# uc-vision/smart-tree

Measured on AMD Instinct MI355X. Metric: points/sec end-to-end (voxelize->sparse-UNet->skeleton), 1M-pt tree, higher is better.
Workload: dtype f32

## Files before the change

### include/smarttree_hip.h

```cpp
#ifndef SMARTTREE_HIP_H
#define SMARTTREE_HIP_H

#include <stdint.h>

#ifdef __cplusplus
extern "C" {
#endif

int st_version(void);
#define ST_SKELETON_STATS_ENTRIES 16
#define ST_SKELETON_TUNING_ENTRIES 24
int st_abi_entries(int what);
const char* st_last_error(void);
int64_t st_query_workspace(int op, int64_t a, int64_t b, int64_t c);

int64_t st_scan_workspace_bytes(int64_t n);
int st_scan_u32(const uint32_t* in, uint32_t* out, int64_t n, uint32_t* total, void* ws, int64_t ws_bytes, void* stream);
int64_t st_sort_workspace_bytes(int64_t n);
int st_sort_pairs_u32(uint32_t* keys, uint32_t* vals, int64_t n, int key_bits, void* ws, int64_t ws_bytes, void* stream);

int64_t st_voxelize_workspace_bytes(int64_t n_points, int max_blocks, int64_t max_voxels);
int st_voxelize_blocks(const float* xyz, const float* rgb, int64_t n, double voxel_size, double block_size,
                       double buffer_size, int min_points, int max_blocks, int64_t max_voxels, float* feats,
                       int32_t* coords, uint8_t* mask, int64_t* point_index, float* block_centres,
                       int64_t* n_voxels_host, int64_t* n_blocks_host, void* ws, int64_t ws_bytes, void* stream);

int64_t st_hash_capacity(int64_t n);
int st_build_coord_hash(const int32_t* coords, int64_t n, unsigned long long* keys, unsigned* vals, int64_t cap, void* stream);
int st_build_subm_rulebook(const int32_t* coords, int64_t n, const unsigned long long* keys, const unsigned* vals,
                           int64_t cap, int32_t* nbr , void* stream);
int64_t st_spatial_order_workspace_bytes(int64_t n);
int st_spatial_order(const int32_t* coords, int64_t n, int32_t* order , void* ws, int64_t ws_bytes, void* stream);
int st_move_rows(const void* src, int row_words, const int32_t* order, int64_t n, void* dst, int scatter, void* stream);
int64_t st_strided_workspace_bytes(int64_t n_fine);
int st_build_strided_outputs(const int32_t* coords, int64_t n, int64_t max_out, int32_t* out_coords,
                             unsigned long long* ckeys, unsigned* cvals, int64_t ccap, int64_t* n_out_host,
                             int32_t* extent_host , void* ws, int64_t ws_bytes, void* stream);
int st_build_strided_rulebook(const int32_t* coords, int64_t n, const unsigned long long* fkeys, const unsigned* fvals,
                              int64_t fcap, const int32_t* out_coords, int64_t n_out, const unsigned long long* ckeys,
                              const unsigned* cvals, int64_t ccap, const int32_t* extent_host,
                              int32_t* nbr_down , int32_t* nbr_up ,
                              int32_t* up_order ,
                              void* stream);

int st_sparse_conv_fwd(const float* x0, int c0, const float* x1, int cin, const int32_t* nbr, int K, int64_t n_out,
                       const float* w, int cout, const float* scale, const float* shift, const float* residual,
                       int relu, float* y, const int32_t* row_order ,
                       void* stream, int64_t nbr_stride );
int st_sparse_conv_mfma_fwd(const float* x0, int c0, const float* x1, int cin, const int32_t* nbr, int K, int64_t n_out,
                            const float* wp, int cout, const float* scale, const float* shift, const float* residual,
                            int relu, float* y, const int32_t* row_order ,
                            void* stream, int64_t nbr_stride ,
                            int variant );
int st_sparse_conv_b3_fwd(const float* x0, int c0, const float* x1, int cin, const int32_t* nbr, int K, int64_t n_out, const void* wq,
                          int cout, const float* scale, const float* shift, const float* residual, int relu, float* y,
                          const int32_t* row_order, void* stream, int64_t nbr_stride, int variant);
int st_sparse_conv_f16_fwd(const void* x0, int c0, const void* x1, int cin, const int32_t* nbr, int K, int64_t n_out,
                           const void* w, int cout, const float* scale, const float* shift, const void* residual, int relu,
                           void* y, int in_half, int out_half, const int32_t* row_order, void* stream, int64_t nbr_stride );

int64_t st_brick_pyramid_workspace_bytes(int64_t n0, int n_blocks, int coord_bound, int depth, const int64_t* caps);
int st_brick_pyramid(const int32_t* coords0 , int64_t n0, int n_blocks ,
                     int coord_bound , int depth, const int32_t* blk_seg ,
                     int nseg, const int64_t* caps ,
                     int32_t* order0 , int32_t* const* coords_out ,
                     int32_t* const* subm , int32_t* const* down ,
                     int32_t* const* up , int32_t* const* up_order ,
                     int64_t* counts_host , void* ws, int64_t ws_bytes, void* stream);
int st_head_param_floats(void);
int st_pointwise_mlp_heads(const float* x, int64_t n, const float* params, float* radius, float* direction,
                           float* class_l, float* medial_vector , int64_t* class_idx , void* stream);

int st_centre_cloud(const float* xyz, int64_t n, float* out, void* ws, int64_t ws_bytes, void* stream);
int st_medial_points(const float* xyz, const float* mv, int64_t n, float* medial, float* radius, void* stream);
int64_t st_knn_workspace_bytes(int64_t n_dst);
int st_knn_radius(const float* src, int64_t n1, const float* dst, int64_t n2, int K, float r, const float* bound,
                  int bound_mode, float cell_hint, int64_t* idx, float* dist, void* ws, int64_t ws_bytes, void* stream);
int64_t st_make_edges_workspace_bytes(int64_t n);
int st_make_edges(const int64_t* idx, const float* dist, int64_t n, int K, int64_t* edges, float* w,
                  int64_t* n_edges_host, void* ws, int64_t ws_bytes, void* stream);
int64_t st_connected_components_workspace_bytes(int64_t n);
int st_connected_components(const int64_t* edges, int64_t E, int64_t n, int32_t* labels, void* ws, int64_t ws_bytes, void* stream);
int64_t st_component_layout_workspace_bytes(int64_t n);
int st_component_layout(const int32_t* labels, int64_t n, int min_vertices, int32_t* comp_size, int32_t* comp_off,
                        int32_t* vert_order, int32_t* new_id, int64_t* n_comp_host, int64_t* n_kept_host, void* ws,
                        int64_t ws_bytes, void* stream);
int64_t st_component_csr_workspace_bytes(int64_t m);
int st_component_csr(const int64_t* edges, const float* w, int64_t E, const int32_t* new_id, int64_t m, uint32_t* row_off,
                     uint32_t* col, float* wgt, void* ws, int64_t ws_bytes, void* stream);
int64_t st_skeleton_workspace_bytes(int64_t m, int64_t n_comp);
int st_skeleton_components(int n_comp, const int32_t* comp_off, const int32_t* comp_size_host, int64_t m, const float* pts,
                           const float* rad, const float* ysurf, const uint32_t* row_off, const uint32_t* col,
                           const float* wgt, float grid_cell, int stages, int block_threads, float* dist, int32_t* pred,
                           int32_t* root_local, float* tree_dist, int32_t* branch_parent, int32_t* branch_off,
                           int32_t* branch_len, int32_t* n_branches, int32_t* path_verts, int32_t* branch_of,
                           int64_t* stats_host, void* ws, int64_t ws_bytes, void* stream);
#define ST_SKELETON_STAGE_ARGS                                                                                          \
    int n_comp, const int32_t *comp_off, const int32_t *comp_size_host, int64_t m, const float *pts, const float *rad, \
        const float *ysurf, const uint32_t *row_off, const uint32_t *col, const float *wgt, float grid_cell,           \
        int block_threads, float *dist, int32_t *pred, int32_t *root_local, float *tree_dist, int32_t *branch_parent,  \
        int32_t *branch_off, int32_t *branch_len, int32_t *n_branches, int32_t *path_verts, int32_t *branch_of,        \
        int64_t *stats_host, void *ws, int64_t ws_bytes, void *stream
int st_sssp(ST_SKELETON_STAGE_ARGS);
int st_tree_distance(ST_SKELETON_STAGE_ARGS);
int st_sample_tree(ST_SKELETON_STAGE_ARGS);
int64_t st_assemble_workspace_bytes(int64_t cap_b);
int st_assemble_branches(int n_comp, const int32_t* comp_off, const int32_t* n_branches, const int32_t* branch_parent,
                         const int32_t* branch_off, const int32_t* branch_len, const int32_t* path_verts,
                         const int32_t* vert_order, const float* medial, const float* radius, int32_t* tree_off,
                         int32_t* parent, int32_t* start, int32_t* length, float* xyz, float* rad, int64_t cap_b,
                         int64_t cap_p, int64_t* counts_host, void* ws, int64_t ws_bytes, void* stream);
int st_post_process(int n_trees, const int32_t* tree_off, const int32_t* parent, const int32_t* start, const int32_t* len,
                    float* xyz, const float* rad_in, float* rad_out, uint8_t* keep, uint8_t* repaired, uint8_t* smoothed,
                    int32_t* depth_scratch, int do_prune, float min_radius, float min_length, int do_repair, int do_smooth, int kernel_size,
                    void* stream);

int st_points_to_nearest_tube(const float* pts, int64_t n, const float* a, const float* b, const float* r1, const float* r2,
                              int64_t m, float* vec, int64_t* idx, float* rad, void* stream);

int st_centre_cloud_seg(const float* xyz, int64_t n, const int32_t* seg_off, int nseg, float* out, void* ws,
                        int64_t ws_bytes , void* stream);
int64_t st_voxelize_workspace_bytes_seg(int64_t n_points, int max_blocks, int64_t max_voxels, int nseg);
int st_voxelize_blocks_seg(const float* xyz, const float* rgb, int64_t n, const int32_t* seg_off, int nseg,
                           double voxel_size, double block_size, double buffer_size, int min_points, int max_blocks,
                           int64_t max_voxels, float* feats, int32_t* coords, uint8_t* mask, int64_t* point_index,
                           float* block_centres, int32_t* blk_seg ,
                           int32_t* seg_vox_off , int32_t* seg_blk_off , int64_t* n_voxels_host,
                           int64_t* n_blocks_host, void* ws, int64_t ws_bytes, void* stream);
int st_build_strided_outputs_seg(const int32_t* coords, int64_t n, int64_t max_out, int32_t* out_coords,
                                 unsigned long long* ckeys, unsigned* cvals, int64_t ccap, int64_t* n_out_host,
                                 int32_t* extent_host, const int32_t* blk_seg, int nseg, int32_t* ext_dev ,
                                 void* ws, int64_t ws_bytes, void* stream);
int st_build_strided_rulebook_seg(const int32_t* coords, int64_t n, const unsigned long long* fkeys, const unsigned* fvals,
                                  int64_t fcap, const int32_t* out_coords, int64_t n_out, const unsigned long long* ckeys,
                                  const unsigned* cvals, int64_t ccap, const int32_t* extent_host, int32_t* nbr_down,
                                  int32_t* nbr_up, int32_t* up_order, const int32_t* blk_seg, const int32_t* ext_dev,
                                  void* stream);
int64_t st_voxelize_cloud_workspace_bytes(int64_t n_points, int64_t max_voxels, int nseg);
int st_voxelize_cloud_seg(const float* xyz, const float* rgb, int64_t n, const int32_t* seg_off, int nseg, double voxel_size,
                          int64_t max_voxels, float* feats, int32_t* coords, uint8_t* mask, int64_t* point_index,
                          int32_t* seg_vox_off, int64_t* n_voxels_host, void* ws, int64_t ws_bytes, void* stream);
int64_t st_knn_workspace_bytes_seg(int64_t n_dst, int nseg);
int st_knn_radius_seg(const float* src, int64_t n1, const float* dst, int64_t n2, int K, float r, const float* bound,
                      int bound_mode, float cell_hint, int64_t* idx, float* dist, const int32_t* src_seg_off,
                      const int32_t* dst_seg_off, int nseg, void* ws, int64_t ws_bytes, void* stream, float cell_mean_mult);
int st_radius_count_seg(const float* src, int64_t n1, const float* dst, int64_t n2, int K, float r, const float* bound,
                        int bound_mode, float cell_hint, uint8_t* mask, const int32_t* src_seg_off,
                        const int32_t* dst_seg_off, int nseg, void* ws, int64_t ws_bytes, void* stream, float cell_mean_mult,
                        const uint8_t* valid );
int64_t st_component_csr_knn_workspace_bytes(int64_t m, int64_t n, int K);
int st_connected_components_knn(const int64_t* idx, int64_t n, int K, const int32_t* first_of , int32_t* labels, void* ws, int64_t ws_bytes, void* stream);
int st_component_csr_knn(const int64_t* idx, const float* dist, int64_t n, int K, const int32_t* first_of,
                         const int32_t* new_id, int64_t m, uint32_t* row_off, uint32_t* col, float* wgt, void* ws,
                         int64_t ws_bytes, void* stream);
int st_make_edges_seg(const int64_t* idx, const float* dist, int64_t n, int K, int64_t* edges, float* w,
                      int64_t* n_edges_host, const int32_t* seg_off, int nseg, void* ws, int64_t ws_bytes, void* stream);
int st_component_layout_seg(const int32_t* labels, int64_t n, int min_vertices, const int32_t* seg_off, int nseg,
                            int32_t* comp_size, int32_t* comp_off, int32_t* vert_order, int32_t* new_id,
                            int32_t* comp_seg , int32_t* comp_seg_off , int32_t* vert_seg_off ,
                            int64_t* n_comp_host, int64_t* n_kept_host, void* ws, int64_t ws_bytes, void* stream,
                            int64_t* max_comp_host );
int64_t st_skeleton_workspace_bytes_seg(int64_t m, int64_t n_comp, int nseg);
int st_skeleton_components_seg(int n_comp, const int32_t* comp_off, const int32_t* comp_seg, const int32_t* vert_seg_off,
                               int nseg, int64_t m, const float* pts, const float* rad, const float* ysurf,
                               const uint32_t* row_off, const uint32_t* col, const float* wgt, float grid_cell, int stages,
                               int block_threads, float* dist, int32_t* pred, int32_t* root_local, float* tree_dist,
                               int32_t* branch_parent, int32_t* branch_off, int32_t* branch_len, int32_t* n_branches,
                               int32_t* path_verts, int32_t* branch_of, int64_t* stats_host, void* ws, int64_t ws_bytes,
                               void* stream, const int64_t* tuning );
int st_post_process_seg(int n_trees, const int32_t* tree_off, const int32_t* parent, const int32_t* start, const int32_t* len,
                        float* xyz, const float* rad_in, float* rad_out, uint8_t* keep, uint8_t* repaired, uint8_t* smoothed,
                        int32_t* depth_scratch, int do_prune, float min_radius, float min_length, int do_repair,
                        int do_smooth, int kernel_size, const int32_t* first_tree ,
                        int n_first, void* stream);

int64_t st_loss_workspace_bytes(void);
int st_loss_forward(const float* radius, const float* direction, const float* class_l, int n_classes, const float* targets,
                    int target_cols, const uint8_t* mask, int64_t n, int vector_class, int target_radius_log,
                    double* out_host, void* ws, int64_t ws_bytes, void* stream);

int st_loss_backward(const float* radius, const float* direction, const float* class_l, int n_classes, const float* targets,
                     int target_cols, const uint8_t* mask, int64_t n, int vector_class, int target_radius_log,
                     double n_vector_rows, double n_class_rows, const float* upstream, float* d_radius, float* d_direction,
                     float* d_class_l, void* stream);

int64_t st_sparse_conv_wgrad_workspace_bytes(int K, int cin, int cout, int64_t n_out);
int st_sparse_conv_wgrad(const float* x0, int c0, const float* x1, int cin, const int32_t* nbr, int K, int64_t n_out,
                         int64_t nbr_stride, const float* dy, int cout, float* dw, void* ws, int64_t ws_bytes, void* stream);

int st_sparse_conv_h_fwd(const void* x0, int c0, const void* x1, int cin, const int32_t* nbr, int K, int64_t n_out,
                         int64_t nbr_stride, const void* w, int cout, void* y, void* stream);
int64_t st_sparse_conv_wgrad_h_workspace_bytes(int K, int cin, int cout, int64_t n_out);
int st_sparse_conv_wgrad_h(const void* x0, int c0, const void* x1, int cin, const int32_t* nbr, int K, int64_t n_out,
                           int64_t nbr_stride, const void* dy, int cout, float* dw, void* ws, int64_t ws_bytes, void* stream);
int st_move_rows_h(const void* src, int row_elems, const int32_t* order, int64_t n, void* dst, int scatter, void* stream);

int64_t st_bn_workspace_bytes(int64_t n, int C);
int st_bn_stats(const void* x, int half, int64_t n, int C, double* out, void* ws, int64_t ws_bytes, void* stream);
int st_bn_apply(const void* x, int half, int64_t n, int C, const float* mean, const float* invstd, const float* gamma,
                const float* beta, void* y, void* stream);
int st_bn_backward_stats(const void* x, const void* dy, int half, int64_t n, int C, const float* mean, const float* invstd,
                         double* out, void* ws, int64_t ws_bytes, void* stream);
int st_bn_backward_apply(const void* x, const void* dy, int half, int64_t n, int C, const float* mean, const float* invstd,
                         const float* gamma, const double* sums, const double* count, void* dx, void* stream);

#ifdef __cplusplus
}
#endif
#endif
```

### smart_tree_amd/_lib.py

```python
from __future__ import annotations

import ctypes
from ctypes import c_double, c_float, c_int, c_int64, c_void_p
from pathlib import Path

import torch

_PKG = Path(__file__).resolve().parent
LIB_PATH = _PKG / "libsmarttree_hip.so"

_LIB = None
_ALLOW_HOST_POINTERS = False

P = c_void_p
I64 = c_int64

SIGNATURES = {
    "st_version": (c_int, []),
    "st_abi_entries": (c_int, [c_int]),
    "st_last_error": (ctypes.c_char_p, []),
    "st_scan_workspace_bytes": (I64, [I64]),
    "st_scan_u32": (c_int, [P, P, I64, P, P, I64, P]),
    "st_sort_workspace_bytes": (I64, [I64]),
    "st_sort_pairs_u32": (c_int, [P, P, I64, c_int, P, I64, P]),
    "st_voxelize_workspace_bytes": (I64, [I64, c_int, I64]),
    "st_voxelize_blocks": (c_int, [P, P, I64, c_double, c_double, c_double, c_int, c_int, I64, P, P, P, P, P,
                                   ctypes.POINTER(I64), ctypes.POINTER(I64), P, I64, P]),
    "st_hash_capacity": (I64, [I64]),
    "st_build_coord_hash": (c_int, [P, I64, P, P, I64, P]),
    "st_build_subm_rulebook": (c_int, [P, I64, P, P, I64, P, P]),
    "st_strided_workspace_bytes": (I64, [I64]),
    "st_spatial_order_workspace_bytes": (I64, [I64]),
    "st_spatial_order": (c_int, [P, I64, P, P, I64, P]),
    "st_move_rows": (c_int, [P, c_int, P, I64, P, c_int, P]),
    "st_build_strided_outputs": (c_int, [P, I64, I64, P, P, P, I64, ctypes.POINTER(I64), ctypes.POINTER(ctypes.c_int32),
                                         P, I64, P]),
    "st_build_strided_rulebook": (c_int, [P, I64, P, P, I64, P, I64, P, P, I64, ctypes.POINTER(ctypes.c_int32), P, P, P, P]),
    "st_sparse_conv_fwd": (c_int, [P, c_int, P, c_int, P, c_int, I64, P, c_int, P, P, P, c_int, P, P, P, I64]),
    "st_sparse_conv_mfma_fwd": (c_int, [P, c_int, P, c_int, P, c_int, I64, P, c_int, P, P, P, c_int, P, P, P, I64, c_int]),
    "st_sparse_conv_b3_fwd": (c_int, [P, c_int, P, c_int, P, c_int, I64, P, c_int, P, P, P, c_int, P, P, P, I64, c_int]),
    "st_sparse_conv_f16_fwd": (c_int, [P, c_int, P, c_int, P, c_int, I64, P, c_int, P, P, P, c_int, P, c_int, c_int, P, P, I64]),
    "st_brick_pyramid_workspace_bytes": (I64, [I64, c_int, c_int, c_int, ctypes.POINTER(I64)]),
    "st_brick_pyramid": (c_int, [P, I64, c_int, c_int, c_int, P, c_int, ctypes.POINTER(I64), P, ctypes.POINTER(P), ctypes.POINTER(P),
                                 ctypes.POINTER(P), ctypes.POINTER(P), ctypes.POINTER(P), ctypes.POINTER(I64), P, I64, P]),
    "st_head_param_floats": (c_int, []),
    "st_pointwise_mlp_heads": (c_int, [P, I64, P, P, P, P, P, P, P]),
    "st_knn_workspace_bytes": (I64, [I64]),
    "st_knn_radius": (c_int, [P, I64, P, I64, c_int, c_float, P, c_int, c_float, P, P, P, I64, P]),
    "st_medial_points": (c_int, [P, P, I64, P, P, P]),
    "st_centre_cloud": (c_int, [P, I64, P, P, I64, P]),
    "st_make_edges_workspace_bytes": (I64, [I64]),
    "st_make_edges": (c_int, [P, P, I64, c_int, P, P, ctypes.POINTER(I64), P, I64, P]),
    "st_connected_components_workspace_bytes": (c_int64, [c_int64]),
    "st_connected_components": (c_int, [P, I64, I64, P, P, I64, P]),
    "st_component_layout_workspace_bytes": (I64, [I64]),
    "st_component_layout": (c_int, [P, I64, c_int, P, P, P, P, ctypes.POINTER(I64), ctypes.POINTER(I64), P, I64, P]),
    "st_component_csr_workspace_bytes": (I64, [I64]),
    "st_component_csr": (c_int, [P, P, I64, P, I64, P, P, P, P, I64, P]),
    "st_assemble_workspace_bytes": (c_int64, [c_int64]),
    "st_assemble_branches": (c_int, [c_int, P, P, P, P, P, P, P, P, P, P, P, P, P, P, P, c_int64, c_int64, P, P, c_int64, P]),
    "st_points_to_nearest_tube": (c_int, [P, c_int64, P, P, P, P, c_int64, P, P, P, P]),
    "st_post_process": (c_int, [c_int, P, P, P, P, P, P, P, P, P, P, P, c_int, c_float, c_float, c_int, c_int, c_int, P]),
    "st_skeleton_workspace_bytes": (I64, [I64, I64]),
    "st_centre_cloud_seg": (c_int, [P, I64, P, c_int, P, P, I64, P]),
    "st_voxelize_workspace_bytes_seg": (I64, [I64, c_int, I64, c_int]),
    "st_voxelize_blocks_seg": (c_int, [P, P, I64, P, c_int, c_double, c_double, c_double, c_int, c_int, I64, P, P, P, P, P, P, P, P,
                                       ctypes.POINTER(I64), ctypes.POINTER(I64), P, I64, P]),
    "st_voxelize_cloud_workspace_bytes": (I64, [I64, I64, c_int]),
    "st_voxelize_cloud_seg": (c_int, [P, P, I64, P, c_int, c_double, I64, P, P, P, P, P, ctypes.POINTER(I64), P, I64, P]),
    "st_loss_workspace_bytes": (I64, []),
    "st_loss_forward": (c_int, [P, P, P, c_int, P, c_int, P, I64, c_int, c_int, ctypes.POINTER(ctypes.c_double), P, I64, P]),
    "st_build_strided_outputs_seg": (c_int, [P, I64, I64, P, P, P, I64, ctypes.POINTER(I64), ctypes.POINTER(ctypes.c_int32),
                                             P, c_int, P, P, I64, P]),
    "st_build_strided_rulebook_seg": (c_int, [P, I64, P, P, I64, P, I64, P, P, I64, ctypes.POINTER(ctypes.c_int32), P, P, P, P, P, P]),
    "st_knn_workspace_bytes_seg": (I64, [I64, c_int]),
    "st_knn_radius_seg": (c_int, [P, I64, P, I64, c_int, c_float, P, c_int, c_float, P, P, P, P, c_int, P, I64, P, c_float]),
    "st_radius_count_seg": (c_int, [P, I64, P, I64, c_int, c_float, P, c_int, c_float, P, P, P, c_int, P, I64, P, c_float, P]),
    "st_connected_components_knn": (c_int, [P, I64, c_int, P, P, P, I64, P]),
    "st_component_csr_knn": (c_int, [P, P, I64, c_int, P, P, I64, P, P, P, P, I64, P]),
    "st_component_csr_knn_workspace_bytes": (I64, [I64, I64, c_int]),
    "st_make_edges_seg": (c_int, [P, P, I64, c_int, P, P, ctypes.POINTER(I64), P, c_int, P, I64, P]),
    "st_component_layout_seg": (c_int, [P, I64, c_int, P, c_int, P, P, P, P, P, P, P, ctypes.POINTER(I64), ctypes.POINTER(I64), P, I64, P,
                                        ctypes.POINTER(I64)]),
    "st_skeleton_workspace_bytes_seg": (I64, [I64, I64, c_int]),
    "st_skeleton_components_seg": (c_int, [c_int, P, P, P, c_int, I64, P, P, P, P, P, P, c_float, c_int, c_int, P, P, P, P, P, P, P, P,
                                           P, P, ctypes.POINTER(I64), P, I64, P, ctypes.POINTER(I64)]),
    "st_post_process_seg": (c_int, [c_int, P, P, P, P, P, P, P, P, P, P, P, c_int, c_float, c_float, c_int, c_int, c_int, P, c_int, P]),
    "st_loss_backward": (c_int, [P, P, P, c_int, P, c_int, P, I64, c_int, c_int, c_double, c_double, P, P, P, P, P]),
    "st_sparse_conv_wgrad_workspace_bytes": (I64, [c_int, c_int, c_int, I64]),
    "st_sparse_conv_wgrad": (c_int, [P, c_int, P, c_int, P, c_int, I64, I64, P, c_int, P, P, I64, P]),
    "st_sparse_conv_h_fwd": (c_int, [P, c_int, P, c_int, P, c_int, I64, I64, P, c_int, P, P]),
    "st_sparse_conv_wgrad_h_workspace_bytes": (I64, [c_int, c_int, c_int, I64]),
    "st_sparse_conv_wgrad_h": (c_int, [P, c_int, P, c_int, P, c_int, I64, I64, P, c_int, P, P, I64, P]),
    "st_move_rows_h": (c_int, [P, c_int, P, I64, P, c_int, P]),
    "st_bn_workspace_bytes": (I64, [I64, c_int]),
    "st_bn_stats": (c_int, [P, c_int, I64, c_int, P, P, I64, P]),
    "st_bn_apply": (c_int, [P, c_int, I64, c_int, P, P, P, P, P, P]),
    "st_bn_backward_stats": (c_int, [P, P, c_int, I64, c_int, P, P, P, P, I64, P]),
    "st_bn_backward_apply": (c_int, [P, P, c_int, I64, c_int, P, P, P, P, P, P, P]),
    "st_skeleton_components": (c_int, [c_int, P, P, I64, P, P, P, P, P, P, c_float, c_int, c_int, P, P, P, P, P, P, P, P,
                                       P, P, ctypes.POINTER(I64), P, I64, P]),
}


ENQUEUE_ONLY = frozenset({
    "st_version", "st_abi_entries", "st_last_error", "st_scan_workspace_bytes", "st_sort_workspace_bytes", "st_voxelize_workspace_bytes",
    "st_hash_capacity", "st_strided_workspace_bytes", "st_head_param_floats", "st_knn_workspace_bytes",
    "st_make_edges_workspace_bytes", "st_connected_components_workspace_bytes", "st_component_layout_workspace_bytes",
    "st_component_csr_workspace_bytes", "st_assemble_workspace_bytes", "st_skeleton_workspace_bytes",
    "st_build_coord_hash", "st_build_subm_rulebook", "st_build_strided_rulebook", "st_sparse_conv_fwd",
    "st_sparse_conv_mfma_fwd", "st_sparse_conv_b3_fwd", "st_sparse_conv_f16_fwd", "st_pointwise_mlp_heads", "st_medial_points", "st_centre_cloud",
    "st_connected_components", "st_component_csr", "st_post_process", "st_knn_radius", "st_brick_pyramid_workspace_bytes",
    "st_centre_cloud_seg", "st_voxelize_workspace_bytes_seg", "st_build_strided_rulebook_seg", "st_knn_workspace_bytes_seg",
    "st_knn_radius_seg", "st_skeleton_workspace_bytes_seg", "st_post_process_seg", "st_radius_count_seg",
    "st_voxelize_cloud_workspace_bytes", "st_loss_workspace_bytes", "st_spatial_order_workspace_bytes", "st_spatial_order", "st_connected_components_knn", "st_component_csr_knn", "st_component_csr_knn_workspace_bytes", "st_move_rows",
    "st_loss_backward", "st_sparse_conv_wgrad_workspace_bytes", "st_sparse_conv_wgrad",
    "st_sparse_conv_h_fwd", "st_sparse_conv_wgrad_h_workspace_bytes", "st_sparse_conv_wgrad_h", "st_move_rows_h",
    "st_bn_workspace_bytes", "st_bn_stats", "st_bn_apply", "st_bn_backward_stats", "st_bn_backward_apply",
})


NOWAIT_VARIANTS = ("st_make_edges", "st_assemble_branches", "st_make_edges_seg")


class _Bound:

    def __init__(self, cdll):
        self._cdll = cdll

    def __getattr__(self, name):
        return getattr(self._cdll, name)


def declare(cdll, pydll=None):
    out = _Bound(cdll) if pydll is not None else cdll
    for name, (res, args) in SIGNATURES.items():
        for handle in ((cdll, pydll) if pydll is not None else (cdll,)):
            fn = getattr(handle, name)
            fn.restype = res
            fn.argtypes = args
        if pydll is not None:
            setattr(out, name, getattr(pydll if name in ENQUEUE_ONLY else cdll, name))
    for name in NOWAIT_VARIANTS:
        setattr(out, name + "_nowait", getattr(pydll if pydll is not None else cdll, name))
    return out


def lib():
    global _LIB
    if _LIB is None:
        if not LIB_PATH.exists():
            raise RuntimeError(
                f"{LIB_PATH} is missing: the HIP extension has not been built. "
                "Run `python -c 'import __graft_entry__ as g; g.build()'` (needs hipcc). "
                "smart_tree_amd has no CPU fallback.")
        import os
        if os.environ.get("ST_CDLL_ONLY") == "1":
            _LIB = declare(ctypes.CDLL(str(LIB_PATH)))
        else:
            _LIB = declare(ctypes.CDLL(str(LIB_PATH)), ctypes.PyDLL(str(LIB_PATH)))
    return _LIB


class StError(RuntimeError):
    pass


def check(rc: int) -> None:
    if rc != 0:
        raise StError(f"smarttree_hip error {rc}: {lib().st_last_error().decode()}")


def ptr(t):
    if t is None:
        return None
    if not t.is_cuda and not _ALLOW_HOST_POINTERS:
        raise StError("smart_tree_amd kernels need tensors on the GPU (got a CPU tensor); there is no CPU fallback")
    if not t.is_contiguous():
        raise StError("smart_tree_amd kernels need contiguous tensors")
    return t.data_ptr()


_HAS_GPU = None
_RAW_STREAM = getattr(torch._C, "_cuda_getCurrentRawStream", None)


def stream(device=None):
    global _HAS_GPU
    if _HAS_GPU is None:
        _HAS_GPU = torch.cuda.is_available()
    if _HAS_GPU and not _ALLOW_HOST_POINTERS:
        if _RAW_STREAM is not None:
            idx = device.index if isinstance(device, torch.device) and device.index is not None else torch.cuda.current_device()
            return _RAW_STREAM(idx)
        return torch.cuda.current_stream(device).cuda_stream
    return None


def workspace(nbytes: int, device) -> torch.Tensor:
    ws = torch.empty(max(int(nbytes), 256), dtype=torch.uint8, device=device)
    if _ALLOW_HOST_POINTERS:
        ws.fill_(0xCD)
    return ws
```

### smart_tree_amd/csrc/graph.hip

```cpp
#include "st_common.h"
#include "st_grid.h"

#define GR_BLOCK 256
static inline unsigned gr_grid(int64_t n) {
    int64_t g = st_div_up(n > 0 ? n : 1, GR_BLOCK);
    return (unsigned)(g < 8192 ? g : 8192);
}
#define GR_LOOP(i, n) for (int64_t i = (int64_t)blockIdx.x * blockDim.x + threadIdx.x; i < (n); i += (int64_t)gridDim.x * blockDim.x)

__global__ void __launch_bounds__(GR_BLOCK) k_medial(const float* xyz, const float* mv, int64_t n, float* medial, float* radius) {
    GR_LOOP(i, n) {
        const float x = mv[3 * i], y = mv[3 * i + 1], z = mv[3 * i + 2];
        medial[3 * i] = xyz[3 * i] + x;
        medial[3 * i + 1] = xyz[3 * i + 1] + y;
        medial[3 * i + 2] = xyz[3 * i + 2] + z;
        float s = x * x;
        float t = y * y;
        s = s + t;
        t = z * z;
        s = s + t;
        radius[i] = sqrtf(s);
    }
}

extern "C" int st_medial_points(const float* xyz, const float* mv, int64_t n, float* medial, float* radius, void* stream_) {
    if (n <= 0) return ST_OK;
    hipLaunchKernelGGL(k_medial, dim3(gr_grid(n)), dim3(GR_BLOCK), 0, (hipStream_t)stream_, xyz, mv, n, medial, radius);
    ST_CHECK_LAUNCH();
    return ST_OK;
}

struct GrRange {
    int64_t i0, i1;
    int64_t a0, a1;
    int64_t nq;
};
__device__ __forceinline__ GrRange gr_range(const void* p0, const void* p1, int64_t n, const int* seg_off, int seg) {
    GrRange r;
    r.i0 = seg_off ? seg_off[seg] : 0;
    r.i1 = seg_off ? seg_off[seg + 1] : n;
    const bool vec = ((((uintptr_t)p0) | ((uintptr_t)p1)) & 15) == 0;
    r.a0 = vec ? st_min((r.i0 + 3) & ~(int64_t)3, r.i1) : r.i1;
    r.a1 = r.a0 + ((r.i1 - r.a0) & ~(int64_t)3);
    r.nq = (r.a1 - r.a0) / 4 * 3;
    return r;
}
__device__ __forceinline__ int64_t gr_edge_point(const GrRange& r, int64_t j) { return j < r.a0 - r.i0 ? r.i0 + j : r.a1 + (j - (r.a0 - r.i0)); }

__global__ void __launch_bounds__(GR_BLOCK) k_bbox(const float* xyz, int64_t n, unsigned* box, const int* seg_off) {
    __shared__ unsigned lo[3], hi[3];
    if (threadIdx.x < 3) { lo[threadIdx.x] = 0xffffffffu; hi[threadIdx.x] = 0u; }
    __syncthreads();
    const int seg = blockIdx.y;
    const GrRange r = gr_range(xyz, nullptr, n, seg_off, seg);
    unsigned lx = 0xffffffffu, ly = 0xffffffffu, lz = 0xffffffffu, hx = 0u, hy = 0u, hz = 0u;
    const float4* v = reinterpret_cast<const float4*>(xyz + 3 * r.a0);
    for (int64_t q = (int64_t)blockIdx.x * blockDim.x + threadIdx.x; q < r.nq; q += (int64_t)gridDim.x * blockDim.x) {
        const float4 f = v[q];
        const int ax = (int)(q % 3);
        const unsigned o0 = st_f2ord(f.x), o1 = st_f2ord(f.y), o2 = st_f2ord(f.z), o3 = st_f2ord(f.w);
        const unsigned a = st_min(o0, o3), b = st_max(o0, o3);
        lx = st_min(lx, ax == 0 ? a : (ax == 1 ? o2 : o1)); hx = st_max(hx, ax == 0 ? b : (ax == 1 ? o2 : o1));
        ly = st_min(ly, ax == 0 ? o1 : (ax == 1 ? a : o2)); hy = st_max(hy, ax == 0 ? o1 : (ax == 1 ? b : o2));
        lz = st_min(lz, ax == 0 ? o2 : (ax == 1 ? o1 : a)); hz = st_max(hz, ax == 0 ? o2 : (ax == 1 ? o1 : b));
    }
    const int64_t ne = (r.a0 - r.i0) + (r.i1 - r.a1);
    for (int64_t j = (int64_t)blockIdx.x * blockDim.x + threadIdx.x; j < ne; j += (int64_t)gridDim.x * blockDim.x) {
        const int64_t i = gr_edge_point(r, j);
        const unsigned ox = st_f2ord(xyz[3 * i]), oy = st_f2ord(xyz[3 * i + 1]), oz = st_f2ord(xyz[3 * i + 2]);
        lx = st_min(lx, ox); hx = st_max(hx, ox); ly = st_min(ly, oy); hy = st_max(hy, oy); lz = st_min(lz, oz); hz = st_max(hz, oz);
    }
    for (int d = 32; d > 0; d >>= 1) {
        lx = st_min(lx, (unsigned)__shfl_xor((int)lx, d)); ly = st_min(ly, (unsigned)__shfl_xor((int)ly, d)); lz = st_min(lz, (unsigned)__shfl_xor((int)lz, d));
        hx = st_max(hx, (unsigned)__shfl_xor((int)hx, d)); hy = st_max(hy, (unsigned)__shfl_xor((int)hy, d)); hz = st_max(hz, (unsigned)__shfl_xor((int)hz, d));
    }
    if ((threadIdx.x & 63) == 0) {
        atomicMin(&lo[0], lx); atomicMin(&lo[1], ly); atomicMin(&lo[2], lz);
        atomicMax(&hi[0], hx); atomicMax(&hi[1], hy); atomicMax(&hi[2], hz);
    }
    __syncthreads();
    if (threadIdx.x < 3 && r.i1 > r.i0) { atomicMin(&box[6 * seg + threadIdx.x], lo[threadIdx.x]); atomicMax(&box[6 * seg + 3 + threadIdx.x], hi[threadIdx.x]); }
}
__global__ void __launch_bounds__(GR_BLOCK) k_centre(const float* xyz, int64_t n, const unsigned* box, float* out, const int* seg_off) {
    const int seg = blockIdx.y;
    const GrRange r = gr_range(xyz, out, n, seg_off, seg);
    float shift[3];
    for (int a = 0; a < 3; a++) {
        const float mn = st_ord2f(box[6 * seg + a]), mx = st_ord2f(box[6 * seg + 3 + a]);
        const float half = (mx - mn) / 2.0f;
        const float centre = mn + half;
        shift[a] = -centre + (a == 1 ? half : 0.0f);
    }
    const float4* v = reinterpret_cast<const float4*>(xyz + 3 * r.a0);
    float4* o = reinterpret_cast<float4*>(out + 3 * r.a0);
    for (int64_t q = (int64_t)blockIdx.x * blockDim.x + threadIdx.x; q < r.nq; q += (int64_t)gridDim.x * blockDim.x) {
        float4 f = v[q];
        const int ax = (int)(q % 3);
        const float s0 = ax == 0 ? shift[0] : (ax == 1 ? shift[1] : shift[2]);
        const float s1 = ax == 0 ? shift[1] : (ax == 1 ? shift[2] : shift[0]);
        const float s2 = ax == 0 ? shift[2] : (ax == 1 ? shift[0] : shift[1]);
        f.x = f.x + s0; f.y = f.y + s1; f.z = f.z + s2; f.w = f.w + s0;
        o[q] = f;
    }
    const int64_t ne = (r.a0 - r.i0) + (r.i1 - r.a1);
    for (int64_t j = (int64_t)blockIdx.x * blockDim.x + threadIdx.x; j < ne; j += (int64_t)gridDim.x * blockDim.x) {
        const int64_t i = gr_edge_point(r, j);
        for (int a = 0; a < 3; a++) out[3 * i + a] = xyz[3 * i + a] + shift[a];
    }
}

__global__ void k_box_init(unsigned* box, int nseg) {
    for (int i = threadIdx.x; i < 6 * nseg; i += blockDim.x) box[i] = i % 6 < 3 ? 0xffffffffu : 0u;
}

extern "C" int st_centre_cloud_seg(const float* xyz, int64_t n, const int32_t* seg_off, int nseg, float* out, void* ws,
                                   int64_t ws_bytes, void* stream_) {
    hipStream_t stream = (hipStream_t)stream_;
    if (n <= 0) return ST_OK;
    ST_REQUIRE(nseg >= 1 && nseg <= ST_MAX_SEG && (nseg == 1 || seg_off), "centre_cloud: 1 <= clouds per batch <= %d", ST_MAX_SEG);
    if (nseg == 1) seg_off = nullptr;
    StArena a(ws, ws_bytes);
    unsigned* box = a.take<unsigned>(6 * (int64_t)nseg);
    if (!box) { st_set_error("centre_cloud: workspace too small"); return ST_ERR_WORKSPACE; }
    hipLaunchKernelGGL(k_box_init, dim3(1), dim3(64), 0, stream, box, nseg);
    const int64_t per = st_div_up(st_div_up(3 * n, 4), nseg);
    const unsigned gx = (unsigned)st_min64(st_div_up(per > 0 ? per : 1, GR_BLOCK), 2048 / (nseg < 8 ? nseg : 8) + 1);
    hipLaunchKernelGGL(k_bbox, dim3(gx, (unsigned)nseg), dim3(GR_BLOCK), 0, stream, xyz, n, box, seg_off);
    hipLaunchKernelGGL(k_centre, dim3((unsigned)st_min64(st_div_up(per > 0 ? per : 1, GR_BLOCK), 8192), (unsigned)nseg), dim3(GR_BLOCK), 0, stream,
                       xyz, n, (const unsigned*)box, out, seg_off);
    ST_CHECK_LAUNCH();
    return ST_OK;
}
extern "C" int st_centre_cloud(const float* xyz, int64_t n, float* out, void* ws, int64_t ws_bytes, void* stream_) {
    return st_centre_cloud_seg(xyz, n, nullptr, 1, out, ws, ws_bytes, stream_);
}

__global__ void __launch_bounds__(GR_BLOCK) k_edge_count(const int64_t* idx, int64_t n, int K, uint32_t* cnt, const int* seg_off,
                                                         int nseg) {
    GR_LOOP(i, n) {
        const int64_t first = seg_off ? seg_off[st_seg_find(seg_off, nseg, i)] : 0;
        uint32_t c = 0;
        for (int k = 0; k < K; k++) c += idx[i * K + k] > first;
        cnt[i] = c;
    }
}
__global__ void __launch_bounds__(GR_BLOCK) k_edge_emit(const int64_t* idx, const float* dist, int64_t n, int K,
                                                        const uint32_t* off, int64_t* edges, float* w, const int* seg_off,
                                                        int nseg) {
    GR_LOOP(i, n) {
        const int64_t first = seg_off ? seg_off[st_seg_find(seg_off, nseg, i)] : 0;
        uint32_t o = off[i];
        for (int k = 0; k < K; k++) {
            int64_t j = idx[i * K + k];
            if (j > first) { edges[2 * (int64_t)o] = i; edges[2 * (int64_t)o + 1] = j; w[o] = dist[i * K + k]; o++; }
        }
    }
}

extern "C" int64_t st_make_edges_workspace_bytes(int64_t n) {
    StArena a(nullptr, 0);
    a.take<uint32_t>(n + 1);
    a.take<char>(st_scan_ws_bytes(n));
    return a.used;
}

__global__ void __launch_bounds__(GR_BLOCK) k_edge_pad(int64_t* edges, float* w, const uint32_t* total, int64_t cap) {
    for (int64_t e = (int64_t)*total + (int64_t)blockIdx.x * blockDim.x + threadIdx.x; e < cap; e += (int64_t)gridDim.x * blockDim.x) {
        edges[2 * e] = 0;
        edges[2 * e + 1] = 0;
        w[e] = 0.0f;
    }
}

extern "C" int st_make_edges_seg(const int64_t* idx, const float* dist, int64_t n, int K, int64_t* edges, float* w,
                                 int64_t* n_edges_host, const int32_t* seg_off, int nseg, void* ws, int64_t ws_bytes,
                                 void* stream_) {
    hipStream_t stream = (hipStream_t)stream_;
    if (n_edges_host) *n_edges_host = 0;
    if (n <= 0) return ST_OK;
    ST_REQUIRE(nseg >= 1 && nseg <= ST_MAX_SEG && (nseg == 1 || seg_off), "make_edges: 1 <= clouds per batch <= %d", ST_MAX_SEG);
    if (nseg == 1) seg_off = nullptr;
    StArena a(ws, ws_bytes);
    uint32_t* cnt = a.take<uint32_t>(n + 1);
    int64_t sb = st_scan_ws_bytes(n);
    char* sw = a.take<char>(sb);
    if (!cnt || !sw) { st_set_error("make_edges: workspace too small"); return ST_ERR_WORKSPACE; }
    hipLaunchKernelGGL(k_edge_count, dim3(gr_grid(n)), dim3(GR_BLOCK), 0, stream, idx, n, K, cnt, seg_off, nseg);
    ST_TRY(st_exclusive_scan_u32(cnt, cnt, n, cnt + n, sw, sb, stream));
    hipLaunchKernelGGL(k_edge_emit, dim3(gr_grid(n)), dim3(GR_BLOCK), 0, stream, idx, dist, n, K, (const uint32_t*)cnt, edges, w,
                       seg_off, nseg);
    if (!n_edges_host) {
        hipLaunchKernelGGL(k_edge_pad, dim3(64), dim3(GR_BLOCK), 0, stream, edges, w, (const uint32_t*)(cnt + n), n * (int64_t)K);
        ST_CHECK_LAUNCH();
        return ST_OK;
    }
    uint32_t total = 0;
    (void)hipMemcpyAsync(&total, cnt + n, sizeof(uint32_t), hipMemcpyDeviceToHost, stream);
    st_stream_wait(stream);
    ST_CHECK_LAUNCH();
    *n_edges_host = total;
    return ST_OK;
}

extern "C" int st_make_edges(const int64_t* idx, const float* dist, int64_t n, int K, int64_t* edges, float* w,
                             int64_t* n_edges_host, void* ws, int64_t ws_bytes, void* stream_) {
    return st_make_edges_seg(idx, dist, n, K, edges, w, n_edges_host, nullptr, 1, ws, ws_bytes, stream_);
}

struct GrEdges {
    const int64_t* edges;
    const float* w;
    const int64_t* idx;
    const float* dist;
    int K, k_shift;
    const int* first_of;
};
static inline int gr_shift_of(int K) { int sh = 0; while ((1 << sh) < K) sh++; return (1 << sh) == K ? sh : -1; }
__device__ __forceinline__ void gr_edge(const GrEdges& G, int64_t e, int64_t* u, int64_t* v) {
    if (G.idx == nullptr) { *u = G.edges[2 * e]; *v = G.edges[2 * e + 1]; return; }
    const int64_t i = G.k_shift >= 0 ? (e >> G.k_shift) : e / G.K, j = G.idx[e];
    const int64_t first = G.first_of ? G.first_of[i] : 0;
    *u = i;
    *v = j > first ? j : i;
}
__device__ __forceinline__ float gr_edge_weight(const GrEdges& G, int64_t e) { return G.idx ? G.dist[e] : G.w[e]; }

#define CC_MUL 0x9E3779B1u
#define CC_INV 0x0E8B2F51u
__device__ __forceinline__ unsigned cc_key(unsigned x) { return x * CC_MUL; }
__device__ __forceinline__ unsigned cc_idx(unsigned k) { return k * CC_INV; }

__device__ __forceinline__ unsigned cc_find(unsigned* label, unsigned k) {
    unsigned p = __atomic_load_n(&label[cc_idx(k)], __ATOMIC_RELAXED);
    while (p != k) {
        const unsigned gp = __atomic_load_n(&label[cc_idx(p)], __ATOMIC_RELAXED);
        if (gp != p) atomicMin(&label[cc_idx(k)], gp);
        k = p;
        p = gp;
    }
    return k;
}
__global__ void __launch_bounds__(GR_BLOCK) k_cc_init(unsigned* label, int64_t n) { GR_LOOP(i, n) label[i] = cc_key((unsigned)i); }
__global__ void __launch_bounds__(GR_BLOCK) k_cc_hook(GrEdges G, int64_t E, unsigned* label, int sample) {
    GR_LOOP(e, E) {
        if (sample && (((uint32_t)e * 2654435761u) >> 29) != 0u) continue;
        int64_t u64, v64;
        gr_edge(G, e, &u64, &v64);
        const unsigned u = (unsigned)u64, v = (unsigned)v64;
        if (u == v) continue;
        if (!sample) {
            if (label[u] == label[v]) continue;
        }
        unsigned a = cc_find(label, cc_key(u)), b = cc_find(label, cc_key(v));
        while (a != b) {
            if (a < b) { const unsigned t = a; a = b; b = t; }
            const unsigned seen = atomicCAS(&label[cc_idx(a)], a, b);
            if (seen == a) break;
            a = seen;
        }
    }
}
__global__ void __launch_bounds__(GR_BLOCK) k_cc_compress(unsigned* label, int64_t n) {
    GR_LOOP(i, n) { const unsigned r = cc_find(label, cc_key((unsigned)i)); label[i] = r; }
}
__global__ void __launch_bounds__(GR_BLOCK) k_cc_minid_init(unsigned* minid, int64_t n) { GR_LOOP(i, n) minid[i] = 0xffffffffu; }
__global__ void __launch_bounds__(GR_BLOCK) k_cc_minid(const unsigned* label, int64_t n, unsigned* minid) {
    const int lane = threadIdx.x & 63;
    for (int64_t base = (int64_t)blockIdx.x * blockDim.x; base < n; base += (int64_t)gridDim.x * blockDim.x) {
        const int64_t i = base + threadIdx.x;
        const bool valid = i < n;
        const unsigned r = valid ? cc_idx(label[i]) : 0xffffffffu;
        unsigned long long todo = __ballot(valid);
        while (todo) {
            const int leader = __ffsll(todo) - 1;
            const unsigned lr = __shfl(r, leader);
            const unsigned long long same = __ballot(valid && r == lr);
            if (lane == leader) atomicMin(&minid[lr], (unsigned)i);
            todo &= ~same;
        }
    }
}
__global__ void __launch_bounds__(GR_BLOCK) k_cc_relabel(unsigned* label, int64_t n, const unsigned* minid) {
    GR_LOOP(i, n) label[i] = minid[cc_idx(label[i])];
}

extern "C" int64_t st_connected_components_workspace_bytes(int64_t n) { return (n > 0 ? n : 1) * (int64_t)sizeof(unsigned) + 256; }

static int cc_run(GrEdges G, int64_t E, int64_t n, int32_t* labels, void* ws, int64_t ws_bytes, void* stream_);

extern "C" int st_connected_components(const int64_t* edges, int64_t E, int64_t n, int32_t* labels, void* ws,
                                       int64_t ws_bytes, void* stream_) {
    GrEdges G = {edges, nullptr, nullptr, nullptr, 0, -1, nullptr};
    return cc_run(G, E, n, labels, ws, ws_bytes, stream_);
}

extern "C" int st_connected_components_knn(const int64_t* idx, int64_t n, int K, const int32_t* first_of,
                                           int32_t* labels, void* ws, int64_t ws_bytes, void* stream_) {
    ST_REQUIRE(K >= 1, "cc(knn): K must be positive");
    GrEdges G = {nullptr, nullptr, idx, nullptr, K, gr_shift_of(K), first_of};
    return cc_run(G, n * (int64_t)K, n, labels, ws, ws_bytes, stream_);
}

static int cc_run(GrEdges G, int64_t E, int64_t n, int32_t* labels, void* ws, int64_t ws_bytes, void* stream_) {
    hipStream_t stream = (hipStream_t)stream_;
    ST_REQUIRE(n < (1ll << 31), "cc: too many vertices");
    if (n <= 0) return ST_OK;
    StArena ar(ws, ws_bytes);
    unsigned* minid = ar.take<unsigned>(n);
    if (!ar.ok() || !minid) {
        st_set_error("cc: workspace too small (%lld < %lld)", (long long)ws_bytes, (long long)ar.used);
        return ST_ERR_WORKSPACE;
    }
    unsigned* label = (unsigned*)labels;
    hipLaunchKernelGGL(k_cc_init, dim3(gr_grid(n)), dim3(GR_BLOCK), 0, stream, label, n);
    if (E > 0) {
        hipLaunchKernelGGL(k_cc_hook, dim3(gr_grid(E)), dim3(GR_BLOCK), 0, stream, G, E, label, 1);
        hipLaunchKernelGGL(k_cc_compress, dim3(gr_grid(n)), dim3(GR_BLOCK), 0, stream, label, n);
        hipLaunchKernelGGL(k_cc_hook, dim3(gr_grid(E)), dim3(GR_BLOCK), 0, stream, G, E, label, 0);
    }
    hipLaunchKernelGGL(k_cc_compress, dim3(gr_grid(n)), dim3(GR_BLOCK), 0, stream, label, n);
    hipLaunchKernelGGL(k_cc_minid_init, dim3(gr_grid(n)), dim3(GR_BLOCK), 0, stream, minid, n);
    hipLaunchKernelGGL(k_cc_minid, dim3(gr_grid(n)), dim3(GR_BLOCK), 0, stream, (const unsigned*)label, n, minid);
    hipLaunchKernelGGL(k_cc_relabel, dim3(gr_grid(n)), dim3(GR_BLOCK), 0, stream, label, n, (const unsigned*)minid);
    ST_CHECK_LAUNCH();
    return ST_OK;
}

__global__ void __launch_bounds__(GR_BLOCK) k_cl_sizes(const int* label, int64_t n, uint32_t* size) {
    const int lane = threadIdx.x & 63;
    for (int64_t base = (int64_t)blockIdx.x * blockDim.x; base < n; base += (int64_t)gridDim.x * blockDim.x) {
        const int64_t i = base + threadIdx.x;
        const bool valid = i < n;
        const int lab = valid ? label[i] : -1;
        unsigned long long todo = __ballot(valid);
        while (todo) {
            const int leader = __ffsll(todo) - 1;
            const int l = __shfl(lab, leader);
            const unsigned long long same = __ballot(valid && lab == l);
            if (lane == leader) atomicAdd(&size[l], (uint32_t)__popcll(same));
            todo &= ~same;
        }
    }
}
__global__ void __launch_bounds__(GR_BLOCK) k_cl_rootflag(const int* label, const uint32_t* size, int64_t n, uint32_t minv,
                                                          uint32_t* flag, uint32_t* kept) {
    GR_LOOP(i, n) {
        const bool root = label[i] == (int)i && size[i] >= minv;
        flag[i] = root ? 1u : 0u;
        if (root) { atomicAdd(kept, size[i]); atomicMax(kept + 1, size[i]); }
    }
}
__global__ void __launch_bounds__(GR_BLOCK) k_cl_rootlist(const uint32_t* flag_off, const int* label, const uint32_t* size,
                                                          int64_t n, uint32_t minv, uint32_t* key, uint32_t* root) {
    GR_LOOP(i, n) if (label[i] == (int)i && size[i] >= minv) { key[flag_off[i]] = 0xffffffffu - size[i]; root[flag_off[i]] = (uint32_t)i; }
}
__global__ void __launch_bounds__(GR_BLOCK) k_cl_rank(const uint32_t* root_sorted, const uint32_t* size, int64_t C,
                                                      int* rank_of_root, uint32_t* comp_size) {
    GR_LOOP(c, C) { rank_of_root[root_sorted[c]] = (int)c; comp_size[c] = size[root_sorted[c]]; }
}
__global__ void __launch_bounds__(GR_BLOCK) k_cl_segkey(const uint32_t* root_sorted, int64_t C, const int* seg_off, int nseg,
                                                        uint32_t* key) {
    GR_LOOP(c, C) key[c] = (uint32_t)st_seg_find(seg_off, nseg, root_sorted[c]);
}
__global__ void __launch_bounds__(GR_BLOCK) k_cl_segments(const uint32_t* root_sorted, int C, const int* seg_off, int nseg,
                                                          const int32_t* comp_off, int32_t* comp_seg, int32_t* comp_seg_off,
                                                          int32_t* vert_seg_off) {
    for (int b = threadIdx.x; b <= nseg; b += blockDim.x) comp_seg_off[b] = C;
    __syncthreads();
    for (int c = threadIdx.x; c < C; c += blockDim.x) {
        const int s = st_seg_find(seg_off, nseg, root_sorted[c]);
        comp_seg[c] = s;
        const int prev = c > 0 ? st_seg_find(seg_off, nseg, root_sorted[c - 1]) : -1;
        for (int b = prev + 1; b <= s; b++) comp_seg_off[b] = c;
    }
    __syncthreads();
    for (int b = threadIdx.x; b <= nseg; b += blockDim.x) vert_seg_off[b] = comp_off[comp_seg_off[b]];
}
__global__ void __launch_bounds__(GR_BLOCK) k_cl_vflag(const int* label, const int* rank_of_root, int64_t n, uint32_t* flag) {
    GR_LOOP(i, n) flag[i] = rank_of_root[label[i]] >= 0 ? 1u : 0u;
}
__global__ void __launch_bounds__(GR_BLOCK) k_cl_vlist(const uint32_t* flag_off, const int* label, const int* rank_of_root,
                                                       int64_t n, uint32_t* vkey, uint32_t* vid) {
    GR_LOOP(i, n) {
        int r = rank_of_root[label[i]];
        if (r >= 0) { vkey[flag_off[i]] = (uint32_t)r; vid[flag_off[i]] = (uint32_t)i; }
    }
}
__global__ void __launch_bounds__(GR_BLOCK) k_cl_newid(const uint32_t* vid_sorted, int64_t m, int* new_id, int32_t* vert_order) {
    GR_LOOP(p, m) { new_id[vid_sorted[p]] = (int)p; vert_order[p] = (int32_t)vid_sorted[p]; }
}
__global__ void __launch_bounds__(GR_BLOCK) k_fill_i32(int* p, int64_t n, int v) { GR_LOOP(i, n) p[i] = v; }

extern "C" int64_t st_component_layout_workspace_bytes(int64_t n) {
    StArena a(nullptr, 0);
    a.take<uint32_t>(n + 2);
    a.take<uint32_t>(n + 1);
    a.take<uint32_t>(n);
    a.take<uint32_t>(n);
    a.take<int>(n);
    a.take<char>(st_sort_ws_bytes(n) > st_scan_ws_bytes(n + 1) ? st_sort_ws_bytes(n) : st_scan_ws_bytes(n + 1));
    return a.used;
}

extern "C" int st_component_layout_seg(const int32_t* labels, int64_t n, int min_vertices, const int32_t* seg_off, int nseg,
                                       int32_t* comp_size, int32_t* comp_off, int32_t* vert_order, int32_t* new_id,
                                       int32_t* comp_seg, int32_t* comp_seg_off, int32_t* vert_seg_off,
                                       int64_t* n_comp_host, int64_t* n_kept_host, void* ws, int64_t ws_bytes, void* stream_,
                                       int64_t* max_comp_host ) {
    hipStream_t stream = (hipStream_t)stream_;
    *n_comp_host = 0;
    *n_kept_host = 0;
    if (max_comp_host) *max_comp_host = 0;
    ST_REQUIRE(nseg >= 1 && nseg <= ST_MAX_SEG, "component_layout: 1 <= clouds per batch <= %d", ST_MAX_SEG);
    ST_REQUIRE(nseg == 1 || (seg_off && comp_seg && comp_seg_off && vert_seg_off), "component_layout: a batch needs seg_off and the per-cloud outputs");
    if (n <= 0) {
        if (nseg > 1) { (void)hipMemsetAsync(comp_seg_off, 0, (nseg + 1) * sizeof(int32_t), stream); (void)hipMemsetAsync(vert_seg_off, 0, (nseg + 1) * sizeof(int32_t), stream); }
        return ST_OK;
    }
    StArena a(ws, ws_bytes);
    uint32_t* size = a.take<uint32_t>(n + 2);
    uint32_t* flag = a.take<uint32_t>(n + 1);
    uint32_t* key = a.take<uint32_t>(n);
    uint32_t* val = a.take<uint32_t>(n);
    int* rank_of_root = a.take<int>(n);
    int64_t sb = st_sort_ws_bytes(n) > st_scan_ws_bytes(n + 1) ? st_sort_ws_bytes(n) : st_scan_ws_bytes(n + 1);
    char* sw = a.take<char>(sb);
    if (!a.ok() || !sw) { st_set_error("component_layout: workspace too small"); return ST_ERR_WORKSPACE; }
    const unsigned g = gr_grid(n);
    uint32_t minv = min_vertices > 0 ? (uint32_t)min_vertices : 0u;
    (void)hipMemsetAsync(size, 0, (n + 2) * sizeof(uint32_t), stream);
    hipLaunchKernelGGL(k_cl_sizes, dim3(g), dim3(GR_BLOCK), 0, stream, labels, n, size);
    hipLaunchKernelGGL(k_cl_rootflag, dim3(g), dim3(GR_BLOCK), 0, stream, labels, (const uint32_t*)size, n, minv, flag, size + n);
    ST_TRY(st_exclusive_scan_u32(flag, flag, n, flag + n, sw, sb, stream));
    uint32_t C = 0, mk[2] = {0, 0};
    (void)hipMemcpyAsync(&C, flag + n, sizeof(uint32_t), hipMemcpyDeviceToHost, stream);
    (void)hipMemcpyAsync(mk, size + n, 2 * sizeof(uint32_t), hipMemcpyDeviceToHost, stream);
    st_stream_wait(stream);
    const uint32_t m = mk[0];
    if (max_comp_host) *max_comp_host = mk[1];
    ST_CHECK_LAUNCH();
    hipLaunchKernelGGL(k_fill_i32, dim3(g), dim3(GR_BLOCK), 0, stream, new_id, n, -1);
    if (C == 0) {
        if (nseg > 1) { (void)hipMemsetAsync(comp_seg_off, 0, (nseg + 1) * sizeof(int32_t), stream); (void)hipMemsetAsync(vert_seg_off, 0, (nseg + 1) * sizeof(int32_t), stream); }
        ST_CHECK_LAUNCH();
        return ST_OK;
    }
    hipLaunchKernelGGL(k_cl_rootlist, dim3(g), dim3(GR_BLOCK), 0, stream, (const uint32_t*)flag, labels, (const uint32_t*)size, n,
                       minv, key, val);
    ST_TRY(st_radix_sort_pairs_u32(key, val, C, 32, sw, sb, stream));
    if (nseg > 1) {
        int sbits = 1;
        while ((1 << sbits) < nseg) sbits++;
        hipLaunchKernelGGL(k_cl_segkey, dim3(gr_grid(C)), dim3(GR_BLOCK), 0, stream, (const uint32_t*)val, (int64_t)C, seg_off, nseg, key);
        ST_TRY(st_radix_sort_pairs_u32(key, val, C, sbits, sw, sb, stream));
    }
    hipLaunchKernelGGL(k_fill_i32, dim3(g), dim3(GR_BLOCK), 0, stream, rank_of_root, n, -1);
    hipLaunchKernelGGL(k_cl_rank, dim3(gr_grid(C)), dim3(GR_BLOCK), 0, stream, (const uint32_t*)val, (const uint32_t*)size,
                       (int64_t)C, rank_of_root, (uint32_t*)comp_size);
    ST_TRY(st_exclusive_scan_u32((const uint32_t*)comp_size, (uint32_t*)comp_off, C, (uint32_t*)comp_off + C, sw, sb, stream));
    if (nseg > 1)
        hipLaunchKernelGGL(k_cl_segments, dim3(1), dim3(GR_BLOCK), 0, stream, (const uint32_t*)val, (int)C, seg_off, nseg,
                           (const int32_t*)comp_off, comp_seg, comp_seg_off, vert_seg_off);
    hipLaunchKernelGGL(k_cl_vflag, dim3(g), dim3(GR_BLOCK), 0, stream, labels, (const int*)rank_of_root, n, flag);
    ST_TRY(st_exclusive_scan_u32(flag, flag, n, flag + n, sw, sb, stream));
    hipLaunchKernelGGL(k_cl_vlist, dim3(g), dim3(GR_BLOCK), 0, stream, (const uint32_t*)flag, labels, (const int*)rank_of_root, n,
                       key, val);
    int bits = 1;
    while ((1u << bits) < C && bits < 32) bits++;
    ST_TRY(st_radix_sort_pairs_u32(key, val, m, bits, sw, sb, stream));
    hipLaunchKernelGGL(k_cl_newid, dim3(gr_grid(m)), dim3(GR_BLOCK), 0, stream, (const uint32_t*)val, (int64_t)m, new_id,
                       vert_order);
    ST_CHECK_LAUNCH();
    *n_comp_host = C;
    *n_kept_host = m;
    return ST_OK;
}

extern "C" int st_component_layout(const int32_t* labels, int64_t n, int min_vertices, int32_t* comp_size, int32_t* comp_off,
                                   int32_t* vert_order, int32_t* new_id, int64_t* n_comp_host, int64_t* n_kept_host,
                                   void* ws, int64_t ws_bytes, void* stream_) {
    return st_component_layout_seg(labels, n, min_vertices, nullptr, 1, comp_size, comp_off, vert_order, new_id, nullptr, nullptr,
                                   nullptr, n_comp_host, n_kept_host, ws, ws_bytes, stream_, nullptr);
}

__device__ __forceinline__ uint32_t gr_run_add(uint32_t* ctr, int key) {
    const int lane = threadIdx.x & 63;
    const int prev = __shfl_up(key, 1);
    const bool head = key >= 0 && (lane == 0 || prev != key);
    const unsigned long long heads = __ballot(head), active = __ballot(key >= 0);
    const unsigned long long upto = heads & (~0ull >> (63 - lane));
    const int h = 63 - __clzll((long long)(upto | 1ull));
    const unsigned long long stop = (heads | ~active) & ~(~0ull >> (63 - h));
    const int end = stop ? __ffsll((long long)stop) - 1 : 64;
    uint32_t base = 0;
    if (head) base = atomicAdd(&ctr[key], (uint32_t)(end - lane));
    base = __shfl(base, h);
    return base + (uint32_t)(lane - h);
}

__device__ __forceinline__ void csr_edge_ends(const GrEdges& G, int64_t E, const int* new_id, int64_t e, int* a, int* b) {
    *a = -1; *b = -1;
    if (e >= E) return;
    int64_t u, v;
    gr_edge(G, e, &u, &v);
    if (u == v) return;
    const int x = new_id[u], y = new_id[v];
    if (x < 0 || y < 0) return;
    *a = x; *b = y;
}

__global__ void __launch_bounds__(GR_BLOCK) k_csr_count(GrEdges G, int64_t E, const int* new_id, uint32_t* deg) {
    const int lane = threadIdx.x & 63;
    for (int64_t base = (int64_t)blockIdx.x * blockDim.x + (threadIdx.x - lane); base < E; base += (int64_t)gridDim.x * blockDim.x) {
        int a, b;
        csr_edge_ends(G, E, new_id, base + lane, &a, &b);
        gr_run_add(deg, a);
        if (b >= 0) atomicAdd(&deg[b], 1u);
    }
}
__global__ void __launch_bounds__(GR_BLOCK) k_csr_fill(GrEdges G, int64_t E, const int* new_id,
                                                       uint32_t* cursor, uint32_t* col, float* wgt) {
    const int lane = threadIdx.x & 63;
    for (int64_t base = (int64_t)blockIdx.x * blockDim.x + (threadIdx.x - lane); base < E; base += (int64_t)gridDim.x * blockDim.x) {
        int a, b;
        csr_edge_ends(G, E, new_id, base + lane, &a, &b);
        const uint32_t pa = gr_run_add(cursor, a);
        if (a < 0) continue;
        const float we = gr_edge_weight(G, base + lane);
        col[pa] = (uint32_t)b; wgt[pa] = we;
        const uint32_t pb = atomicAdd(&cursor[b], 1u);
        col[pb] = (uint32_t)a; wgt[pb] = we;
    }
}

#define CSRK_MUTUAL 0x40000000
struct __attribute__((aligned(16))) GrI64x2 { int64_t x, y; };
template <int K>
__global__ void __launch_bounds__(GR_BLOCK) k_csrk_count(const int64_t* __restrict__ idx, int64_t n, const int* __restrict__ first_of,
                                                         const int* __restrict__ new_id, uint32_t* deg, uint32_t* fwdc,
                                                         int32_t* __restrict__ tgt) {
    const int64_t E = n * K;
    const int lane = threadIdx.x & 63;
    for (int64_t base = (int64_t)blockIdx.x * blockDim.x + (threadIdx.x - lane); base < E; base += (int64_t)gridDim.x * blockDim.x) {
        const int64_t e = base + lane;
        const int64_t i = e / K;
        int x = -1, y = -1;
        bool mutual = false;
        if (e < E) {
            x = new_id[i];
            const int64_t j = idx[e], first = first_of ? first_of[i] : 0;
            if (x >= 0 && j > first && j != i) {
                y = new_id[j];
                if (y >= 0 && i > first) {
                    const int64_t* row = idx + j * K;
                    if (K % 2 == 0) {
#pragma unroll
                        for (int k = 0; k < K; k += 2) {
                            const GrI64x2 r = *reinterpret_cast<const GrI64x2*>(row + k);
                            mutual = mutual || r.x == i || r.y == i;
                        }
                    } else {
                        for (int k = 0; k < K; k++) mutual = mutual || row[k] == i;
                    }
                }
            }
        }
        const bool fwd = y >= 0;
        const unsigned long long fb = __ballot(fwd);
        if (e < E) tgt[e] = fwd ? (y | (mutual ? CSRK_MUTUAL : 0)) : -1;
        if (fwd && !mutual) atomicAdd(&deg[y], 1u);
        if ((lane % K) == 0 && x >= 0) {
            const unsigned cnt = (unsigned)__popcll(K == 64 ? fb : (fb >> lane) & ((1ull << (K & 63)) - 1ull));
            fwdc[x] = cnt;
            if (cnt) atomicAdd(&deg[x], cnt);
        }
    }
}
template <int K>
__global__ void __launch_bounds__(GR_BLOCK) k_csrk_fill(const int64_t n, const float* __restrict__ dist, const int* __restrict__ new_id,
                                                        const int32_t* __restrict__ tgt, const uint32_t* __restrict__ row_off,
                                                        uint32_t* cursor, uint32_t* __restrict__ col, float* __restrict__ wgt) {
    const int64_t E = n * K;
    const int lane = threadIdx.x & 63;
    for (int64_t base = (int64_t)blockIdx.x * blockDim.x + (threadIdx.x - lane); base < E; base += (int64_t)gridDim.x * blockDim.x) {
        const int64_t e = base + lane;
        const int32_t t = e < E ? tgt[e] : -1;
        const bool fwd = t >= 0;
        const unsigned long long fb = __ballot(fwd);
        if (!fwd) continue;
        const int x = new_id[e / K], y = t & ~CSRK_MUTUAL;
        const float we = dist[e];
        const int k = lane % K;
        const unsigned long long mine = K == 64 ? fb : (fb >> (lane - k)) & ((1ull << (K & 63)) - 1ull);
        const uint32_t pa = row_off[x] + (uint32_t)__popcll(mine & ((1ull << k) - 1ull));
        col[pa] = (uint32_t)y; wgt[pa] = we;
        if (!(t & CSRK_MUTUAL)) {
            const uint32_t pb = atomicAdd(&cursor[y], 1u);
            col[pb] = (uint32_t)x; wgt[pb] = we;
        }
    }
}
__global__ void __launch_bounds__(GR_BLOCK) k_csrk_cursor(const uint32_t* __restrict__ row_off, const uint32_t* __restrict__ fwdc, int64_t m,
                                                          uint32_t* __restrict__ cursor) {
    GR_LOOP(v, m) cursor[v] = row_off[v] + fwdc[v];
}

extern "C" int64_t st_component_csr_workspace_bytes(int64_t m) {
    StArena a(nullptr, 0);
    a.take<uint32_t>(m + 1);
    a.take<char>(st_scan_ws_bytes(m + 1));
    return a.used;
}
extern "C" int64_t st_component_csr_knn_workspace_bytes(int64_t m, int64_t n, int K) {
    StArena a(nullptr, 0);
    a.take<uint32_t>(m + 1);
    a.take<char>(st_scan_ws_bytes(m + 1));
    a.take<uint32_t>(m + 1);
    a.take<int32_t>(n * (int64_t)(K > 0 ? K : 1));
    return a.used;
}

static int csr_run(GrEdges G, int64_t E, const int32_t* new_id, int64_t m, uint32_t* row_off, uint32_t* col, float* wgt, void* ws,
                   int64_t ws_bytes, void* stream_);

extern "C" int st_component_csr(const int64_t* edges, const float* w, int64_t E, const int32_t* new_id, int64_t m,
                                uint32_t* row_off, uint32_t* col, float* wgt, void* ws, int64_t ws_bytes, void* stream_) {
    GrEdges G = {edges, w, nullptr, nullptr, 0, -1, nullptr};
    return csr_run(G, E, new_id, m, row_off, col, wgt, ws, ws_bytes, stream_);
}

template <int K>
static void csrk_launch(const int64_t* idx, const float* dist, int64_t n, const int32_t* first_of, const int32_t* new_id, int64_t m,
                        uint32_t* row_off, uint32_t* col, float* wgt, uint32_t* cursor, uint32_t* fwdc, int32_t* tgt, char* sw, int64_t sb,
                        hipStream_t stream, int* rc) {
    const int64_t E = n * K;
    (void)hipMemsetAsync(row_off, 0, (m + 1) * sizeof(uint32_t), stream);
    hipLaunchKernelGGL((k_csrk_count<K>), dim3(gr_grid(E)), dim3(GR_BLOCK), 0, stream, idx, n, first_of, new_id, row_off, fwdc, tgt);
    *rc = st_exclusive_scan_u32(row_off, row_off, m + 1, nullptr, sw, sb, stream);
    if (*rc != ST_OK) return;
    hipLaunchKernelGGL(k_csrk_cursor, dim3(gr_grid(m)), dim3(GR_BLOCK), 0, stream, (const uint32_t*)row_off, (const uint32_t*)fwdc, m, cursor);
    hipLaunchKernelGGL((k_csrk_fill<K>), dim3(gr_grid(E)), dim3(GR_BLOCK), 0, stream, n, dist, new_id, (const int32_t*)tgt,
                       (const uint32_t*)row_off, cursor, col, wgt);
}
extern "C" int st_component_csr_knn(const int64_t* idx, const float* dist, int64_t n, int K, const int32_t* first_of,
                                    const int32_t* new_id, int64_t m, uint32_t* row_off, uint32_t* col, float* wgt, void* ws,
                                    int64_t ws_bytes, void* stream_) {
    ST_REQUIRE(K >= 1, "csr(knn): K must be positive");
    hipStream_t stream = (hipStream_t)stream_;
    if (m > 0 && n > 0 && gr_shift_of(K) >= 0 && K <= 64 && ws_bytes >= st_component_csr_knn_workspace_bytes(m, n, K)) {
        ST_REQUIRE(m < CSRK_MUTUAL, "csr(knn): too many vertices");
        StArena a(ws, ws_bytes);
        uint32_t* cursor = a.take<uint32_t>(m + 1);
        const int64_t sb = st_scan_ws_bytes(m + 1);
        char* sw = a.take<char>(sb);
        uint32_t* fwdc = a.take<uint32_t>(m + 1);
        int32_t* tgt = a.take<int32_t>(n * (int64_t)K);
        if (!cursor || !sw || !fwdc || !tgt) { st_set_error("component_csr(knn): workspace too small"); return ST_ERR_WORKSPACE; }
        int rc = ST_OK;
#define CSRK_CASE(K_) case K_: csrk_launch<K_>(idx, dist, n, first_of, new_id, m, row_off, col, wgt, cursor, fwdc, tgt, sw, sb, stream, &rc); break;
        switch (K) { CSRK_CASE(1) CSRK_CASE(2) CSRK_CASE(4) CSRK_CASE(8) CSRK_CASE(16) CSRK_CASE(32) CSRK_CASE(64) }
#undef CSRK_CASE
        if (rc != ST_OK) return rc;
        ST_CHECK_LAUNCH();
        return ST_OK;
    }
    GrEdges G = {nullptr, nullptr, idx, dist, K, gr_shift_of(K), first_of};
    return csr_run(G, n * (int64_t)K, new_id, m, row_off, col, wgt, ws, ws_bytes, stream_);
}

static int csr_run(GrEdges G, int64_t E, const int32_t* new_id, int64_t m, uint32_t* row_off, uint32_t* col, float* wgt, void* ws,
                   int64_t ws_bytes, void* stream_) {
    hipStream_t stream = (hipStream_t)stream_;
    if (m <= 0) return ST_OK;
    StArena a(ws, ws_bytes);
    uint32_t* cursor = a.take<uint32_t>(m + 1);
    int64_t sb = st_scan_ws_bytes(m + 1);
    char* sw = a.take<char>(sb);
    if (!cursor || !sw) { st_set_error("component_csr: workspace too small"); return ST_ERR_WORKSPACE; }
    (void)hipMemsetAsync(row_off, 0, (m + 1) * sizeof(uint32_t), stream);
    if (E > 0) hipLaunchKernelGGL(k_csr_count, dim3(gr_grid(E)), dim3(GR_BLOCK), 0, stream, G, E, new_id, row_off);
    ST_TRY(st_exclusive_scan_u32(row_off, row_off, m + 1, nullptr, sw, sb, stream));
    (void)hipMemcpyAsync(cursor, row_off, (m + 1) * sizeof(uint32_t), hipMemcpyDeviceToDevice, stream);
    if (E > 0) hipLaunchKernelGGL(k_csr_fill, dim3(gr_grid(E)), dim3(GR_BLOCK), 0, stream, G, E, new_id, cursor, col, wgt);
    ST_CHECK_LAUNCH();
    return ST_OK;
}
```

### smart_tree_amd/csrc/prims.hip

```cpp
#include <cstdarg>

#include "st_common.h"

static thread_local char g_err[512] = "";

void st_set_error(const char* fmt, ...) {
    va_list ap;
    va_start(ap, fmt);
    vsnprintf(g_err, sizeof(g_err), fmt, ap);
    va_end(ap);
}

extern "C" const char* st_last_error(void) { return g_err; }
void st_stream_wait(hipStream_t stream) { (void)hipStreamSynchronize(stream); }

extern "C" int st_version(void) { return 104; }

#define SCAN_BLOCK 256
#define SCAN_ITEMS 16
#define SCAN_TILE (SCAN_BLOCK * SCAN_ITEMS)
#define SCAN_DIRECT_BLOCKS 1024

__device__ __forceinline__ void scan_load(const uint32_t* in, int64_t base, int64_t n, uint32_t (&v)[SCAN_ITEMS]) {
    if (base + SCAN_ITEMS <= n && ((((uintptr_t)in) & 15) == 0)) {
        const uint4* p = reinterpret_cast<const uint4*>(in + base);
#pragma unroll
        for (int q = 0; q < SCAN_ITEMS / 4; q++) {
            const uint4 t = p[q];
            v[4 * q] = t.x; v[4 * q + 1] = t.y; v[4 * q + 2] = t.z; v[4 * q + 3] = t.w;
        }
    } else {
#pragma unroll
        for (int i = 0; i < SCAN_ITEMS; i++) v[i] = base + i < n ? in[base + i] : 0u;
    }
}

__global__ void __launch_bounds__(SCAN_BLOCK) k_scan_reduce(const uint32_t* in, uint32_t* block_sums, int64_t n, const int64_t* n_dev) {
    __shared__ uint32_t lds[SCAN_BLOCK / 64 + 1];
    if (n_dev) {
        const int64_t m = *n_dev;
        n = m < n ? m : n;
        if ((int64_t)blockIdx.x * SCAN_TILE >= n) { if (threadIdx.x == 0) block_sums[blockIdx.x] = 0u; return; }
    }
    int64_t base = (int64_t)blockIdx.x * SCAN_TILE + (int64_t)threadIdx.x * SCAN_ITEMS;
    uint32_t v[SCAN_ITEMS];
    scan_load(in, base, n, v);
    uint32_t s = 0;
#pragma unroll
    for (int i = 0; i < SCAN_ITEMS; i++) s += v[i];
    uint32_t total;
    block_exclusive_scan(s, lds, &total);
    if (threadIdx.x == 0) block_sums[blockIdx.x] = total;
}

__global__ void __launch_bounds__(SCAN_BLOCK) k_scan_apply(const uint32_t* in, uint32_t* out, const uint32_t* block_sums,
                                                           int64_t n, uint32_t* total_out, int sums_scanned, const int64_t* n_dev) {
    __shared__ uint32_t lds[SCAN_BLOCK / 64 + 1];
    if (n_dev) {
        const int64_t m = *n_dev;
        n = m < n ? m : n;
        const bool last_live = (int64_t)blockIdx.x * SCAN_TILE < n && ((int64_t)blockIdx.x + 1) * SCAN_TILE >= n;
        if ((int64_t)blockIdx.x * SCAN_TILE >= n && !(n == 0 && blockIdx.x == 0)) return;
        if (total_out && !last_live && !(n == 0)) total_out = nullptr;
    } else if (blockIdx.x != gridDim.x - 1) {
        total_out = nullptr;
    }
    uint32_t carry;
    if (sums_scanned) {
        carry = block_sums[blockIdx.x];
    } else {
        uint32_t pre = 0;
        for (int64_t j = threadIdx.x; j < (int64_t)blockIdx.x; j += SCAN_BLOCK) pre += block_sums[j];
        block_exclusive_scan(pre, lds, &carry);
    }
    int64_t base = (int64_t)blockIdx.x * SCAN_TILE + (int64_t)threadIdx.x * SCAN_ITEMS;
    uint32_t v[SCAN_ITEMS];
    scan_load(in, base, n, v);
    uint32_t s = 0;
#pragma unroll
    for (int i = 0; i < SCAN_ITEMS; i++) s += v[i];
    uint32_t total;
    uint32_t ex = block_exclusive_scan(s, lds, &total) + carry;
    if (base + SCAN_ITEMS <= n && ((((uintptr_t)out) & 15) == 0)) {
        uint4* p = reinterpret_cast<uint4*>(out + base);
#pragma unroll
        for (int q = 0; q < SCAN_ITEMS / 4; q++) {
            uint4 t;
            t.x = ex; ex += v[4 * q];
            t.y = ex; ex += v[4 * q + 1];
            t.z = ex; ex += v[4 * q + 2];
            t.w = ex; ex += v[4 * q + 3];
            p[q] = t;
        }
    } else {
#pragma unroll
        for (int i = 0; i < SCAN_ITEMS; i++) {
            if (base + i < n) out[base + i] = ex;
            ex += v[i];
        }
    }
    if (total_out && threadIdx.x == 0) *total_out = carry + total;
}

int64_t st_scan_ws_bytes(int64_t n) {
    StArena a(nullptr, 0);
    for (int64_t nb = st_div_up(n > 0 ? n : 1, SCAN_TILE);; nb = st_div_up(nb, SCAN_TILE)) {
        a.take<uint32_t>(nb + 1);
        if (nb <= SCAN_DIRECT_BLOCKS) break;
    }
    return a.used;
}

static int scan_level(const uint32_t* in, uint32_t* out, int64_t n, uint32_t* total, StArena& a, hipStream_t stream,
                      const int64_t* n_dev = nullptr) {
    const int64_t nb = st_div_up(n, SCAN_TILE);
    uint32_t* sums = a.take<uint32_t>(nb + 1);
    if (!sums) {
        st_set_error("scan: workspace too small (%lld < %lld)", (long long)a.size, (long long)a.used);
        return ST_ERR_WORKSPACE;
    }
    hipLaunchKernelGGL(k_scan_reduce, dim3((unsigned)nb), dim3(SCAN_BLOCK), 0, stream, in, sums, n, n_dev);
    const bool deep = nb > SCAN_DIRECT_BLOCKS;
    if (deep) ST_TRY(scan_level(sums, sums, nb, sums + nb, a, stream));
    hipLaunchKernelGGL(k_scan_apply, dim3((unsigned)nb), dim3(SCAN_BLOCK), 0, stream, in, out, (const uint32_t*)sums, n, total,
                       deep ? 1 : 0, n_dev);
    return ST_OK;
}

int st_exclusive_scan_u32(const uint32_t* in, uint32_t* out, int64_t n, uint32_t* total, void* ws, int64_t ws_bytes,
                          hipStream_t stream, const int64_t* n_dev) {
    if (n <= 0) {
        if (total) (void)hipMemsetAsync(total, 0, sizeof(uint32_t), stream);
        return ST_OK;
    }
    StArena a(ws, ws_bytes);
    ST_TRY(scan_level(in, out, n, total, a, stream, n_dev));
    ST_CHECK_LAUNCH();
    return ST_OK;
}

__global__ void __launch_bounds__(SCAN_BLOCK) k_fill_u32_dev(uint32_t* p, int64_t n, const int64_t* n_dev, uint32_t value) {
    const int64_t m = *n_dev < n ? *n_dev : n;
    for (int64_t i = ((int64_t)blockIdx.x * blockDim.x + threadIdx.x) * 4; i < m; i += (int64_t)gridDim.x * blockDim.x * 4) {
        if (i + 4 <= m && ((((uintptr_t)p) & 15) == 0)) *reinterpret_cast<uint4*>(p + i) = make_uint4(value, value, value, value);
        else for (int64_t j = i; j < m && j < i + 4; j++) p[j] = value;
    }
}
void st_fill_u32_dev(uint32_t* p, int64_t n, const int64_t* n_dev, uint32_t value, hipStream_t stream) {
    if (n <= 0) return;
    const int64_t g = st_div_up(st_div_up(n, 4), SCAN_BLOCK);
    hipLaunchKernelGGL(k_fill_u32_dev, dim3((unsigned)(g < 16384 ? g : 16384)), dim3(SCAN_BLOCK), 0, stream, p, n, n_dev, value);
}

#define SORT_BLOCK 256
#define SORT_ITEMS 4
#define SORT_TILE (SORT_BLOCK * SORT_ITEMS)
#define SORT_WAVES (SORT_BLOCK / 64)

__global__ void __launch_bounds__(SORT_BLOCK) k_sort_hist(const uint32_t* keys, int64_t n, int shift, uint32_t* hist,
                                                          int64_t nb) {
    __shared__ uint32_t h[256];
    h[threadIdx.x] = 0;
    __syncthreads();
    int64_t base = (int64_t)blockIdx.x * SORT_TILE;
    for (int r = 0; r < SORT_ITEMS; r++) {
        int64_t e = base + (int64_t)r * SORT_BLOCK + threadIdx.x;
        if (e < n) atomicAdd(&h[(keys[e] >> shift) & 255u], 1u);
    }
    __syncthreads();
    hist[(int64_t)threadIdx.x * nb + blockIdx.x] = h[threadIdx.x];
}

__global__ void __launch_bounds__(SORT_BLOCK) k_sort_scatter(const uint32_t* keys, const uint32_t* vals, uint32_t* okeys,
                                                             uint32_t* ovals, int64_t n, int shift, const uint32_t* hist,
                                                             int64_t nb) {
    __shared__ uint32_t running[256];
    __shared__ uint32_t wd[SORT_WAVES][256];
    const int tid = threadIdx.x, lane = tid & 63, wave = tid >> 6;
    running[tid] = hist[(int64_t)tid * nb + blockIdx.x];
    for (int w = 0; w < SORT_WAVES; w++) wd[w][tid] = 0;
    __syncthreads();
    int64_t base = (int64_t)blockIdx.x * SORT_TILE;
    for (int r = 0; r < SORT_ITEMS; r++) {
        int64_t e = base + (int64_t)r * SORT_BLOCK + tid;
        bool valid = e < n;
        uint32_t key = valid ? keys[e] : 0u;
        uint32_t val = valid ? vals[e] : 0u;
        uint32_t digit = (key >> shift) & 255u;
        unsigned long long peers = __ballot(valid);
        for (int b = 0; b < 8; b++) {
            bool bit = (digit >> b) & 1u;
            unsigned long long bal = __ballot(valid && bit);
            peers &= bit ? bal : ~bal;
        }
        unsigned long long below = peers & ((1ull << lane) - 1ull);
        uint32_t rank = (uint32_t)__popcll(below);
        if (valid && rank == 0) wd[wave][digit] = (uint32_t)__popcll(peers);
        __syncthreads();
        if (valid) {
            uint32_t off = running[digit] + rank;
            for (int w = 0; w < wave; w++) off += wd[w][digit];
            okeys[off] = key;
            ovals[off] = val;
        }
        __syncthreads();
        uint32_t add = 0;
        for (int w = 0; w < SORT_WAVES; w++) {
            add += wd[w][tid];
            wd[w][tid] = 0;
        }
        running[tid] += add;
        __syncthreads();
    }
}

int64_t st_sort_ws_bytes(int64_t n) {
    if (n <= 0) n = 1;
    StArena a(nullptr, 0);
    int64_t nb = st_div_up(n, SORT_TILE);
    a.take<uint32_t>(n);
    a.take<uint32_t>(n);
    a.take<uint32_t>(256 * nb);
    a.take<char>(st_scan_ws_bytes(256 * nb));
    return a.used;
}

int st_radix_sort_pairs_u32(uint32_t* keys, uint32_t* vals, int64_t n, int key_bits, void* ws, int64_t ws_bytes,
                            hipStream_t stream) {
    if (n <= 1 || key_bits <= 0) return ST_OK;
    StArena a(ws, ws_bytes);
    int64_t nb = st_div_up(n, SORT_TILE);
    uint32_t* tk = a.take<uint32_t>(n);
    uint32_t* tv = a.take<uint32_t>(n);
    uint32_t* hist = a.take<uint32_t>(256 * nb);
    int64_t scan_bytes = st_scan_ws_bytes(256 * nb);
    char* scan_ws = a.take<char>(scan_bytes);
    if (!tk || !tv || !hist || !scan_ws) {
        st_set_error("sort: workspace too small (%lld < %lld)", (long long)ws_bytes, (long long)a.used);
        return ST_ERR_WORKSPACE;
    }
    uint32_t *ik = keys, *iv = vals, *ok = tk, *ov = tv;
    for (int shift = 0; shift < key_bits; shift += 8) {
        hipLaunchKernelGGL(k_sort_hist, dim3((unsigned)nb), dim3(SORT_BLOCK), 0, stream, (const uint32_t*)ik, n, shift,
                           hist, nb);
        ST_TRY(st_exclusive_scan_u32(hist, hist, 256 * nb, nullptr, scan_ws, scan_bytes, stream));
        hipLaunchKernelGGL(k_sort_scatter, dim3((unsigned)nb), dim3(SORT_BLOCK), 0, stream, (const uint32_t*)ik,
                           (const uint32_t*)iv, ok, ov, n, shift, (const uint32_t*)hist, nb);
        uint32_t* t;
        t = ik; ik = ok; ok = t;
        t = iv; iv = ov; ov = t;
    }
    if (ik != keys) {
        (void)hipMemcpyAsync(keys, ik, n * sizeof(uint32_t), hipMemcpyDeviceToDevice, stream);
        (void)hipMemcpyAsync(vals, iv, n * sizeof(uint32_t), hipMemcpyDeviceToDevice, stream);
    }
    ST_CHECK_LAUNCH();
    return ST_OK;
}

extern "C" int64_t st_scan_workspace_bytes(int64_t n) { return st_scan_ws_bytes(n); }
extern "C" int st_scan_u32(const uint32_t* in, uint32_t* out, int64_t n, uint32_t* total, void* ws, int64_t ws_bytes,
                           void* stream) {
    return st_exclusive_scan_u32(in, out, n, total, ws, ws_bytes, (hipStream_t)stream);
}
extern "C" int64_t st_sort_workspace_bytes(int64_t n) { return st_sort_ws_bytes(n); }
extern "C" int st_sort_pairs_u32(uint32_t* keys, uint32_t* vals, int64_t n, int key_bits, void* ws, int64_t ws_bytes,
                                 void* stream) {
    return st_radix_sort_pairs_u32(keys, vals, n, key_bits, ws, ws_bytes, (hipStream_t)stream);
}

extern "C" int64_t st_voxelize_workspace_bytes(int64_t, int, int64_t);
extern "C" int64_t st_strided_workspace_bytes(int64_t);
extern "C" int64_t st_knn_workspace_bytes(int64_t);
extern "C" int64_t st_make_edges_workspace_bytes(int64_t);
extern "C" int64_t st_component_layout_workspace_bytes(int64_t);
extern "C" int64_t st_component_csr_workspace_bytes(int64_t);
extern "C" int64_t st_skeleton_workspace_bytes(int64_t, int64_t);
extern "C" int64_t st_query_workspace(int op, int64_t a, int64_t b, int64_t c) {
    switch (op) {
        case 0: return st_scan_ws_bytes(a);
        case 1: return st_sort_ws_bytes(a);
        case 2: return st_voxelize_workspace_bytes(a, (int)b, c);
        case 3: return st_strided_workspace_bytes(a);
        case 4: return st_knn_workspace_bytes(a);
        case 5: return st_make_edges_workspace_bytes(a);
        case 6: return st_component_layout_workspace_bytes(a);
        case 7: return st_component_csr_workspace_bytes(a);
        case 8: return st_skeleton_workspace_bytes(a, b);
        default: st_set_error("st_query_workspace: unknown op %d", op); return -1;
    }
}
```

### smart_tree_amd/csrc/voxelize.hip

```cpp
#include "st_common.h"
#include "st_grid.h"

#define VX_BLOCK 256
#define VX_TABLE_CAP 32768
static inline int64_t vx_table_cells(int max_blocks, int nseg) {
    const int64_t want = 8ll * ((max_blocks + nseg - 1) / (nseg > 0 ? nseg : 1));
    return want > VX_TABLE_CAP ? want : VX_TABLE_CAP;
}
#define VX_LDS_BLOCKS 128

struct VxState {
    int lo[3], hi[3];
    uint32_t n_blocks;
    uint32_t n_vox;
    uint32_t overflow;
    int table_cells;
    uint32_t seg_blk_off[ST_MAX_SEG + 1];
    uint32_t seg_vox_off[ST_MAX_SEG + 1];
};

struct VxParams {
    float bs;
    float bs_inv;
    float half_outer;
    float half_inner;
    float bs_half;
    float vs;
    float vs_inv;
    int min_points;
    int max_blocks;
    int nseg;
    int whole;
};

__device__ __forceinline__ int vx_block_id(float v, const VxParams& p) {
    if (p.whole) return 0;
    return (int)floorf(p.bs_inv != 0.0f ? v * p.bs_inv : v / p.bs);
}

template <class F>
__device__ __forceinline__ void vx_stream_points(const float* __restrict__ xyz, int64_t n_total, int64_t i0, int64_t i1, F fn) {
    const bool vec = (((uintptr_t)xyz) & 15) == 0;
    const int64_t step = (int64_t)gridDim.x * blockDim.x * 4;
    for (int64_t base = (i0 & ~(int64_t)3) + ((int64_t)blockIdx.x * blockDim.x + threadIdx.x) * 4; base < i1; base += step) {
        float c[12];
        if (vec && base + 4 <= n_total) {
            const float4* v = reinterpret_cast<const float4*>(xyz + 3 * base);
            const float4 f0 = v[0], f1 = v[1], f2 = v[2];
            c[0] = f0.x; c[1] = f0.y; c[2] = f0.z; c[3] = f0.w; c[4] = f1.x; c[5] = f1.y; c[6] = f1.z; c[7] = f1.w;
            c[8] = f2.x; c[9] = f2.y; c[10] = f2.z; c[11] = f2.w;
        } else {
#pragma unroll
            for (int j = 0; j < 12; j++) c[j] = base + j / 3 < n_total ? xyz[3 * base + j] : 0.0f;
        }
#pragma unroll
        for (int j = 0; j < 4; j++) {
            const int64_t i = base + j;
            if (i >= i0 && i < i1) fn(i, c[3 * j], c[3 * j + 1], c[3 * j + 2]);
        }
    }
}

__global__ void k_vx_init(VxState* st, int table_cells) {
    if (threadIdx.x == 0 && blockIdx.x == 0) {
        st->table_cells = table_cells;
        for (int a = 0; a < 3; a++) { st->lo[a] = 0x7fffffff; st->hi[a] = (int)0x80000000; }
        st->n_blocks = 0; st->n_vox = 0; st->overflow = 0;
    }
}

__device__ __forceinline__ int vx_wave_min(int v) { for (int d = 32; d > 0; d >>= 1) { const int o = __shfl_xor(v, d); v = o < v ? o : v; } return v; }
__device__ __forceinline__ int vx_wave_max(int v) { for (int d = 32; d > 0; d >>= 1) { const int o = __shfl_xor(v, d); v = o > v ? o : v; } return v; }

__global__ void __launch_bounds__(VX_BLOCK) k_vx_bbox(const float* xyz, int64_t n, const int* seg_off, VxParams p, VxState* st) {
    __shared__ int lo[3], hi[3];
    if (threadIdx.x < 3) { lo[threadIdx.x] = 0x7fffffff; hi[threadIdx.x] = (int)0x80000000; }
    __syncthreads();
    const int seg = blockIdx.y;
    const int64_t i0 = seg_off ? seg_off[seg] : 0, i1 = seg_off ? seg_off[seg + 1] : n;
    int l[3] = {0x7fffffff, 0x7fffffff, 0x7fffffff}, h[3] = {(int)0x80000000, (int)0x80000000, (int)0x80000000};
    bool finite = true;
    vx_stream_points(xyz, n, i0, i1, [&](int64_t, float x, float y, float z) {
        if (!(fabsf(x) <= 3.0e38f && fabsf(y) <= 3.0e38f && fabsf(z) <= 3.0e38f)) { finite = false; return; }
        const int q[3] = {vx_block_id(x, p), vx_block_id(y, p), vx_block_id(z, p)};
#pragma unroll
        for (int a = 0; a < 3; a++) { l[a] = q[a] < l[a] ? q[a] : l[a]; h[a] = q[a] > h[a] ? q[a] : h[a]; }
    });
    if (!finite) atomicOr(&st->overflow, 16u);
#pragma unroll
    for (int a = 0; a < 3; a++) { l[a] = vx_wave_min(l[a]); h[a] = vx_wave_max(h[a]); }
    if ((threadIdx.x & 63) == 0)
        for (int a = 0; a < 3; a++) { atomicMin(&lo[a], l[a]); atomicMax(&hi[a], h[a]); }
    __syncthreads();
    if (threadIdx.x < 3 && lo[threadIdx.x] <= hi[threadIdx.x]) { atomicMin(&st->lo[threadIdx.x], lo[threadIdx.x]); atomicMax(&st->hi[threadIdx.x], hi[threadIdx.x]); }
}

__device__ __forceinline__ bool vx_dims(const VxState* st, int* d) {
    int64_t total = 1;
    for (int a = 0; a < 3; a++) { d[a] = st->hi[a] - st->lo[a] + 1; if (d[a] < 1) return false; total *= d[a]; }
    return total <= st->table_cells;
}

#define VX_LDS_CELLS 2048
__global__ void __launch_bounds__(VX_BLOCK) k_vx_hist(const float* xyz, int64_t n, const int* seg_off, VxParams p, VxState* st,
                                                      int* table) {
    __shared__ int h[VX_LDS_CELLS];
    int d[3];
    if (st->overflow & 16u) return;
    if (!vx_dims(st, d)) { if (threadIdx.x == 0 && blockIdx.x == 0 && blockIdx.y == 0) atomicOr(&st->overflow, 1u); return; }
    const int ncell = d[0] * d[1] * d[2];
    const int seg = blockIdx.y;
    int* tab = table + (int64_t)seg * ncell;
    const int64_t i0 = seg_off ? seg_off[seg] : 0, i1 = seg_off ? seg_off[seg + 1] : n;
    const bool use_lds = ncell <= VX_LDS_CELLS;
    if (use_lds) for (int c = threadIdx.x; c < ncell; c += blockDim.x) h[c] = 0;
    __syncthreads();
    const int l0 = st->lo[0], l1 = st->lo[1], l2 = st->lo[2];
    vx_stream_points(xyz, n, i0, i1, [&](int64_t, float x, float y, float z) {
        const int c = ((vx_block_id(x, p) - l0) * d[1] + (vx_block_id(y, p) - l1)) * d[2] + (vx_block_id(z, p) - l2);
        if (use_lds) atomicAdd(&h[c], 1); else atomicAdd(&tab[c], 1);
    });
    __syncthreads();
    if (use_lds) for (int c = threadIdx.x; c < ncell; c += blockDim.x) if (h[c]) atomicAdd(&tab[c], h[c]);
}

__global__ void __launch_bounds__(VX_BLOCK) k_vx_blocks(VxState* st, int* table, VxParams p, float* centres, unsigned* blk_lo,
                                                        unsigned* blk_hi, int32_t* blk_seg) {
    __shared__ uint32_t lds[VX_BLOCK / 64 + 1];
    int d[3];
    if (!vx_dims(st, d)) return;
    const int ncell = d[0] * d[1] * d[2];
    const int64_t total_cells = (int64_t)ncell * p.nseg;
    uint32_t carry = 0;
    for (int64_t base = 0; base < total_cells; base += VX_BLOCK) {
        const int64_t g = base + threadIdx.x;
        const int seg = (int)(g / ncell), c = (int)(g % ncell);
        uint32_t keep = (g < total_cells && table[g] > p.min_points) ? 1u : 0u;
        uint32_t total;
        uint32_t rank = block_exclusive_scan(keep, lds, &total) + carry;
        if (g < total_cells) {
            if (c == 0) st->seg_blk_off[seg] = rank < (uint32_t)p.max_blocks ? rank : (uint32_t)p.max_blocks;
            if (keep && (int)rank < p.max_blocks) {
                table[g] = (int)rank;
                int cz = c % d[2], cy = (c / d[2]) % d[1], cx = c / (d[2] * d[1]);
                float id[3] = {(float)(cx + st->lo[0]), (float)(cy + st->lo[1]), (float)(cz + st->lo[2])};
                for (int a = 0; a < 3; a++) {
                    centres[3 * rank + a] = id[a] * p.bs + p.bs_half;
                    blk_lo[3 * rank + a] = 0xffffffffu;
                    blk_hi[3 * rank + a] = 0u;
                }
                if (blk_seg) blk_seg[rank] = seg;
            } else {
                table[g] = -1;
            }
        }
        carry += total;
    }
    if (threadIdx.x == 0) {
        st->n_blocks = carry;
        st->seg_blk_off[p.nseg] = carry < (uint32_t)p.max_blocks ? carry : (uint32_t)p.max_blocks;
        if ((int)carry > p.max_blocks) atomicOr(&st->overflow, 2u);
    }
}

template <class F>
__device__ __forceinline__ void vx_for_each_block(const float* pt, const VxState* st, const int* d, const int* table,
                                                  const VxParams& p, F fn) {
    if (p.whole) {
        if (table[0] >= 0) fn(table[0]);
        return;
    }
    int q[3];
    unsigned ok[3];
    for (int a = 0; a < 3; a++) {
        q[a] = vx_block_id(pt[a], p) - st->lo[a];
        ok[a] = 0;
        for (int o = -1; o <= 1; o++) {
            const int c = q[a] + o;
            if (c < 0 || c >= d[a]) continue;
            const float ctr = (float)(c + st->lo[a]) * p.bs + p.bs_half;
            if (pt[a] >= ctr - p.half_outer && pt[a] < ctr + p.half_outer) ok[a] |= 1u << (o + 1);
        }
    }
    if (!(ok[0] && ok[1] && ok[2])) return;
    if (__popc(ok[0]) <= 2 && __popc(ok[1]) <= 2 && __popc(ok[2]) <= 2) {
        int lo_opt[3], hi_opt[3];
        for (int a = 0; a < 3; a++) {
            lo_opt[a] = __ffs(ok[a]) - 2;
            const unsigned rest = ok[a] & (ok[a] - 1u);
            hi_opt[a] = rest ? __ffs(rest) - 2 : 2;
        }
        int blk[8];
#pragma unroll
        for (int j = 0; j < 8; j++) {
            const int ox = (j & 4) ? hi_opt[0] : lo_opt[0], oy = (j & 2) ? hi_opt[1] : lo_opt[1], oz = (j & 1) ? hi_opt[2] : lo_opt[2];
            blk[j] = (ox == 2 || oy == 2 || oz == 2) ? -1 : table[((q[0] + ox) * d[1] + (q[1] + oy)) * d[2] + (q[2] + oz)];
        }
#pragma unroll
        for (int j = 0; j < 8; j++)
            if (blk[j] >= 0) fn(blk[j]);
        return;
    }
    for (int dx = -1; dx <= 1; dx++) {
        if (!((ok[0] >> (dx + 1)) & 1u)) continue;
        for (int dy = -1; dy <= 1; dy++) {
            if (!((ok[1] >> (dy + 1)) & 1u)) continue;
            for (int dz = -1; dz <= 1; dz++) {
                if (!((ok[2] >> (dz + 1)) & 1u)) continue;
                const int b = table[((q[0] + dx) * d[1] + (q[1] + dy)) * d[2] + (q[2] + dz)];
                if (b >= 0) fn(b);
            }
        }
    }
}

__global__ void __launch_bounds__(VX_BLOCK) k_vx_minmax(const float* xyz, int64_t n, const int* seg_off, const VxState* st,
                                                        const int* table, VxParams p, unsigned* blk_lo, unsigned* blk_hi) {
    __shared__ unsigned slo[VX_LDS_BLOCKS * 3], shi[VX_LDS_BLOCKS * 3];
    int d[3];
    if ((st->overflow & 16u) || !vx_dims(st, d)) return;
    const int seg = blockIdx.y;
    const int* tab = table + (int64_t)seg * (d[0] * d[1] * d[2]);
    const int64_t i0 = seg_off ? seg_off[seg] : 0, i1 = seg_off ? seg_off[seg + 1] : n;
    const int b0 = (int)st->seg_blk_off[seg], nb = (int)st->seg_blk_off[seg + 1] - b0;
    const bool use_lds = nb <= VX_LDS_BLOCKS;
    if (use_lds)
        for (int i = threadIdx.x; i < nb * 3; i += blockDim.x) { slo[i] = 0xffffffffu; shi[i] = 0u; }
    __syncthreads();
    vx_stream_points(xyz, n, i0, i1, [&](int64_t, float x, float y, float z) {
        const float pt[3] = {x, y, z};
        vx_for_each_block(pt, st, d, tab, p, [&](int b) {
            for (int a = 0; a < 3; a++) {
                unsigned o = st_f2ord(pt[a]);
                if (use_lds) {
                    if (o < slo[3 * (b - b0) + a]) atomicMin(&slo[3 * (b - b0) + a], o);
                    if (o > shi[3 * (b - b0) + a]) atomicMax(&shi[3 * (b - b0) + a], o);
                } else {
                    atomicMin(&blk_lo[3 * b + a], o);
                    atomicMax(&blk_hi[3 * b + a], o);
                }
            }
        });
    });
    __syncthreads();
    if (use_lds)
        for (int i = threadIdx.x; i < nb * 3; i += blockDim.x) {
            if (slo[i] != 0xffffffffu) atomicMin(&blk_lo[3 * b0 + i], slo[i]);
            if (shi[i] != 0u) atomicMax(&blk_hi[3 * b0 + i], shi[i]);
        }
}

__global__ void __launch_bounds__(VX_BLOCK) k_vx_block_grid(VxState* st, int max_blocks, const unsigned* blk_lo,
                                                            const unsigned* blk_hi, float vs, float* blk_lof, int* blk_grid) {
    const int nb = (int)st_min<uint32_t>(st->n_blocks, (uint32_t)max_blocks);
    for (int i = blockIdx.x * blockDim.x + threadIdx.x; i < 3 * nb; i += gridDim.x * blockDim.x) {
        const float lo = st_ord2f(blk_lo[i]), hi = st_ord2f(blk_hi[i]);
        blk_lof[i] = lo;
        const float cells = roundf((hi - lo) / vs);
        if (!(cells <= 65535.0f)) atomicOr(&st->overflow, 8u);
        blk_grid[i] = cells <= 65535.0f ? (int)cells : 65535;
    }
}

__device__ __forceinline__ int vx_floor_div(float q, float v, float inv_v) {
    const float t = q * inv_v;
    const float f = floorf(t);
    const float frac = t - f, tol = fabsf(t) * 1e-6f + 1e-30f;
    if (frac < tol || 1.0f - frac < tol) return (int)floorf(q / v);
    return (int)f;
}

__device__ __forceinline__ bool vx_coord(const float* pt, int b, const float* blk_lof, const int* blk_grid, float vs, float inv_vs,
                                         int* c) {
    bool ok = true;
    for (int a = 0; a < 3; a++) {
        c[a] = vx_floor_div(pt[a] - blk_lof[3 * b + a], vs, inv_vs);
        ok = ok && c[a] >= 0 && c[a] < blk_grid[3 * b + a];
    }
    return ok;
}

struct __attribute__((aligned(16))) VxSlot {
    unsigned long long key;
    unsigned val;
    unsigned pad;
};
struct __attribute__((aligned(16))) VxRaw { unsigned long long x, y; };
__device__ __forceinline__ int vx_insert_min(VxSlot* slots, unsigned long long cap, unsigned long long key, unsigned val,
                                             const unsigned* give_up) {
    unsigned long long slot = st_hash_slot(key, cap);
    for (unsigned long long probe = 0; probe < cap && probe < ST_HASH_MAX_PROBE; probe++) {
        if ((probe & 63ull) == 63ull && (__hip_atomic_load(give_up, __ATOMIC_RELAXED, __HIP_MEMORY_SCOPE_AGENT) & 4u)) return 0;
        const VxRaw seen = *reinterpret_cast<const VxRaw*>(&slots[slot]);
        unsigned long long prev = seen.x;
        if (prev == ST_EMPTY_KEY) prev = atomicCAS(&slots[slot].key, (unsigned long long)ST_EMPTY_KEY, key);
        if (prev == ST_EMPTY_KEY || prev == key) {
            if (seen.x != key || (unsigned)(seen.y & 0xffffffffull) > val) { atomicMin(&slots[slot].val, val); return 2; }
            return 1;
        }
        slot = st_hash_next(slot, key, cap);
    }
    return 0;
}
__device__ __forceinline__ int vx_find(const VxSlot* slots, unsigned long long cap, unsigned long long key) {
    unsigned long long slot = st_hash_slot(key, cap);
    for (unsigned long long probe = 0; probe < cap && probe < ST_HASH_MAX_PROBE; probe++) {
        const VxRaw seen = *reinterpret_cast<const VxRaw*>(&slots[slot]);
        if (seen.x == key) return (int)(unsigned)(seen.y & 0xffffffffull);
        if (seen.x == ST_EMPTY_KEY) return -1;
        slot = st_hash_next(slot, key, cap);
    }
    return -1;
}

__global__ void __launch_bounds__(VX_BLOCK) k_vx_insert(const float* xyz, int64_t n, const int* seg_off, VxState* st,
                                                        const int* table, VxParams p, const float* blk_lof,
                                                        const int* blk_grid, VxSlot* slots, unsigned long long cap) {
    int d[3];
    if ((st->overflow & 16u) || !vx_dims(st, d)) return;
    const int seg = blockIdx.y;
    const int* tab = table + (int64_t)seg * (d[0] * d[1] * d[2]);
    const int64_t i0 = seg_off ? seg_off[seg] : 0, i1 = seg_off ? seg_off[seg + 1] : n;
    for (int64_t i = i0 + (int64_t)blockIdx.x * blockDim.x + threadIdx.x; i < i1; i += (int64_t)gridDim.x * blockDim.x) {
        const float pt[3] = {xyz[3 * i], xyz[3 * i + 1], xyz[3 * i + 2]};
        vx_for_each_block(pt, st, d, tab, p, [&](int b) {
            int c[3];
            if (!vx_coord(pt, b, blk_lof, blk_grid, p.vs, p.vs_inv, c)) return;
            if (vx_insert_min(slots, cap, st_pack_key(b, c[2], c[1], c[0]), (unsigned)i, &st->overflow) == 0) atomicOr(&st->overflow, 4u);
        });
    }
}

#define VX_EMIT_TILE 4096
__global__ void __launch_bounds__(VX_BLOCK) k_vx_emit(const VxSlot* __restrict__ slots, unsigned long long cap, VxState* st,
                                                      uint32_t* __restrict__ rec_b, uint32_t* __restrict__ rec_pt, int64_t max_voxels) {
    __shared__ uint32_t l_pt[VX_EMIT_TILE], l_b[VX_EMIT_TILE];
    __shared__ unsigned l_n, l_base;
    const int lane = threadIdx.x & 63;
    const unsigned long long ntile = (cap + VX_EMIT_TILE - 1) / VX_EMIT_TILE;
    for (unsigned long long tile = blockIdx.x; tile < ntile; tile += gridDim.x) {
        if (threadIdx.x == 0) l_n = 0u;
        __syncthreads();
#pragma unroll 4
        for (int k = 0; k < VX_EMIT_TILE / VX_BLOCK; k++) {
            const unsigned long long s = tile * VX_EMIT_TILE + (unsigned long long)k * VX_BLOCK + threadIdx.x;
            VxRaw seen = {ST_EMPTY_KEY, 0ull};
            if (s < cap) seen = *reinterpret_cast<const VxRaw*>(&slots[s]);
            const bool occ = seen.x != ST_EMPTY_KEY;
            const unsigned long long ob = __ballot(occ);
            if (ob == 0ull) continue;
            unsigned at = 0;
            if (lane == 0) at = atomicAdd(&l_n, (unsigned)__popcll(ob));
            at = __shfl(at, 0) + (unsigned)__popcll(ob & ((1ull << lane) - 1ull));
            if (occ) { l_pt[at] = (uint32_t)(seen.y & 0xffffffffull); l_b[at] = (uint32_t)(seen.x >> 48); }
        }
        __syncthreads();
        const unsigned cnt = l_n;
        if (threadIdx.x == 0 && cnt) l_base = atomicAdd(&st->n_vox, cnt);
        __syncthreads();
        for (unsigned i = threadIdx.x; i < cnt; i += VX_BLOCK)
            if ((int64_t)l_base + i < max_voxels) { rec_pt[l_base + i] = l_pt[i]; rec_b[l_base + i] = l_b[i]; }
        __syncthreads();
    }
}

__global__ void __launch_bounds__(VX_BLOCK) k_vx_iota(uint32_t* v, int64_t n) {
    for (int64_t i = (int64_t)blockIdx.x * blockDim.x + threadIdx.x; i < n; i += (int64_t)gridDim.x * blockDim.x)
        v[i] = (uint32_t)i;
}

__global__ void __launch_bounds__(VX_BLOCK) k_vx_gather(const float* xyz, const float* rgb, int64_t m, const uint32_t* sorted_b,
                                                        const uint32_t* order, const uint32_t* rec_pt, const float* centres,
                                                        VxParams p, const float* blk_lof, const int* blk_grid,
                                                        float* feats, int32_t* coords, uint8_t* mask, int64_t* point_index,
                                                        const int32_t* blk_seg, VxState* st) {
    for (int64_t j = (int64_t)blockIdx.x * blockDim.x + threadIdx.x; j < m; j += (int64_t)gridDim.x * blockDim.x) {
        int b = (int)sorted_b[j];
        int64_t i = order ? rec_pt[order[j]] : rec_pt[j];
        float pt[3] = {xyz[3 * i], xyz[3 * i + 1], xyz[3 * i + 2]};
        int c[3];
        vx_coord(pt, b, blk_lof, blk_grid, p.vs, p.vs_inv, c);
        bool inner = true;
        for (int a = 0; a < 3; a++) {
            float ctr = centres[3 * b + a];
            feats[6 * j + a] = pt[a];
            feats[6 * j + 3 + a] = rgb ? rgb[3 * i + a] : 0.0f;
            inner = inner && pt[a] >= ctr - p.half_inner && pt[a] < ctr + p.half_inner;
        }
        if (p.whole) inner = true;
        coords[4 * j] = b;
        coords[4 * j + 1] = c[2];
        coords[4 * j + 2] = c[1];
        coords[4 * j + 3] = c[0];
        mask[j] = inner ? 1 : 0;
        point_index[j] = i;
        if (blk_seg) {
            const int s = blk_seg[b], prev = j > 0 ? blk_seg[sorted_b[j - 1]] : -1;
            for (int t = prev + 1; t <= s; t++) st->seg_vox_off[t] = (uint32_t)j;
        }
    }
}
__global__ void k_vx_seg_vox_init(VxState* st, int nseg, const uint32_t* n_vox) {
    for (int t = threadIdx.x; t <= nseg; t += blockDim.x) st->seg_vox_off[t] = *n_vox;
}
__global__ void k_vx_seg_out(const VxState* st, int nseg, int32_t* seg_vox_off, int32_t* seg_blk_off) {
    for (int t = threadIdx.x; t <= nseg; t += blockDim.x) { seg_vox_off[t] = (int32_t)st->seg_vox_off[t]; seg_blk_off[t] = (int32_t)st->seg_blk_off[t]; }
}

static inline unsigned vx_grid(int64_t n) {
    int64_t g = st_div_up(n > 0 ? n : 1, VX_BLOCK);
    return (unsigned)(g < 4096 ? g : 4096);
}

static inline dim3 vx_grid_seg(int64_t n, int nseg, int64_t cap) {
    int64_t per = st_div_up(n > 0 ? n : 1, nseg);
    int64_t g = st_div_up(st_div_up(per, 4), VX_BLOCK) + 1;
    if (g > cap) g = cap;
    return dim3((unsigned)g, (unsigned)nseg);
}

static int64_t vx_layout(StArena& a, int64_t n, int max_blocks, int64_t max_voxels, int nseg, VxState** st, int** table,
                         unsigned** blk_lo, unsigned** blk_hi, float** blk_lof, int** blk_grid, VxSlot** slots, uint32_t** cnt, uint32_t** win,
                         uint32_t** rec_b, uint32_t** rec_pt, uint32_t** order, char** sub, int64_t* sub_bytes,
                         int64_t* cap, float** spare_centres = nullptr, int32_t** spare_i32 = nullptr) {
    *cap = st_next_pow2((max_voxels > 8 ? max_voxels : 8) + (max_voxels > 8 ? max_voxels : 8) / 2);
    *st = a.take<VxState>(1);
    *table = a.take<int>(vx_table_cells(max_blocks, nseg) * nseg);
    *blk_lo = a.take<unsigned>(3 * (int64_t)max_blocks);
    *blk_hi = a.take<unsigned>(3 * (int64_t)max_blocks);
    *blk_lof = a.take<float>(3 * (int64_t)max_blocks);
    *blk_grid = a.take<int>(3 * (int64_t)max_blocks);
    *slots = a.take<VxSlot>(*cap);
    *cnt = a.take<uint32_t>(n);
    *win = a.take<uint32_t>(n);
    *rec_b = a.take<uint32_t>(max_voxels);
    *rec_pt = a.take<uint32_t>(max_voxels);
    *order = a.take<uint32_t>(max_voxels);
    int64_t s1 = st_scan_ws_bytes(n), s2 = st_sort_ws_bytes(max_voxels);
    *sub_bytes = s1 > s2 ? s1 : s2;
    *sub = a.take<char>(*sub_bytes);
    float* sc = a.take<float>(3 * (int64_t)max_blocks);
    int32_t* si = a.take<int32_t>(max_blocks + 2 * ((int64_t)nseg + 1));
    if (spare_centres) *spare_centres = sc;
    if (spare_i32) *spare_i32 = si;
    return a.used;
}

extern "C" int64_t st_voxelize_workspace_bytes_seg(int64_t n_points, int max_blocks, int64_t max_voxels, int nseg) {
    StArena a(nullptr, 0);
    VxState* st; int* table; unsigned *lo, *hi; float* lof; int* grd; VxSlot* slots;
    uint32_t *cnt, *win, *rb, *rp, *ord; char* sub; int64_t sb, cap;
    return vx_layout(a, n_points, max_blocks, max_voxels, nseg < 1 ? 1 : nseg, &st, &table, &lo, &hi, &lof, &grd, &slots, &cnt,
                     &win, &rb, &rp, &ord, &sub, &sb, &cap);
}
extern "C" int64_t st_voxelize_workspace_bytes(int64_t n_points, int max_blocks, int64_t max_voxels) {
    return st_voxelize_workspace_bytes_seg(n_points, max_blocks, max_voxels, 1);
}

static int vx_voxelize(const float* xyz, const float* rgb, int64_t n, const int32_t* seg_off, int nseg, double voxel_size,
                       double block_size, double buffer_size, int min_points, int max_blocks, int64_t max_voxels, float* feats,
                       int32_t* coords, uint8_t* mask, int64_t* point_index, float* block_centres, int32_t* blk_seg,
                       int32_t* seg_vox_off, int32_t* seg_blk_off, int64_t* n_voxels_out, int64_t* n_blocks_out, void* ws,
                       int64_t ws_bytes, void* stream_, int whole) {
    hipStream_t stream = (hipStream_t)stream_;
    ST_REQUIRE(n >= 0 && n < (1ll << 31), "voxelize: n_points out of range");
    ST_REQUIRE(voxel_size > 0 && block_size > 0 && buffer_size >= 0 && buffer_size < block_size,
               "voxelize: need voxel_size > 0, 0 <= buffer_size < block_size");
    ST_REQUIRE(max_blocks > 0 && max_blocks < 65536 && max_voxels > 0, "voxelize: bad capacities");
    ST_REQUIRE(nseg >= 1 && nseg <= ST_MAX_SEG, "voxelize: 1 <= clouds per batch <= %d", ST_MAX_SEG);
    ST_REQUIRE(nseg == 1 || (seg_off && seg_vox_off && (whole || (blk_seg && seg_blk_off))), "voxelize: a batch needs seg_off and the per-cloud outputs");
    if (nseg == 1) seg_off = nullptr;
    *n_voxels_out = 0;
    *n_blocks_out = 0;
    if (n == 0) {
        if (seg_vox_off) (void)hipMemsetAsync(seg_vox_off, 0, (nseg + 1) * sizeof(int32_t), stream);
        if (seg_blk_off) (void)hipMemsetAsync(seg_blk_off, 0, (nseg + 1) * sizeof(int32_t), stream);
        return ST_OK;
    }

    StArena a(ws, ws_bytes);
    VxState* st; int* table; unsigned *blk_lo, *blk_hi; float* blk_lof; int* blk_grid; VxSlot* slots;
    uint32_t *cnt, *win, *rec_b, *rec_pt, *order; char* sub; int64_t sub_bytes, cap;
    float* spare_centres = nullptr; int32_t* spare_i32 = nullptr;
    vx_layout(a, n, max_blocks, max_voxels, nseg, &st, &table, &blk_lo, &blk_hi, &blk_lof, &blk_grid, &slots, &cnt, &win, &rec_b,
              &rec_pt, &order, &sub, &sub_bytes, &cap, &spare_centres, &spare_i32);
    if (!a.ok() || !sub || !spare_centres || !spare_i32) {
        st_set_error("voxelize: workspace too small (%lld < %lld)", (long long)ws_bytes, (long long)a.used);
        return ST_ERR_WORKSPACE;
    }
    if (!block_centres) block_centres = spare_centres;
    if (nseg > 1 && !blk_seg) blk_seg = spare_i32;
    if (nseg > 1 && !seg_blk_off) seg_blk_off = spare_i32 + max_blocks;
    VxParams p;
    p.whole = whole;
    p.bs = (float)block_size;
    {
        int e = 0;
        const float mant = frexpf(p.bs, &e);
        p.bs_inv = mant == 0.5f ? 1.0f / p.bs : 0.0f;
    }
    p.half_outer = (float)((block_size + buffer_size * 2) / 2);
    p.half_inner = (float)(block_size / 2);
    p.bs_half = (float)(block_size / 2);
    p.vs = (float)voxel_size;
    p.vs_inv = 1.0f / p.vs;
    p.min_points = min_points;
    p.max_blocks = max_blocks;
    p.nseg = nseg;

    const dim3 gr = vx_grid_seg(n, nseg, 512 / (nseg < 8 ? nseg : 8) + 8);
    hipLaunchKernelGGL(k_vx_init, dim3(1), dim3(64), 0, stream, st, (int)vx_table_cells(max_blocks, nseg));
    (void)hipMemsetAsync(table, 0, vx_table_cells(max_blocks, nseg) * nseg * sizeof(int), stream);
    (void)hipMemsetAsync(slots, 0xff, cap * sizeof(VxSlot), stream);
    hipLaunchKernelGGL(k_vx_bbox, gr, dim3(VX_BLOCK), 0, stream, xyz, n, seg_off, p, st);
    hipLaunchKernelGGL(k_vx_hist, gr, dim3(VX_BLOCK), 0, stream, xyz, n, seg_off, p, st, table);
    hipLaunchKernelGGL(k_vx_blocks, dim3(1), dim3(VX_BLOCK), 0, stream, st, table, p, block_centres, blk_lo, blk_hi, blk_seg);
    hipLaunchKernelGGL(k_vx_minmax, gr, dim3(VX_BLOCK), 0, stream, xyz, n, seg_off, (const VxState*)st, (const int*)table, p, blk_lo,
                       blk_hi);
    hipLaunchKernelGGL(k_vx_block_grid, dim3((unsigned)st_min64(st_div_up(3 * (int64_t)max_blocks, VX_BLOCK), 64)), dim3(VX_BLOCK), 0, stream,
                       st, max_blocks, (const unsigned*)blk_lo, (const unsigned*)blk_hi, p.vs, blk_lof, blk_grid);
    {
        const int64_t per = st_div_up(n > 0 ? n : 1, nseg);
        const dim3 gi((unsigned)st_min64(st_div_up(per, VX_BLOCK) + 1, 8192), (unsigned)nseg);
        hipLaunchKernelGGL(k_vx_insert, gi, dim3(VX_BLOCK), 0, stream, xyz, n, seg_off, st, (const int*)table, p, (const float*)blk_lof,
                           (const int*)blk_grid, slots, (unsigned long long)cap);
    }
    hipLaunchKernelGGL(k_vx_emit, dim3((unsigned)st_min64(st_div_up(cap, VX_EMIT_TILE), 4096)), dim3(VX_BLOCK), 0, stream,
                       (const VxSlot*)slots, (unsigned long long)cap, st, rec_b, rec_pt, max_voxels);
    if (nseg > 1) hipLaunchKernelGGL(k_vx_seg_vox_init, dim3(1), dim3(128), 0, stream, st, nseg, (const uint32_t*)&st->n_vox);
    ST_CHECK_LAUNCH();

    VxState h;
    (void)hipMemcpyAsync(&h, st, sizeof(VxState), hipMemcpyDeviceToHost, stream);
    st_stream_wait(stream);
    ST_CHECK_LAUNCH();
    ST_REQUIRE(!(h.overflow & 16u), "voxelize: the cloud holds non-finite coordinates (NaN or infinity)");
    ST_REQUIRE(!(h.overflow & 1u), "voxelize: the block-id bounding box of a cloud has more than %lld cells (raise max_blocks)",
               (long long)vx_table_cells(max_blocks, nseg));
    ST_REQUIRE(!(h.overflow & 2u), "voxelize: %u blocks exceed max_blocks=%d", h.n_blocks, max_blocks);
    ST_REQUIRE(!(h.overflow & 8u), "voxelize: a voxel grid spans more than 65535 cells along an axis (voxel size %g): use blocks, or a larger voxel", voxel_size);
    ST_REQUIRE(!(h.overflow & 4u) && (int64_t)h.n_vox <= max_voxels, "voxelize: %u voxels exceed max_voxels=%lld",
               h.n_vox, (long long)max_voxels);
    const int64_t m = h.n_vox;
    *n_voxels_out = m;
    *n_blocks_out = h.n_blocks;
    if (m > 0) {
        int bits = 1, pbits = 1;
        while ((1u << bits) < h.n_blocks) bits++;
        while ((1ll << pbits) < n) pbits++;
        ST_TRY(st_radix_sort_pairs_u32(rec_pt, rec_b, m, pbits, sub, sub_bytes, stream));
        ST_TRY(st_radix_sort_pairs_u32(rec_b, rec_pt, m, bits, sub, sub_bytes, stream));
        hipLaunchKernelGGL(k_vx_gather, dim3(vx_grid(m)), dim3(VX_BLOCK), 0, stream, xyz, rgb, m, (const uint32_t*)rec_b,
                           (const uint32_t*)nullptr, (const uint32_t*)rec_pt, (const float*)block_centres, p,
                           (const float*)blk_lof, (const int*)blk_grid, feats, coords, mask, point_index,
                           (const int32_t*)(nseg > 1 ? blk_seg : nullptr), st);
    }
    if (nseg > 1) hipLaunchKernelGGL(k_vx_seg_out, dim3(1), dim3(128), 0, stream, (const VxState*)st, nseg, seg_vox_off, seg_blk_off);
    ST_CHECK_LAUNCH();
    return ST_OK;
}

extern "C" int st_voxelize_blocks_seg(const float* xyz, const float* rgb, int64_t n, const int32_t* seg_off, int nseg,
                                      double voxel_size, double block_size, double buffer_size, int min_points, int max_blocks,
                                      int64_t max_voxels, float* feats, int32_t* coords, uint8_t* mask, int64_t* point_index,
                                      float* block_centres, int32_t* blk_seg, int32_t* seg_vox_off, int32_t* seg_blk_off,
                                      int64_t* n_voxels_out, int64_t* n_blocks_out, void* ws, int64_t ws_bytes, void* stream_) {
    ST_REQUIRE(block_centres != nullptr, "voxelize: block_centres is an output of the blocked call");
    ST_REQUIRE(nseg == 1 || (blk_seg && seg_blk_off), "voxelize: a batch needs the per-cloud block outputs");
    return vx_voxelize(xyz, rgb, n, seg_off, nseg, voxel_size, block_size, buffer_size, min_points, max_blocks, max_voxels, feats,
                       coords, mask, point_index, block_centres, blk_seg, seg_vox_off, seg_blk_off, n_voxels_out, n_blocks_out, ws,
                       ws_bytes, stream_, 0);
}

extern "C" int64_t st_voxelize_cloud_workspace_bytes(int64_t n_points, int64_t max_voxels, int nseg) {
    return st_voxelize_workspace_bytes_seg(n_points, nseg < 1 ? 1 : nseg, max_voxels, nseg);
}
extern "C" int st_voxelize_cloud_seg(const float* xyz, const float* rgb, int64_t n, const int32_t* seg_off, int nseg,
                                     double voxel_size, int64_t max_voxels, float* feats, int32_t* coords, uint8_t* mask,
                                     int64_t* point_index, int32_t* seg_vox_off, int64_t* n_voxels_out, void* ws, int64_t ws_bytes,
                                     void* stream_) {
    int64_t n_blocks = 0;
    return vx_voxelize(xyz, rgb, n, seg_off, nseg, voxel_size, 1.0, 0.0, -1, nseg < 1 ? 1 : nseg, max_voxels, feats, coords, mask,
                       point_index, nullptr, nullptr, seg_vox_off, nullptr, n_voxels_out, &n_blocks, ws, ws_bytes, stream_, 1);
}

extern "C" int st_voxelize_blocks(const float* xyz, const float* rgb, int64_t n, double voxel_size, double block_size,
                                  double buffer_size, int min_points, int max_blocks, int64_t max_voxels, float* feats,
                                  int32_t* coords, uint8_t* mask, int64_t* point_index, float* block_centres,
                                  int64_t* n_voxels_out, int64_t* n_blocks_out, void* ws, int64_t ws_bytes,
                                  void* stream_) {
    return st_voxelize_blocks_seg(xyz, rgb, n, nullptr, 1, voxel_size, block_size, buffer_size, min_points, max_blocks, max_voxels,
                                  feats, coords, mask, point_index, block_centres, nullptr, nullptr, nullptr, n_voxels_out,
                                  n_blocks_out, ws, ws_bytes, stream_);
}
```

### smart_tree_amd/data_types/cloud.py

```python
from __future__ import annotations

from dataclasses import dataclass, fields, replace
from pathlib import Path
from typing import Optional

import numpy as np
import torch
import torch.nn.functional as F

_PER_POINT = ("xyz", "rgb", "medial_vector", "branch_direction", "branch_ids", "class_l")

_CLASS_LISTS: dict = {}


def _class_tensor(classes, device) -> torch.Tensor:
    if torch.is_tensor(classes):
        return classes.to(device)
    key = (tuple(int(c) for c in classes), str(device))
    t = _CLASS_LISTS.get(key)
    if t is None:
        t = _CLASS_LISTS[key] = torch.as_tensor(list(key[0]), device=device)
    return t


@dataclass
class Cloud:
    xyz: torch.Tensor
    rgb: Optional[torch.Tensor] = None
    medial_vector: Optional[torch.Tensor] = None
    branch_direction: Optional[torch.Tensor] = None
    branch_ids: Optional[torch.Tensor] = None
    class_l: Optional[torch.Tensor] = None
    filename: Optional[Path] = None
    seg_off: Optional[torch.Tensor] = None

    def __post_init__(self):
        n = self.xyz.shape[0]
        if self.xyz.ndim != 2 or self.xyz.shape[1] != 3:
            raise TypeError(f"xyz must be [N,3], got {tuple(self.xyz.shape)}")
        for name, width in (("rgb", 3), ("medial_vector", 3), ("branch_direction", 3), ("branch_ids", 1), ("class_l", 1)):
            t = getattr(self, name)
            if t is not None and tuple(t.shape) != (n, width):
                raise TypeError(f"{name} must be [{n},{width}], got {tuple(t.shape)}")

    def __len__(self) -> int:
        return self.xyz.shape[0]

    def __str__(self) -> str:
        return (f"Cloud with {len(self)} points, min {self.min_xyz.tolist()}, "
                f"max {self.max_xyz.tolist()}, device {self.xyz.device}")

    def _map(self, fn) -> "Cloud":
        changed = {name: fn(getattr(self, name)) for name in _PER_POINT if getattr(self, name) is not None}
        return replace(self, **changed)

    def filter(self, mask, assume_sorted: bool = False) -> "Cloud":
        mask = mask.to(self.xyz.device)
        if mask.dtype == torch.bool:
            mask = mask.nonzero().view(-1)
        elif self.seg_off is not None and not assume_sorted and mask.numel() > 1 and not bool((mask[1:] > mask[:-1]).all()):
            raise ValueError("Cloud.filter: a batch of clouds (seg_off) needs a boolean mask or a strictly increasing index; "
                             "split() the batch before reordering / resampling its points")
        out = self._map(lambda t: t.index_select(0, mask))
        if self.seg_off is not None:
            out.seg_off = torch.searchsorted(mask, self.seg_off.to(mask.dtype)).to(torch.int32)
        return out

    @property
    def n_seg(self) -> int:
        return 1 if self.seg_off is None else int(self.seg_off.shape[0]) - 1

    @staticmethod
    def collate(clouds) -> "Cloud":
        clouds = list(clouds)
        dev = clouds[0].xyz.device
        sizes = [0] + [len(c) for c in clouds]
        kw = {}
        for name in _PER_POINT:
            parts = [getattr(c, name) for c in clouds]
            if all(p is not None for p in parts):
                kw[name] = torch.cat(parts)
        off = torch.tensor(sizes, dtype=torch.int64).cumsum(0).to(torch.int32)
        return Cloud(seg_off=off.to(dev, non_blocking=True), **kw)

    def split(self):
        if self.seg_off is None:
            return [self]
        off = self.seg_off.tolist()
        out = []
        for a, b in zip(off[:-1], off[1:]):
            out.append(Cloud(**{name: getattr(self, name)[a:b] for name in _PER_POINT if getattr(self, name) is not None}))
        return out

    def filter_by_class(self, classes) -> "Cloud":
        wanted = _class_tensor(classes, self.class_l.device)
        return self.filter(torch.isin(self.class_l, wanted).view(-1))

    def to_device(self, device) -> "Cloud":
        out = self._map(lambda t: t.to(device))
        if self.seg_off is not None:
            out.seg_off = self.seg_off.to(device)
        return out

    def cpu(self) -> "Cloud":
        return self.to_device(torch.device("cpu"))

    def pin_memory(self) -> "Cloud":
        return self._map(lambda t: t.pin_memory())

    def cat(self) -> torch.Tensor:
        return torch.cat((self.xyz, self.rgb), 1)

    def voxel_down_sample(self, voxel_size) -> "Cloud":
        q = torch.div(self.xyz, voxel_size, rounding_mode="floor")
        _, inverse, counts = torch.unique(q, dim=0, sorted=True, return_inverse=True, return_counts=True)
        _, by_voxel = torch.sort(inverse, stable=True)
        starts = counts.cumsum(0)[:-1]
        return self.filter(by_voxel[starts])

    def scale(self, factor) -> "Cloud":
        return Cloud(self.xyz * factor, self.rgb, seg_off=self.seg_off)

    def translate(self, offset) -> "Cloud":
        return Cloud(self.xyz + offset.to(self.xyz.device), self.rgb, seg_off=self.seg_off)

    def rotate(self, rot_mat) -> "Cloud":
        rot_mat = rot_mat.to(device=self.xyz.device, dtype=self.xyz.dtype)
        return Cloud(self.xyz @ rot_mat, self.rgb, seg_off=self.seg_off)

    @property
    def max_xyz(self) -> torch.Tensor:
        return self.xyz.max(0)[0]

    @property
    def min_xyz(self) -> torch.Tensor:
        return self.xyz.min(0)[0]

    @property
    def bbox(self):
        half = (self.max_xyz - self.min_xyz) / 2
        return self.min_xyz + half, half

    @property
    def root_idx(self) -> int:
        return int(torch.argmin(self.xyz[:, 1]).item())

    @property
    def number_classes(self) -> int:
        return 1 if self.class_l is None else int(self.class_l.max().item()) + 1

    @property
    def medial_pts(self) -> torch.Tensor:
        return self.xyz + self.medial_vector

    @property
    def radius(self) -> torch.Tensor:
        v = self.medial_vector
        return ((v[:, 0] * v[:, 0] + v[:, 1] * v[:, 1]) + v[:, 2] * v[:, 2]).sqrt()

    @property
    def direction(self) -> torch.Tensor:
        return F.normalize(self.medial_vector)

    @staticmethod
    def from_numpy(**arrays) -> "Cloud":
        known = {f.name for f in fields(Cloud)} - {"filename"}
        kw = {}
        for key, value in arrays.items():
            if key in known:
                kw[key] = torch.as_tensor(np.asarray(value)).float()
            elif key == "vector":
                kw["medial_vector"] = torch.as_tensor(np.asarray(value))
        return Cloud(**kw)


def _same_device(a: torch.device, b) -> bool:
    b = torch.device(b)
    return a.type == b.type and (b.index is None or a.index is None or a.index == b.index)


class MaskedCloud(Cloud):

    def __init__(self, base: Cloud, mask: torch.Tensor):
        assert mask.dtype == torch.bool and mask.shape[0] == len(base)
        self.__dict__.update(_base=base, _mask=mask.to(base.xyz.device), _real=None)

    def _cloud(self) -> Cloud:
        if self.__dict__["_real"] is None:
            self.__dict__["_real"] = self.__dict__["_base"].filter(self.__dict__["_mask"])
        return self.__dict__["_real"]

    def filter_by_class(self, classes) -> Cloud:
        base, mask = self.__dict__["_base"], self.__dict__["_mask"]
        if self.__dict__["_real"] is not None or base.class_l is None:
            return self._cloud().filter_by_class(classes)
        wanted = _class_tensor(classes, base.class_l.device)
        return MaskedCloud(base, mask & torch.isin(base.class_l, wanted).view(-1))

    def pending(self):
        return None if self.__dict__["_real"] is not None else (self.__dict__["_base"], self.__dict__["_mask"])

    def _map(self, fn) -> Cloud:
        return self._cloud()._map(fn)

    def to_device(self, device) -> Cloud:
        if self.__dict__["_real"] is None and _same_device(self.__dict__["_base"].xyz.device, device):
            return self
        return self._cloud().to_device(device)

    def __repr__(self):
        return f"MaskedCloud({self._cloud()!r})"


for _name in [f.name for f in fields(Cloud)]:
    setattr(MaskedCloud, _name, property(lambda self, _name=_name: getattr(self._cloud(), _name)))
del _name
```

### smart_tree_amd/dataset/augmentations.py

```python
from __future__ import annotations

from abc import ABC, abstractmethod
from typing import Sequence

import torch

from .. import _lib
from ..data_types.cloud import Cloud


class Augmentation(ABC):
    @abstractmethod
    def __call__(self, cloud: Cloud) -> Cloud:
        ...


class CentreCloud(Augmentation):

    def __call__(self, cloud: Cloud) -> Cloud:
        if cloud.xyz.is_cuda or _lib._ALLOW_HOST_POINTERS:
            L = _lib.lib()
            xyz = cloud.xyz.contiguous().float()
            out = torch.empty_like(xyz)
            nseg = cloud.n_seg
            ws = _lib.workspace(256 + 24 * nseg, xyz.device)
            _lib.check(L.st_centre_cloud_seg(_lib.ptr(xyz), xyz.shape[0], _lib.ptr(cloud.seg_off), nseg, _lib.ptr(out), _lib.ptr(ws),
                                             ws.numel(), _lib.stream(xyz.device)))
            return Cloud(out, cloud.rgb, seg_off=cloud.seg_off)
        if cloud.seg_off is not None:
            raise _lib.StError("batched clouds are centred on the GPU only")
        centre, half = cloud.bbox
        lift = torch.zeros(3, device=centre.device, dtype=centre.dtype)
        lift[1] = half[1]
        return cloud.translate(-centre + lift)


class Scale(Augmentation):

    def __init__(self, min_scale=0.9, max_scale=1.1):
        self.min_scale, self.max_scale = min_scale, max_scale

    def __call__(self, cloud: Cloud) -> Cloud:
        t = torch.rand(1, device=cloud.xyz.device) * (self.max_scale - self.min_scale)
        return cloud.scale(t + self.min_scale)


def euler_angles_to_rotation(xyz: torch.Tensor) -> torch.Tensor:
    x, y, z = (torch.as_tensor(a, dtype=torch.float32).cpu() for a in xyz)
    cx, sx, cy, sy, cz, sz = torch.cos(x), torch.sin(x), torch.cos(y), torch.sin(y), torch.cos(z), torch.sin(z)
    rx = torch.tensor([[1.0, 0.0, 0.0], [0.0, cx, -sx], [0.0, sx, cx]])
    ry = torch.tensor([[cy, 0.0, sy], [0.0, 1.0, 0.0], [-sy, 0.0, cy]])
    rz = torch.tensor([[cz, -sz, 0.0], [sz, cz, 0.0], [0.0, 0.0, 1.0]])
    return rz @ (ry @ rx)


class FixedRotate(Augmentation):

    def __init__(self, xyz):
        self.xyz = xyz

    def __call__(self, cloud: Cloud) -> Cloud:
        self.rot_mat = euler_angles_to_rotation(torch.tensor(self.xyz)).float()
        return cloud.rotate(self.rot_mat)


class VoxelDownsample(Augmentation):

    def __init__(self, voxel_size):
        self.voxel_size = voxel_size

    def __call__(self, cloud: Cloud) -> Cloud:
        return cloud.voxel_down_sample(self.voxel_size)


class FixedTranslate(Augmentation):

    def __init__(self, xyz):
        self.xyz = torch.tensor(xyz)

    def __call__(self, cloud: Cloud) -> Cloud:
        return cloud.translate(self.xyz)


class RandomCrop(Augmentation):

    def __init__(self, max_x, max_y, max_z):
        self.max_translation = torch.tensor([max_x, max_y, max_z])

    def __call__(self, cloud: Cloud) -> Cloud:
        dev = cloud.xyz.device
        offset = (torch.rand(3, device=dev) - 0.5) * self.max_translation.to(device=dev)
        p = cloud.xyz + offset
        return cloud.filter(torch.logical_and(p >= cloud.min_xyz, p <= cloud.max_xyz).all(dim=1))


class RandomCubicCrop(Augmentation):

    def __init__(self, size):
        self.size = size

    def __call__(self, cloud: Cloud) -> Cloud:
        centre = cloud.xyz[torch.randint(0, cloud.xyz.shape[0], (1,))]
        lo, hi = centre - self.size / 2, centre + self.size / 2
        return cloud.filter(torch.logical_and(cloud.xyz >= lo, cloud.xyz <= hi).all(dim=1))


class RandomDropout(Augmentation):

    def __init__(self, max_drop_out):
        self.max_drop_out = max_drop_out

    def __call__(self, cloud: Cloud) -> Cloud:
        dev = cloud.xyz.device
        n = int((1.0 - (self.max_drop_out * torch.rand(1, device=dev))) * cloud.xyz.shape[0])
        return cloud.filter(torch.randint(high=cloud.xyz.shape[0], size=(n, 1), device=dev).squeeze(1))


class AugmentationPipeline(Augmentation):
    def __init__(self, augmentations: Sequence[Augmentation]):
        self.augmentations = list(augmentations)

    def __call__(self, cloud: Cloud) -> Cloud:
        for aug in self.augmentations:
            cloud = aug(cloud)
        return cloud
```

### smart_tree_amd/dataset/dataset.py

```python
from __future__ import annotations

import ctypes
from dataclasses import dataclass
from typing import Optional

import torch

from .. import _lib
from ..data_types.cloud import Cloud


_VOXELS_PER_POINT = {}


@dataclass
class VoxelBatch:
    feats: torch.Tensor
    coords: torch.Tensor
    mask: torch.Tensor
    point_index: torch.Tensor
    block_centres: torch.Tensor
    blk_seg: Optional[torch.Tensor] = None
    seg_vox_off: Optional[torch.Tensor] = None
    seg_blk_off: Optional[torch.Tensor] = None
    n_seg: int = 1


def voxelize_blocks(xyz: torch.Tensor, rgb: Optional[torch.Tensor], voxel_size: float, block_size: float = 4,
                    buffer_size: float = 0.4, min_points: int = 20, max_blocks: int = 4096,
                    seg_off: Optional[torch.Tensor] = None) -> VoxelBatch:
    L = _lib.lib()
    dev = xyz.device
    xyz = xyz.contiguous().float()
    rgb = rgb.contiguous().float() if rgb is not None else None
    n = xyz.shape[0]
    nseg = 1 if seg_off is None else int(seg_off.shape[0]) - 1
    return _voxelize_blocks(xyz, rgb, n, nseg, seg_off, voxel_size, block_size, buffer_size, min_points, max_blocks)


def _voxelize_blocks(xyz, rgb, n, nseg, seg_off, voxel_size, block_size, buffer_size, min_points, max_blocks):
    L = _lib.lib()
    dev = xyz.device
    per_cloud_blocks = max_blocks
    max_blocks = min(max_blocks * nseg, 65535)
    n_vox, n_blk = ctypes.c_int64(0), ctypes.c_int64(0)
    i32 = lambda k: torch.empty((k,), dtype=torch.int32, device=dev)
    blk_seg, seg_vox, seg_blk = (i32(max_blocks), i32(nseg + 1), i32(nseg + 1)) if nseg > 1 else (None, None, None)
    key = (float(voxel_size), float(block_size), float(buffer_size))
    worst = (8 if 2 * buffer_size < block_size else 27) * n + 1024
    guess = int(n * 1.5 * _VOXELS_PER_POINT.get(key, 1.0 / 3.0)) + 4096
    for cap in sorted({min(guess, worst), min(3 * n + 1024, worst), worst}):
        feats = torch.empty((cap, 6), dtype=torch.float32, device=dev)
        coords = torch.empty((cap, 4), dtype=torch.int32, device=dev)
        mask = torch.empty((cap,), dtype=torch.uint8, device=dev)
        pidx = torch.empty((cap,), dtype=torch.int64, device=dev)
        centres = torch.empty((max_blocks, 3), dtype=torch.float32, device=dev)
        ws = _lib.workspace(L.st_voxelize_workspace_bytes_seg(n, max_blocks, cap, nseg), dev)
        rc = L.st_voxelize_blocks_seg(_lib.ptr(xyz), _lib.ptr(rgb), n, _lib.ptr(seg_off), nseg, float(voxel_size),
                                      float(block_size), float(buffer_size), int(min_points), int(max_blocks), cap,
                                      _lib.ptr(feats), _lib.ptr(coords), _lib.ptr(mask), _lib.ptr(pidx), _lib.ptr(centres),
                                      _lib.ptr(blk_seg), _lib.ptr(seg_vox), _lib.ptr(seg_blk), ctypes.byref(n_vox),
                                      ctypes.byref(n_blk), _lib.ptr(ws), ws.numel(), _lib.stream(dev))
        if rc == 0 or b"exceed max_voxels" not in L.st_last_error():
            break
    if rc != 0 and (b"bounding box of a cloud has more than" in L.st_last_error() or b"exceed max_blocks" in L.st_last_error()) \
            and per_cloud_blocks * nseg < 65535:
        return _voxelize_blocks(xyz, rgb, n, nseg, seg_off, voxel_size, block_size, buffer_size, min_points,
                                min(per_cloud_blocks * 8, 65535))
    _lib.check(rc)
    m, b = n_vox.value, n_blk.value
    if n > 0:
        _VOXELS_PER_POINT[key] = max(m / n, 1e-3)
    return VoxelBatch(feats[:m], coords[:m], mask[:m].bool(), pidx[:m], centres[:b],
                      blk_seg[:b] if blk_seg is not None else None, seg_vox, seg_blk, nseg)


def voxelize_cloud(xyz: torch.Tensor, rgb: Optional[torch.Tensor], voxel_size: float,
                   seg_off: Optional[torch.Tensor] = None) -> VoxelBatch:
    L = _lib.lib()
    dev = xyz.device
    xyz = xyz.contiguous().float()
    rgb = rgb.contiguous().float() if rgb is not None else None
    n = xyz.shape[0]
    nseg = 1 if seg_off is None else int(seg_off.shape[0]) - 1
    cap = n + 8
    feats = torch.empty((cap, 6), dtype=torch.float32, device=dev)
    coords = torch.empty((cap, 4), dtype=torch.int32, device=dev)
    mask = torch.empty((cap,), dtype=torch.uint8, device=dev)
    pidx = torch.empty((cap,), dtype=torch.int64, device=dev)
    seg_vox = torch.empty((nseg + 1,), dtype=torch.int32, device=dev) if nseg > 1 else None
    n_vox = ctypes.c_int64(0)
    ws = _lib.workspace(L.st_voxelize_cloud_workspace_bytes(n, cap, nseg), dev)
    _lib.check(L.st_voxelize_cloud_seg(_lib.ptr(xyz), _lib.ptr(rgb), n, _lib.ptr(seg_off), nseg, float(voxel_size), cap,
                                       _lib.ptr(feats), _lib.ptr(coords), _lib.ptr(mask), _lib.ptr(pidx), _lib.ptr(seg_vox),
                                       ctypes.byref(n_vox), _lib.ptr(ws), ws.numel(), _lib.stream(dev)))
    m = n_vox.value
    return VoxelBatch(feats[:m], coords[:m], mask[:m].bool(), pidx[:m], torch.zeros((nseg, 3), dtype=torch.float32, device=dev),
                      None, seg_vox, None, nseg)


def at_least_2d(t: torch.Tensor) -> torch.Tensor:
    return t.unsqueeze(1) if t.dim() == 1 else t


class TreeDataset:

    def __init__(self, voxel_size, json_path, directory, mode: str, input_features, target_features, augmentation=None,
                 cache: bool = False, device=None):
        import json
        from pathlib import Path

        self.voxel_size = voxel_size
        self.mode = mode
        self.augmentation = augmentation
        self.directory = directory
        self.device = device if device is not None else torch.device("cuda:0")
        self.input_features = list(input_features)
        self.target_features = list(target_features)
        if not Path(json_path).is_file():
            raise AssertionError(f"json metadata does not exist at '{json_path}'")
        if mode not in ("train", "validation", "test"):
            raise ValueError(f"TreeDataset: mode must be train / validation / test, got {mode!r}")
        with open(json_path) as f:
            self.tree_paths = json.load(f)[mode]
        missing = [p for p in self.tree_paths if not Path(f"{self.directory}/{p}").is_file()]
        if missing:
            raise AssertionError(f"Missing {len(missing)} files: {missing}")
        self.cache = {} if cache else None

    def load(self, filename) -> Cloud:
        from ..util.file import load_cloud

        if self.cache is None:
            return load_cloud(filename)
        if filename not in self.cache:
            cld = load_cloud(filename)
            self.cache[filename] = cld.pin_memory() if torch.cuda.is_available() else cld
        return self.cache[filename]

    def __getitem__(self, idx):
        from pathlib import Path

        return self.process_cloud(self.load(Path(f"{self.directory}/{self.tree_paths[idx]}")), self.tree_paths[idx])

    def process_cloud(self, cld: Cloud, filename):
        cld = cld.to_device(self.device)
        if self.augmentation is not None:
            cld = self.augmentation(cld)
        inputs = torch.cat([at_least_2d(getattr(cld, a)) for a in self.input_features], dim=1)
        targets = torch.cat([at_least_2d(getattr(cld, a)) for a in self.target_features], dim=1)
        if inputs.shape[0] == 0:
            raise AssertionError(f"Empty cloud after augmentation: {filename}")
        vb = voxelize_cloud(cld.xyz, None, self.voxel_size)
        rep = vb.point_index
        loss_mask = torch.ones(rep.shape[0], dtype=torch.bool, device=rep.device)
        return (inputs.index_select(0, rep), targets.float().index_select(0, rep)), vb.coords, loss_mask, filename

    def __len__(self) -> int:
        return len(self.tree_paths)


class SingleTreeInference:

    def __init__(self, cloud: Cloud, voxel_size: float, block_size: float = 4, buffer_size: float = 0.4,
                 min_points: int = 20, file_name=None, device=None):
        self.cloud = cloud
        self.voxel_size = voxel_size
        self.block_size = block_size
        self.buffer_size = buffer_size
        self.min_points = min_points
        self.file_name = file_name
        self.batch = voxelize_blocks(cloud.xyz, cloud.rgb, voxel_size, block_size, buffer_size, min_points,
                                     seg_off=cloud.seg_off)
        self.block_centres = self.batch.block_centres

    def __len__(self) -> int:
        return self.block_centres.shape[0]

    def __getitem__(self, idx):
        sel = self.batch.coords[:, 0] == idx
        coords = self.batch.coords[sel].clone()
        coords[:, 0] = 0
        return self.batch.feats[sel], coords, self.batch.mask[sel], self.file_name


def load_dataloader(cloud: Cloud, voxel_size: float, block_size: float, buffer_size: float, num_workers: float,
                    batch_size: float):
    ds = SingleTreeInference(cloud, voxel_size, block_size, buffer_size)
    b = ds.batch
    return [(b.feats, b.coords, b.mask, ds.file_name)]
```

### smart_tree_amd/model/model_inference.py

```python
from __future__ import annotations

from pathlib import Path

import numpy as np
import torch

from .. import profiling
from ..data_types.cloud import Cloud, MaskedCloud
from ..dataset.dataset import SingleTreeInference, voxelize_cloud
from .model import Smart_Tree
from .sparse import sparse_from_batch

_WEIGHTS_DIR = Path(__file__).resolve().parent / "weights"


def _load_state_dict(weights_path):
    p = Path(str(weights_path))
    if not p.exists():
        bundled = _WEIGHTS_DIR / (p.name.replace("_model_weights.pt", "").replace("_model.pt", "").replace(".npz", "") + ".npz")
        if not bundled.exists():
            raise FileNotFoundError(f"weights not found: {weights_path}")
        p = bundled
    if p.suffix == ".npz":
        with np.load(p) as z:
            return {k: torch.from_numpy(z[k]) for k in z.files}
    return torch.load(str(p), map_location="cpu", weights_only=True)


def load_model(model_path, weights_path, device=torch.device("cuda:0"), fp16: bool = False):
    return Smart_Tree(_load_state_dict(weights_path), device=device, fp16=fp16).eval()


class ModelInference:
    def __init__(self, model_path, weights_path, voxel_size: float, block_size: float, buffer_size: float,
                 num_workers=8, batch_size=4, device=torch.device("cuda:0"), verbose=False, fp16: bool = False,
                 blocking: str = "blocks"):
        if blocking not in ("blocks", "whole"):
            raise ValueError(f"ModelInference: blocking must be 'blocks' or 'whole', got {blocking!r}")
        self.blocking = blocking
        self.device = torch.device(device)
        self.verbose = verbose
        self.voxel_size = voxel_size
        self.block_size = block_size
        self.buffer_size = buffer_size
        self.num_workers = num_workers
        self.batch_size = batch_size
        self.model = load_model(model_path, weights_path, self.device, fp16=fp16)
        self.on_network_done = None
        self.last_point_index = None
        if self.verbose:
            print("Model Loaded Succesfully")

    def forward(self, cloud: Cloud, return_masked: bool = True) -> Cloud:
        cloud = cloud.to_device(self.device)
        if cloud.rgb is None:
            cloud = Cloud(cloud.xyz, torch.zeros_like(cloud.xyz), seg_off=cloud.seg_off)
        with profiling.stage("voxelize"):
            if self.blocking == "whole":
                vb = voxelize_cloud(cloud.xyz, cloud.rgb, self.voxel_size, seg_off=cloud.seg_off)
                if vb.n_seg > 1:
                    vb.blk_seg = torch.arange(vb.n_seg, dtype=torch.int32, device=self.device)
            else:
                vb = SingleTreeInference(cloud, self.voxel_size, self.block_size, self.buffer_size).batch
        hint = None
        if self.blocking == "blocks" and vb.block_centres.shape[0] > 0:
            hint = (int(vb.block_centres.shape[0]), int(round((self.block_size + 2 * self.buffer_size) / self.voxel_size)) + 2)
        sparse_input = sparse_from_batch(vb.feats[:, :3].contiguous(), vb.coords, device=self.device, blk_seg=vb.blk_seg,
                                         n_seg=vb.n_seg, brick_hint=hint)
        with profiling.stage("unet"):
            _, _, _, mv, cls = self.model.forward_fused_tail(sparse_input)
        masks = vb.mask
        self.last_point_index = vb.point_index
        lc = Cloud(xyz=sparse_input.features, rgb=vb.feats[:, 3:6].contiguous(), medial_vector=mv, class_l=cls,
                   seg_off=vb.seg_vox_off)
        if self.on_network_done is not None:
            self.on_network_done()
        return MaskedCloud(lc, masks) if return_masked else lc

    @staticmethod
    def from_cfg(cfg):
        return ModelInference(model_path=cfg.model_path, weights_path=cfg.weights_path, voxel_size=cfg.voxel_size,
                              block_size=cfg.block_size, buffer_size=cfg.buffer_size, num_workers=cfg.num_workers,
                              batch_size=cfg.batch_size, blocking=getattr(cfg, "blocking", "blocks"))
```

Measured before the change: 906.3 million.

## Reuse centring bounding box in voxelizer and pack kNN indices to int32

The centring kernel now writes the per-cloud bounding box of the centred points, and the blocked voxelizer seeds its block-id extents from that box during init, so it no longer needs its own bounds pass. The minmax kernel gains a shared-memory zone path for small block grids. Separately, the kNN CSR build packs int64 neighbour indices into int32 so the mutual-neighbour check reads half the bytes with vector loads. The cost is an extra pack kernel, more workspace, and extra float-equivalence assumptions on the box.

```diff
diff --git a/include/smarttree_hip.h b/include/smarttree_hip.h
--- a/include/smarttree_hip.h
+++ b/include/smarttree_hip.h
@@ -120,6 +120,14 @@
 
 int st_centre_cloud_seg(const float* xyz, int64_t n, const int32_t* seg_off, int nseg, float* out, void* ws,
                         int64_t ws_bytes , void* stream);
+int st_centre_cloud_box_seg(const float* xyz, int64_t n, const int32_t* seg_off, int nseg, float* out, void* ws,
+                            int64_t ws_bytes , void* stream, float* box_out);
+int st_voxelize_blocks_box_seg(const float* xyz, const float* rgb, int64_t n, const int32_t* seg_off, int nseg,
+                               double voxel_size, double block_size, double buffer_size, int min_points, int max_blocks,
+                               int64_t max_voxels, float* feats, int32_t* coords, uint8_t* mask, int64_t* point_index,
+                               float* block_centres, int32_t* blk_seg, int32_t* seg_vox_off, int32_t* seg_blk_off,
+                               int64_t* n_voxels_host, int64_t* n_blocks_host, void* ws, int64_t ws_bytes, void* stream,
+                               const float* centred_box );
 int64_t st_voxelize_workspace_bytes_seg(int64_t n_points, int max_blocks, int64_t max_voxels, int nseg);
 int st_voxelize_blocks_seg(const float* xyz, const float* rgb, int64_t n, const int32_t* seg_off, int nseg,
                            double voxel_size, double block_size, double buffer_size, int min_points, int max_blocks,
diff --git a/smart_tree_amd/_lib.py b/smart_tree_amd/_lib.py
--- a/smart_tree_amd/_lib.py
+++ b/smart_tree_amd/_lib.py
@@ -63,6 +63,9 @@
     "st_post_process": (c_int, [c_int, P, P, P, P, P, P, P, P, P, P, P, c_int, c_float, c_float, c_int, c_int, c_int, P]),
     "st_skeleton_workspace_bytes": (I64, [I64, I64]),
     "st_centre_cloud_seg": (c_int, [P, I64, P, c_int, P, P, I64, P]),
+    "st_centre_cloud_box_seg": (c_int, [P, I64, P, c_int, P, P, I64, P, P]),
+    "st_voxelize_blocks_box_seg": (c_int, [P, P, I64, P, c_int, c_double, c_double, c_double, c_int, c_int, I64, P, P, P, P, P, P, P, P,
+                                           ctypes.POINTER(I64), ctypes.POINTER(I64), P, I64, P, P]),
     "st_voxelize_workspace_bytes_seg": (I64, [I64, c_int, I64, c_int]),
     "st_voxelize_blocks_seg": (c_int, [P, P, I64, P, c_int, c_double, c_double, c_double, c_int, c_int, I64, P, P, P, P, P, P, P, P,
                                        ctypes.POINTER(I64), ctypes.POINTER(I64), P, I64, P]),
@@ -111,7 +114,7 @@
     "st_build_coord_hash", "st_build_subm_rulebook", "st_build_strided_rulebook", "st_sparse_conv_fwd",
     "st_sparse_conv_mfma_fwd", "st_sparse_conv_b3_fwd", "st_sparse_conv_f16_fwd", "st_pointwise_mlp_heads", "st_medial_points", "st_centre_cloud",
     "st_connected_components", "st_component_csr", "st_post_process", "st_knn_radius", "st_brick_pyramid_workspace_bytes",
-    "st_centre_cloud_seg", "st_voxelize_workspace_bytes_seg", "st_build_strided_rulebook_seg", "st_knn_workspace_bytes_seg",
+    "st_centre_cloud_seg", "st_centre_cloud_box_seg", "st_voxelize_workspace_bytes_seg", "st_build_strided_rulebook_seg", "st_knn_workspace_bytes_seg",
     "st_knn_radius_seg", "st_skeleton_workspace_bytes_seg", "st_post_process_seg", "st_radius_count_seg",
     "st_voxelize_cloud_workspace_bytes", "st_loss_workspace_bytes", "st_spatial_order_workspace_bytes", "st_spatial_order", "st_connected_components_knn", "st_component_csr_knn", "st_component_csr_knn_workspace_bytes", "st_move_rows",
     "st_loss_backward", "st_sparse_conv_wgrad_workspace_bytes", "st_sparse_conv_wgrad",
diff --git a/smart_tree_amd/csrc/graph.hip b/smart_tree_amd/csrc/graph.hip
--- a/smart_tree_amd/csrc/graph.hip
+++ b/smart_tree_amd/csrc/graph.hip
@@ -81,7 +81,8 @@
     __syncthreads();
     if (threadIdx.x < 3 && r.i1 > r.i0) { atomicMin(&box[6 * seg + threadIdx.x], lo[threadIdx.x]); atomicMax(&box[6 * seg + 3 + threadIdx.x], hi[threadIdx.x]); }
 }
-__global__ void __launch_bounds__(GR_BLOCK) k_centre(const float* xyz, int64_t n, const unsigned* box, float* out, const int* seg_off) {
+__global__ void __launch_bounds__(GR_BLOCK) k_centre(const float* xyz, int64_t n, const unsigned* box, float* out, const int* seg_off,
+                                                     float* box_out) {
     const int seg = blockIdx.y;
     const GrRange r = gr_range(xyz, out, n, seg_off, seg);
     float shift[3];
@@ -90,6 +91,10 @@
         const float half = (mx - mn) / 2.0f;
         const float centre = mn + half;
         shift[a] = -centre + (a == 1 ? half : 0.0f);
+        if (box_out && blockIdx.x == 0 && threadIdx.x == 0) {
+            box_out[6 * seg + a] = r.i1 > r.i0 ? mn + shift[a] : INFINITY;
+            box_out[6 * seg + 3 + a] = r.i1 > r.i0 ? mx + shift[a] : -INFINITY;
+        }
     }
     const float4* v = reinterpret_cast<const float4*>(xyz + 3 * r.a0);
     float4* o = reinterpret_cast<float4*>(out + 3 * r.a0);
@@ -113,10 +118,13 @@
     for (int i = threadIdx.x; i < 6 * nseg; i += blockDim.x) box[i] = i % 6 < 3 ? 0xffffffffu : 0u;
 }
 
-extern "C" int st_centre_cloud_seg(const float* xyz, int64_t n, const int32_t* seg_off, int nseg, float* out, void* ws,
-                                   int64_t ws_bytes, void* stream_) {
+extern "C" int st_centre_cloud_box_seg(const float* xyz, int64_t n, const int32_t* seg_off, int nseg, float* out, void* ws,
+                                       int64_t ws_bytes, void* stream_, float* box_out) {
     hipStream_t stream = (hipStream_t)stream_;
-    if (n <= 0) return ST_OK;
+    if (n <= 0) {
+        ST_REQUIRE(!box_out, "centre_cloud: no box of an empty array");
+        return ST_OK;
+    }
     ST_REQUIRE(nseg >= 1 && nseg <= ST_MAX_SEG && (nseg == 1 || seg_off), "centre_cloud: 1 <= clouds per batch <= %d", ST_MAX_SEG);
     if (nseg == 1) seg_off = nullptr;
     StArena a(ws, ws_bytes);
@@ -127,9 +135,13 @@
     const unsigned gx = (unsigned)st_min64(st_div_up(per > 0 ? per : 1, GR_BLOCK), 2048 / (nseg < 8 ? nseg : 8) + 1);
     hipLaunchKernelGGL(k_bbox, dim3(gx, (unsigned)nseg), dim3(GR_BLOCK), 0, stream, xyz, n, box, seg_off);
     hipLaunchKernelGGL(k_centre, dim3((unsigned)st_min64(st_div_up(per > 0 ? per : 1, GR_BLOCK), 8192), (unsigned)nseg), dim3(GR_BLOCK), 0, stream,
-                       xyz, n, (const unsigned*)box, out, seg_off);
+                       xyz, n, (const unsigned*)box, out, seg_off, box_out);
     ST_CHECK_LAUNCH();
     return ST_OK;
+}
+extern "C" int st_centre_cloud_seg(const float* xyz, int64_t n, const int32_t* seg_off, int nseg, float* out, void* ws,
+                                   int64_t ws_bytes, void* stream_) {
+    return st_centre_cloud_box_seg(xyz, n, seg_off, nseg, out, ws, ws_bytes, stream_, nullptr);
 }
 extern "C" int st_centre_cloud(const float* xyz, int64_t n, float* out, void* ws, int64_t ws_bytes, void* stream_) {
     return st_centre_cloud_seg(xyz, n, nullptr, 1, out, ws, ws_bytes, stream_);
@@ -535,10 +547,14 @@
 
 #define CSRK_MUTUAL 0x40000000
 struct __attribute__((aligned(16))) GrI64x2 { int64_t x, y; };
-template <int K>
-__global__ void __launch_bounds__(GR_BLOCK) k_csrk_count(const int64_t* __restrict__ idx, int64_t n, const int* __restrict__ first_of,
-                                                         const int* __restrict__ new_id, uint32_t* deg, uint32_t* fwdc,
-                                                         int32_t* __restrict__ tgt) {
+struct __attribute__((aligned(16))) GrI32x4 { int32_t x, y, z, w; };
+__global__ void __launch_bounds__(GR_BLOCK) k_csrk_pack(const int64_t* __restrict__ idx, int64_t E, int32_t* __restrict__ idx32) {
+    GR_LOOP(e, E) idx32[e] = (int32_t)idx[e];
+}
+template <int K, bool PACKED>
+__global__ void __launch_bounds__(GR_BLOCK) k_csrk_count(const int64_t* __restrict__ idx, const int32_t* __restrict__ idx32, int64_t n,
+                                                         const int* __restrict__ first_of, const int* __restrict__ new_id, uint32_t* deg,
+                                                         uint32_t* fwdc, int32_t* __restrict__ tgt) {
     const int64_t E = n * K;
     const int lane = threadIdx.x & 63;
     for (int64_t base = (int64_t)blockIdx.x * blockDim.x + (threadIdx.x - lane); base < E; base += (int64_t)gridDim.x * blockDim.x) {
@@ -548,12 +564,22 @@
         bool mutual = false;
         if (e < E) {
             x = new_id[i];
-            const int64_t j = idx[e], first = first_of ? first_of[i] : 0;
+            const int64_t j = PACKED ? (int64_t)idx32[e] : idx[e], first = first_of ? first_of[i] : 0;
             if (x >= 0 && j > first && j != i) {
                 y = new_id[j];
                 if (y >= 0 && i > first) {
                     const int64_t* row = idx + j * K;
-                    if (K % 2 == 0) {
+                    if (PACKED && K % 4 == 0) {
+                        const int32_t* row32 = idx32 + j * K;
+                        const int32_t i32 = (int32_t)i;
+#pragma unroll
+                        for (int k = 0; k < K; k += 4) {
+                            const GrI32x4 r = *reinterpret_cast<const GrI32x4*>(row32 + k);
+                            mutual = mutual || r.x == i32 || r.y == i32 || r.z == i32 || r.w == i32;
+                        }
+                    } else if (PACKED) {
+                        for (int k = 0; k < K; k++) mutual = mutual || (int64_t)idx32[j * K + k] == i;
+                    } else if (K % 2 == 0) {
 #pragma unroll
                         for (int k = 0; k < K; k += 2) {
                             const GrI64x2 r = *reinterpret_cast<const GrI64x2*>(row + k);
@@ -617,6 +643,7 @@
     a.take<char>(st_scan_ws_bytes(m + 1));
     a.take<uint32_t>(m + 1);
     a.take<int32_t>(n * (int64_t)(K > 0 ? K : 1));
+    a.take<int32_t>(n * (int64_t)(K > 0 ? K : 1));
     return a.used;
 }
 
@@ -631,11 +658,18 @@
 
 template <int K>
 static void csrk_launch(const int64_t* idx, const float* dist, int64_t n, const int32_t* first_of, const int32_t* new_id, int64_t m,
-                        uint32_t* row_off, uint32_t* col, float* wgt, uint32_t* cursor, uint32_t* fwdc, int32_t* tgt, char* sw, int64_t sb,
-                        hipStream_t stream, int* rc) {
+                        uint32_t* row_off, uint32_t* col, float* wgt, uint32_t* cursor, uint32_t* fwdc, int32_t* tgt, int32_t* idx32,
+                        char* sw, int64_t sb, hipStream_t stream, int* rc) {
     const int64_t E = n * K;
     (void)hipMemsetAsync(row_off, 0, (m + 1) * sizeof(uint32_t), stream);
-    hipLaunchKernelGGL((k_csrk_count<K>), dim3(gr_grid(E)), dim3(GR_BLOCK), 0, stream, idx, n, first_of, new_id, row_off, fwdc, tgt);
+    if (idx32) {
+        hipLaunchKernelGGL(k_csrk_pack, dim3(gr_grid(E)), dim3(GR_BLOCK), 0, stream, idx, E, idx32);
+        hipLaunchKernelGGL((k_csrk_count<K, true>), dim3(gr_grid(E)), dim3(GR_BLOCK), 0, stream, idx, (const int32_t*)idx32, n, first_of,
+                           new_id, row_off, fwdc, tgt);
+    } else {
+        hipLaunchKernelGGL((k_csrk_count<K, false>), dim3(gr_grid(E)), dim3(GR_BLOCK), 0, stream, idx, (const int32_t*)nullptr, n, first_of,
+                           new_id, row_off, fwdc, tgt);
+    }
     *rc = st_exclusive_scan_u32(row_off, row_off, m + 1, nullptr, sw, sb, stream);
     if (*rc != ST_OK) return;
     hipLaunchKernelGGL(k_csrk_cursor, dim3(gr_grid(m)), dim3(GR_BLOCK), 0, stream, (const uint32_t*)row_off, (const uint32_t*)fwdc, m, cursor);
@@ -655,9 +689,11 @@
         char* sw = a.take<char>(sb);
         uint32_t* fwdc = a.take<uint32_t>(m + 1);
         int32_t* tgt = a.take<int32_t>(n * (int64_t)K);
-        if (!cursor || !sw || !fwdc || !tgt) { st_set_error("component_csr(knn): workspace too small"); return ST_ERR_WORKSPACE; }
+        int32_t* idx32 = a.take<int32_t>(n * (int64_t)K);
+        if (!cursor || !sw || !fwdc || !tgt || !idx32) { st_set_error("component_csr(knn): workspace too small"); return ST_ERR_WORKSPACE; }
+        if (n >= (1ll << 31)) idx32 = nullptr;
         int rc = ST_OK;
-#define CSRK_CASE(K_) case K_: csrk_launch<K_>(idx, dist, n, first_of, new_id, m, row_off, col, wgt, cursor, fwdc, tgt, sw, sb, stream, &rc); break;
+#define CSRK_CASE(K_) case K_: csrk_launch<K_>(idx, dist, n, first_of, new_id, m, row_off, col, wgt, cursor, fwdc, tgt, idx32, sw, sb, stream, &rc); break;
         switch (K) { CSRK_CASE(1) CSRK_CASE(2) CSRK_CASE(4) CSRK_CASE(8) CSRK_CASE(16) CSRK_CASE(32) CSRK_CASE(64) }
 #undef CSRK_CASE
         if (rc != ST_OK) return rc;
diff --git a/smart_tree_amd/csrc/prims.hip b/smart_tree_amd/csrc/prims.hip
--- a/smart_tree_amd/csrc/prims.hip
+++ b/smart_tree_amd/csrc/prims.hip
@@ -14,7 +14,7 @@
 extern "C" const char* st_last_error(void) { return g_err; }
 void st_stream_wait(hipStream_t stream) { (void)hipStreamSynchronize(stream); }
 
-extern "C" int st_version(void) { return 104; }
+extern "C" int st_version(void) { return 105; }
 
 #define SCAN_BLOCK 256
 #define SCAN_ITEMS 16
diff --git a/smart_tree_amd/csrc/voxelize.hip b/smart_tree_amd/csrc/voxelize.hip
--- a/smart_tree_amd/csrc/voxelize.hip
+++ b/smart_tree_amd/csrc/voxelize.hip
@@ -61,11 +61,23 @@
     }
 }
 
-__global__ void k_vx_init(VxState* st, int table_cells) {
+__global__ void k_vx_init(VxState* st, int table_cells, const float* box, VxParams p) {
     if (threadIdx.x == 0 && blockIdx.x == 0) {
         st->table_cells = table_cells;
         for (int a = 0; a < 3; a++) { st->lo[a] = 0x7fffffff; st->hi[a] = (int)0x80000000; }
         st->n_blocks = 0; st->n_vox = 0; st->overflow = 0;
+        for (int s = 0; box && s < p.nseg; s++) {
+            const float* b = box + 6 * s;
+            if (b[0] > b[3]) continue;
+            bool finite = true;
+            for (int j = 0; j < 6; j++) finite = finite && fabsf(b[j]) <= 3.0e38f;
+            if (!finite) { st->overflow |= 16u; continue; }
+            for (int a = 0; a < 3; a++) {
+                const int l = vx_block_id(b[a], p), h = vx_block_id(b[3 + a], p);
+                st->lo[a] = l < st->lo[a] ? l : st->lo[a];
+                st->hi[a] = h > st->hi[a] ? h : st->hi[a];
+            }
+        }
     }
 }
 
@@ -125,7 +137,7 @@
 }
 
 __global__ void __launch_bounds__(VX_BLOCK) k_vx_blocks(VxState* st, int* table, VxParams p, float* centres, unsigned* blk_lo,
-                                                        unsigned* blk_hi, int32_t* blk_seg) {
+                                                        unsigned* blk_hi, int32_t* blk_seg, int* blk_cell) {
     __shared__ uint32_t lds[VX_BLOCK / 64 + 1];
     int d[3];
     if (!vx_dims(st, d)) return;
@@ -150,6 +162,7 @@
                     blk_hi[3 * rank + a] = 0u;
                 }
                 if (blk_seg) blk_seg[rank] = seg;
+                blk_cell[rank] = (int)g;
             } else {
                 table[g] = -1;
             }
@@ -161,6 +174,18 @@
         st->seg_blk_off[p.nseg] = carry < (uint32_t)p.max_blocks ? carry : (uint32_t)p.max_blocks;
         if ((int)carry > p.max_blocks) atomicOr(&st->overflow, 2u);
     }
+}
+
+__device__ __forceinline__ unsigned vx_axis_cols(float v, int lo, int dim, const VxParams& p, int* q) {
+    *q = vx_block_id(v, p) - lo;
+    unsigned ok = 0;
+    for (int o = -1; o <= 1; o++) {
+        const int c = *q + o;
+        if (c < 0 || c >= dim) continue;
+        const float ctr = (float)(c + lo) * p.bs + p.bs_half;
+        if (v >= ctr - p.half_outer && v < ctr + p.half_outer) ok |= 1u << (o + 1);
+    }
+    return ok;
 }
 
 template <class F>
@@ -172,16 +197,7 @@
     }
     int q[3];
     unsigned ok[3];
-    for (int a = 0; a < 3; a++) {
-        q[a] = vx_block_id(pt[a], p) - st->lo[a];
-        ok[a] = 0;
-        for (int o = -1; o <= 1; o++) {
-            const int c = q[a] + o;
-            if (c < 0 || c >= d[a]) continue;
-            const float ctr = (float)(c + st->lo[a]) * p.bs + p.bs_half;
-            if (pt[a] >= ctr - p.half_outer && pt[a] < ctr + p.half_outer) ok[a] |= 1u << (o + 1);
-        }
-    }
+    for (int a = 0; a < 3; a++) ok[a] = vx_axis_cols(pt[a], st->lo[a], d[a], p, &q[a]);
     if (!(ok[0] && ok[1] && ok[2])) return;
     if (__popc(ok[0]) <= 2 && __popc(ok[1]) <= 2 && __popc(ok[2]) <= 2) {
         int lo_opt[3], hi_opt[3];
@@ -214,14 +230,69 @@
     }
 }
 
+#define VX_ZONE_MAX 1024
+__device__ __forceinline__ bool vx_zone_dims(const int* d, const VxParams& p, int* z) {
+    if (p.whole) return false;
+    int64_t total = 1;
+    for (int a = 0; a < 3; a++) { z[a] = 2 * d[a] - 1; total *= z[a]; }
+    return total <= VX_ZONE_MAX;
+}
 __global__ void __launch_bounds__(VX_BLOCK) k_vx_minmax(const float* xyz, int64_t n, const int* seg_off, const VxState* st,
-                                                        const int* table, VxParams p, unsigned* blk_lo, unsigned* blk_hi) {
-    __shared__ unsigned slo[VX_LDS_BLOCKS * 3], shi[VX_LDS_BLOCKS * 3];
-    int d[3];
+                                                        const int* table, VxParams p, unsigned* blk_lo, unsigned* blk_hi,
+                                                        unsigned* zone) {
+    __shared__ __attribute__((aligned(8))) unsigned lds[VX_ZONE_MAX * 6];
+    int d[3], zd[3];
     if ((st->overflow & 16u) || !vx_dims(st, d)) return;
     const int seg = blockIdx.y;
     const int* tab = table + (int64_t)seg * (d[0] * d[1] * d[2]);
     const int64_t i0 = seg_off ? seg_off[seg] : 0, i1 = seg_off ? seg_off[seg + 1] : n;
+    if (vx_zone_dims(d, p, zd)) {
+        const int ncell = zd[0] * zd[1] * zd[2];
+        for (int i = threadIdx.x; i < ncell * 6; i += blockDim.x) lds[i] = 0u;
+        __syncthreads();
+        const int l0 = st->lo[0], l1 = st->lo[1], l2 = st->lo[2];
+        vx_stream_points(xyz, n, i0, i1, [&](int64_t, float x, float y, float z) {
+            const float pt[3] = {x, y, z};
+            const int lo[3] = {l0, l1, l2};
+            int zc[3];
+            bool plain = true;
+            for (int a = 0; a < 3; a++) {
+                int q;
+                const unsigned ok = vx_axis_cols(pt[a], lo[a], d[a], p, &q);
+                if (ok == 0u) return;
+                zc[a] = 2 * (q + __ffs(ok) - 2) + (ok == 3u || ok == 6u ? 1 : 0);
+                plain = plain && (ok == 1u || ok == 2u || ok == 4u || ok == 3u || ok == 6u);
+            }
+            const unsigned ox = st_f2ord(x), oy = st_f2ord(y), oz = st_f2ord(z);
+            if (!plain) {
+                vx_for_each_block(pt, st, d, tab, p, [&](int b) {
+                    atomicMin(&blk_lo[3 * b], ox); atomicMin(&blk_lo[3 * b + 1], oy); atomicMin(&blk_lo[3 * b + 2], oz);
+                    atomicMax(&blk_hi[3 * b], ox); atomicMax(&blk_hi[3 * b + 1], oy); atomicMax(&blk_hi[3 * b + 2], oz);
+                });
+                return;
+            }
+            unsigned* cell = &lds[6 * ((zc[0] * zd[1] + zc[1]) * zd[2] + zc[2])];
+            const uint2* c2 = reinterpret_cast<const uint2*>(cell);
+            const uint2 a0 = c2[0], a1 = c2[1], a2 = c2[2];
+            const unsigned v[6] = {~ox, ~oy, ~oz, ox, oy, oz}, have[6] = {a0.x, a0.y, a1.x, a1.y, a2.x, a2.y};
+            bool moves = false;
+#pragma unroll
+            for (int k = 0; k < 6; k++) moves = moves || v[k] > have[k];
+            if (moves) {
+#pragma unroll
+                for (int k = 0; k < 6; k++)
+                    if (v[k] > have[k]) atomicMax(&cell[k], v[k]);
+            }
+        });
+        __syncthreads();
+        unsigned* out = zone + (int64_t)seg * (VX_ZONE_MAX * 6);
+        for (int i = threadIdx.x; i < ncell * 6; i += blockDim.x) {
+            const unsigned v = lds[i];
+            if (v != 0u && v > __hip_atomic_load(&out[i], __ATOMIC_RELAXED, __HIP_MEMORY_SCOPE_AGENT)) atomicMax(&out[i], v);
+        }
+        return;
+    }
+    unsigned *slo = lds, *shi = lds + VX_LDS_BLOCKS * 3;
     const int b0 = (int)st->seg_blk_off[seg], nb = (int)st->seg_blk_off[seg + 1] - b0;
     const bool use_lds = nb <= VX_LDS_BLOCKS;
     if (use_lds)
@@ -250,10 +321,30 @@
         }
 }
 
-__global__ void __launch_bounds__(VX_BLOCK) k_vx_block_grid(VxState* st, int max_blocks, const unsigned* blk_lo,
-                                                            const unsigned* blk_hi, float vs, float* blk_lof, int* blk_grid) {
+__global__ void __launch_bounds__(VX_BLOCK) k_vx_block_grid(VxState* st, int max_blocks, unsigned* blk_lo, unsigned* blk_hi,
+                                                            VxParams p, float* blk_lof, int* blk_grid, const int* blk_cell,
+                                                            const unsigned* zone) {
+    const float vs = p.vs;
     const int nb = (int)st_min<uint32_t>(st->n_blocks, (uint32_t)max_blocks);
+    int d[3], zd[3];
+    const bool zones = !(st->overflow & 16u) && vx_dims(st, d) && vx_zone_dims(d, p, zd);
     for (int i = blockIdx.x * blockDim.x + threadIdx.x; i < 3 * nb; i += gridDim.x * blockDim.x) {
+        if (zones) {
+            const int b = i / 3, a = i % 3, ncell = d[0] * d[1] * d[2];
+            const int g = blk_cell[b], seg = g / ncell, c = g % ncell;
+            const int cc[3] = {c / (d[2] * d[1]), (c / d[2]) % d[1], c % d[2]};
+            const unsigned* zs = zone + (int64_t)seg * (VX_ZONE_MAX * 6);
+            unsigned nlo = ~blk_lo[i], hi = blk_hi[i];
+            for (int zx = st_max(2 * cc[0] - 1, 0); zx <= st_min(2 * cc[0] + 1, zd[0] - 1); zx++)
+                for (int zy = st_max(2 * cc[1] - 1, 0); zy <= st_min(2 * cc[1] + 1, zd[1] - 1); zy++)
+                    for (int zz = st_max(2 * cc[2] - 1, 0); zz <= st_min(2 * cc[2] + 1, zd[2] - 1); zz++) {
+                        const unsigned* cell = zs + 6 * ((zx * zd[1] + zy) * zd[2] + zz);
+                        nlo = st_max(nlo, cell[a]);
+                        hi = st_max(hi, cell[3 + a]);
+                    }
+            blk_lo[i] = ~nlo;
+            blk_hi[i] = hi;
+        }
         const float lo = st_ord2f(blk_lo[i]), hi = st_ord2f(blk_hi[i]);
         blk_lof[i] = lo;
         const float cells = roundf((hi - lo) / vs);
@@ -422,10 +513,15 @@
 static int64_t vx_layout(StArena& a, int64_t n, int max_blocks, int64_t max_voxels, int nseg, VxState** st, int** table,
                          unsigned** blk_lo, unsigned** blk_hi, float** blk_lof, int** blk_grid, VxSlot** slots, uint32_t** cnt, uint32_t** win,
                          uint32_t** rec_b, uint32_t** rec_pt, uint32_t** order, char** sub, int64_t* sub_bytes,
-                         int64_t* cap, float** spare_centres = nullptr, int32_t** spare_i32 = nullptr) {
+                         int64_t* cap, float** spare_centres = nullptr, int32_t** spare_i32 = nullptr, unsigned** zone = nullptr,
+                         int** blk_cell = nullptr) {
     *cap = st_next_pow2((max_voxels > 8 ? max_voxels : 8) + (max_voxels > 8 ? max_voxels : 8) / 2);
     *st = a.take<VxState>(1);
     *table = a.take<int>(vx_table_cells(max_blocks, nseg) * nseg);
+    unsigned* zn = a.take<unsigned>(6ll * VX_ZONE_MAX * nseg);
+    int* bc = a.take<int>(max_blocks);
+    if (zone) *zone = zn;
+    if (blk_cell) *blk_cell = bc;
     *blk_lo = a.take<unsigned>(3 * (int64_t)max_blocks);
     *blk_hi = a.take<unsigned>(3 * (int64_t)max_blocks);
     *blk_lof = a.take<float>(3 * (int64_t)max_blocks);
@@ -461,7 +557,7 @@
                        double block_size, double buffer_size, int min_points, int max_blocks, int64_t max_voxels, float* feats,
                        int32_t* coords, uint8_t* mask, int64_t* point_index, float* block_centres, int32_t* blk_seg,
                        int32_t* seg_vox_off, int32_t* seg_blk_off, int64_t* n_voxels_out, int64_t* n_blocks_out, void* ws,
-                       int64_t ws_bytes, void* stream_, int whole) {
+                       int64_t ws_bytes, void* stream_, int whole, const float* centred_box = nullptr) {
     hipStream_t stream = (hipStream_t)stream_;
     ST_REQUIRE(n >= 0 && n < (1ll << 31), "voxelize: n_points out of range");
     ST_REQUIRE(voxel_size > 0 && block_size > 0 && buffer_size >= 0 && buffer_size < block_size,
@@ -481,10 +577,10 @@
     StArena a(ws, ws_bytes);
     VxState* st; int* table; unsigned *blk_lo, *blk_hi; float* blk_lof; int* blk_grid; VxSlot* slots;
     uint32_t *cnt, *win, *rec_b, *rec_pt, *order; char* sub; int64_t sub_bytes, cap;
-    float* spare_centres = nullptr; int32_t* spare_i32 = nullptr;
+    float* spare_centres = nullptr; int32_t* spare_i32 = nullptr; unsigned* zone = nullptr; int* blk_cell = nullptr;
     vx_layout(a, n, max_blocks, max_voxels, nseg, &st, &table, &blk_lo, &blk_hi, &blk_lof, &blk_grid, &slots, &cnt, &win, &rec_b,
-              &rec_pt, &order, &sub, &sub_bytes, &cap, &spare_centres, &spare_i32);
-    if (!a.ok() || !sub || !spare_centres || !spare_i32) {
+              &rec_pt, &order, &sub, &sub_bytes, &cap, &spare_centres, &spare_i32, &zone, &blk_cell);
+    if (!a.ok() || !sub || !spare_centres || !spare_i32 || !zone || !blk_cell) {
         st_set_error("voxelize: workspace too small (%lld < %lld)", (long long)ws_bytes, (long long)a.used);
         return ST_ERR_WORKSPACE;
     }
@@ -509,16 +605,17 @@
     p.nseg = nseg;
 
     const dim3 gr = vx_grid_seg(n, nseg, 512 / (nseg < 8 ? nseg : 8) + 8);
-    hipLaunchKernelGGL(k_vx_init, dim3(1), dim3(64), 0, stream, st, (int)vx_table_cells(max_blocks, nseg));
-    (void)hipMemsetAsync(table, 0, vx_table_cells(max_blocks, nseg) * nseg * sizeof(int), stream);
+    if (whole) centred_box = nullptr;
+    hipLaunchKernelGGL(k_vx_init, dim3(1), dim3(64), 0, stream, st, (int)vx_table_cells(max_blocks, nseg), centred_box, p);
+    (void)hipMemsetAsync(table, 0, (size_t)((char*)(zone + 6ll * VX_ZONE_MAX * nseg) - (char*)table), stream);
     (void)hipMemsetAsync(slots, 0xff, cap * sizeof(VxSlot), stream);
-    hipLaunchKernelGGL(k_vx_bbox, gr, dim3(VX_BLOCK), 0, stream, xyz, n, seg_off, p, st);
+    if (!centred_box) hipLaunchKernelGGL(k_vx_bbox, gr, dim3(VX_BLOCK), 0, stream, xyz, n, seg_off, p, st);
     hipLaunchKernelGGL(k_vx_hist, gr, dim3(VX_BLOCK), 0, stream, xyz, n, seg_off, p, st, table);
-    hipLaunchKernelGGL(k_vx_blocks, dim3(1), dim3(VX_BLOCK), 0, stream, st, table, p, block_centres, blk_lo, blk_hi, blk_seg);
+    hipLaunchKernelGGL(k_vx_blocks, dim3(1), dim3(VX_BLOCK), 0, stream, st, table, p, block_centres, blk_lo, blk_hi, blk_seg, blk_cell);
     hipLaunchKernelGGL(k_vx_minmax, gr, dim3(VX_BLOCK), 0, stream, xyz, n, seg_off, (const VxState*)st, (const int*)table, p, blk_lo,
-                       blk_hi);
+                       blk_hi, zone);
     hipLaunchKernelGGL(k_vx_block_grid, dim3((unsigned)st_min64(st_div_up(3 * (int64_t)max_blocks, VX_BLOCK), 64)), dim3(VX_BLOCK), 0, stream,
-                       st, max_blocks, (const unsigned*)blk_lo, (const unsigned*)blk_hi, p.vs, blk_lof, blk_grid);
+                       st, max_blocks, blk_lo, blk_hi, p, blk_lof, blk_grid, (const int*)blk_cell, (const unsigned*)zone);
     {
         const int64_t per = st_div_up(n > 0 ? n : 1, nseg);
         const dim3 gi((unsigned)st_min64(st_div_up(per, VX_BLOCK) + 1, 8192), (unsigned)nseg);
@@ -560,16 +657,26 @@
     return ST_OK;
 }
 
+extern "C" int st_voxelize_blocks_box_seg(const float* xyz, const float* rgb, int64_t n, const int32_t* seg_off, int nseg,
+                                          double voxel_size, double block_size, double buffer_size, int min_points, int max_blocks,
+                                          int64_t max_voxels, float* feats, int32_t* coords, uint8_t* mask, int64_t* point_index,
+                                          float* block_centres, int32_t* blk_seg, int32_t* seg_vox_off, int32_t* seg_blk_off,
+                                          int64_t* n_voxels_out, int64_t* n_blocks_out, void* ws, int64_t ws_bytes, void* stream_,
+                                          const float* centred_box) {
+    ST_REQUIRE(block_centres != nullptr, "voxelize: block_centres is an output of the blocked call");
+    ST_REQUIRE(nseg == 1 || (blk_seg && seg_blk_off), "voxelize: a batch needs the per-cloud block outputs");
+    return vx_voxelize(xyz, rgb, n, seg_off, nseg, voxel_size, block_size, buffer_size, min_points, max_blocks, max_voxels, feats,
+                       coords, mask, point_index, block_centres, blk_seg, seg_vox_off, seg_blk_off, n_voxels_out, n_blocks_out, ws,
+                       ws_bytes, stream_, 0, centred_box);
+}
 extern "C" int st_voxelize_blocks_seg(const float* xyz, const float* rgb, int64_t n, const int32_t* seg_off, int nseg,
                                       double voxel_size, double block_size, double buffer_size, int min_points, int max_blocks,
                                       int64_t max_voxels, float* feats, int32_t* coords, uint8_t* mask, int64_t* point_index,
                                       float* block_centres, int32_t* blk_seg, int32_t* seg_vox_off, int32_t* seg_blk_off,
                                       int64_t* n_voxels_out, int64_t* n_blocks_out, void* ws, int64_t ws_bytes, void* stream_) {
-    ST_REQUIRE(block_centres != nullptr, "voxelize: block_centres is an output of the blocked call");
-    ST_REQUIRE(nseg == 1 || (blk_seg && seg_blk_off), "voxelize: a batch needs the per-cloud block outputs");
-    return vx_voxelize(xyz, rgb, n, seg_off, nseg, voxel_size, block_size, buffer_size, min_points, max_blocks, max_voxels, feats,
-                       coords, mask, point_index, block_centres, blk_seg, seg_vox_off, seg_blk_off, n_voxels_out, n_blocks_out, ws,
-                       ws_bytes, stream_, 0);
+    return st_voxelize_blocks_box_seg(xyz, rgb, n, seg_off, nseg, voxel_size, block_size, buffer_size, min_points, max_blocks,
+                                      max_voxels, feats, coords, mask, point_index, block_centres, blk_seg, seg_vox_off, seg_blk_off,
+                                      n_voxels_out, n_blocks_out, ws, ws_bytes, stream_, nullptr);
 }
 
 extern "C" int64_t st_voxelize_cloud_workspace_bytes(int64_t n_points, int64_t max_voxels, int nseg) {
diff --git a/smart_tree_amd/data_types/cloud.py b/smart_tree_amd/data_types/cloud.py
--- a/smart_tree_amd/data_types/cloud.py
+++ b/smart_tree_amd/data_types/cloud.py
@@ -33,6 +33,7 @@
     class_l: Optional[torch.Tensor] = None
     filename: Optional[Path] = None
     seg_off: Optional[torch.Tensor] = None
+    centred_box: Optional[torch.Tensor] = None
 
     def __post_init__(self):
         n = self.xyz.shape[0]
@@ -62,6 +63,7 @@
             raise ValueError("Cloud.filter: a batch of clouds (seg_off) needs a boolean mask or a strictly increasing index; "
                              "split() the batch before reordering / resampling its points")
         out = self._map(lambda t: t.index_select(0, mask))
+        out.centred_box = None
         if self.seg_off is not None:
             out.seg_off = torch.searchsorted(mask, self.seg_off.to(mask.dtype)).to(torch.int32)
         return out
@@ -100,6 +102,8 @@
         out = self._map(lambda t: t.to(device))
         if self.seg_off is not None:
             out.seg_off = self.seg_off.to(device)
+        if self.centred_box is not None:
+            out.centred_box = self.centred_box.to(device)
         return out
 
     def cpu(self) -> "Cloud":
@@ -164,7 +168,7 @@
 
     @staticmethod
     def from_numpy(**arrays) -> "Cloud":
-        known = {f.name for f in fields(Cloud)} - {"filename"}
+        known = {f.name for f in fields(Cloud)} - {"filename", "centred_box"}
         kw = {}
         for key, value in arrays.items():
             if key in known:
diff --git a/smart_tree_amd/dataset/augmentations.py b/smart_tree_amd/dataset/augmentations.py
--- a/smart_tree_amd/dataset/augmentations.py
+++ b/smart_tree_amd/dataset/augmentations.py
@@ -24,9 +24,10 @@
             out = torch.empty_like(xyz)
             nseg = cloud.n_seg
             ws = _lib.workspace(256 + 24 * nseg, xyz.device)
-            _lib.check(L.st_centre_cloud_seg(_lib.ptr(xyz), xyz.shape[0], _lib.ptr(cloud.seg_off), nseg, _lib.ptr(out), _lib.ptr(ws),
-                                             ws.numel(), _lib.stream(xyz.device)))
-            return Cloud(out, cloud.rgb, seg_off=cloud.seg_off)
+            box = torch.empty((nseg, 6), dtype=torch.float32, device=xyz.device) if xyz.shape[0] > 0 else None
+            _lib.check(L.st_centre_cloud_box_seg(_lib.ptr(xyz), xyz.shape[0], _lib.ptr(cloud.seg_off), nseg, _lib.ptr(out), _lib.ptr(ws),
+                                                 ws.numel(), _lib.stream(xyz.device), _lib.ptr(box)))
+            return Cloud(out, cloud.rgb, seg_off=cloud.seg_off, centred_box=box)
         if cloud.seg_off is not None:
             raise _lib.StError("batched clouds are centred on the GPU only")
         centre, half = cloud.bbox
diff --git a/smart_tree_amd/dataset/dataset.py b/smart_tree_amd/dataset/dataset.py
--- a/smart_tree_amd/dataset/dataset.py
+++ b/smart_tree_amd/dataset/dataset.py
@@ -28,17 +28,21 @@
 
 def voxelize_blocks(xyz: torch.Tensor, rgb: Optional[torch.Tensor], voxel_size: float, block_size: float = 4,
                     buffer_size: float = 0.4, min_points: int = 20, max_blocks: int = 4096,
-                    seg_off: Optional[torch.Tensor] = None) -> VoxelBatch:
+                    seg_off: Optional[torch.Tensor] = None, centred_box: Optional[torch.Tensor] = None) -> VoxelBatch:
     L = _lib.lib()
     dev = xyz.device
     xyz = xyz.contiguous().float()
     rgb = rgb.contiguous().float() if rgb is not None else None
     n = xyz.shape[0]
     nseg = 1 if seg_off is None else int(seg_off.shape[0]) - 1
-    return _voxelize_blocks(xyz, rgb, n, nseg, seg_off, voxel_size, block_size, buffer_size, min_points, max_blocks)
+    if centred_box is not None:
+        centred_box = centred_box.contiguous().float()
+        if tuple(centred_box.shape) != (nseg, 6):
+            raise ValueError(f"centred_box must be [{nseg},6], got {tuple(centred_box.shape)}")
+    return _voxelize_blocks(xyz, rgb, n, nseg, seg_off, voxel_size, block_size, buffer_size, min_points, max_blocks, centred_box)
 
 
-def _voxelize_blocks(xyz, rgb, n, nseg, seg_off, voxel_size, block_size, buffer_size, min_points, max_blocks):
+def _voxelize_blocks(xyz, rgb, n, nseg, seg_off, voxel_size, block_size, buffer_size, min_points, max_blocks, centred_box=None):
     L = _lib.lib()
     dev = xyz.device
     per_cloud_blocks = max_blocks
@@ -56,17 +60,17 @@
         pidx = torch.empty((cap,), dtype=torch.int64, device=dev)
         centres = torch.empty((max_blocks, 3), dtype=torch.float32, device=dev)
         ws = _lib.workspace(L.st_voxelize_workspace_bytes_seg(n, max_blocks, cap, nseg), dev)
-        rc = L.st_voxelize_blocks_seg(_lib.ptr(xyz), _lib.ptr(rgb), n, _lib.ptr(seg_off), nseg, float(voxel_size),
-                                      float(block_size), float(buffer_size), int(min_points), int(max_blocks), cap,
-                                      _lib.ptr(feats), _lib.ptr(coords), _lib.ptr(mask), _lib.ptr(pidx), _lib.ptr(centres),
-                                      _lib.ptr(blk_seg), _lib.ptr(seg_vox), _lib.ptr(seg_blk), ctypes.byref(n_vox),
-                                      ctypes.byref(n_blk), _lib.ptr(ws), ws.numel(), _lib.stream(dev))
+        rc = L.st_voxelize_blocks_box_seg(_lib.ptr(xyz), _lib.ptr(rgb), n, _lib.ptr(seg_off), nseg, float(voxel_size),
+                                          float(block_size), float(buffer_size), int(min_points), int(max_blocks), cap,
+                                          _lib.ptr(feats), _lib.ptr(coords), _lib.ptr(mask), _lib.ptr(pidx), _lib.ptr(centres),
+                                          _lib.ptr(blk_seg), _lib.ptr(seg_vox), _lib.ptr(seg_blk), ctypes.byref(n_vox),
+                                          ctypes.byref(n_blk), _lib.ptr(ws), ws.numel(), _lib.stream(dev), _lib.ptr(centred_box))
         if rc == 0 or b"exceed max_voxels" not in L.st_last_error():
             break
     if rc != 0 and (b"bounding box of a cloud has more than" in L.st_last_error() or b"exceed max_blocks" in L.st_last_error()) \
             and per_cloud_blocks * nseg < 65535:
         return _voxelize_blocks(xyz, rgb, n, nseg, seg_off, voxel_size, block_size, buffer_size, min_points,
-                                min(per_cloud_blocks * 8, 65535))
+                                min(per_cloud_blocks * 8, 65535), centred_box)
     _lib.check(rc)
     m, b = n_vox.value, n_blk.value
     if n > 0:
@@ -171,7 +175,7 @@
         self.min_points = min_points
         self.file_name = file_name
         self.batch = voxelize_blocks(cloud.xyz, cloud.rgb, voxel_size, block_size, buffer_size, min_points,
-                                     seg_off=cloud.seg_off)
+                                     seg_off=cloud.seg_off, centred_box=getattr(cloud, "centred_box", None))
         self.block_centres = self.batch.block_centres
 
     def __len__(self) -> int:
diff --git a/smart_tree_amd/model/model_inference.py b/smart_tree_amd/model/model_inference.py
--- a/smart_tree_amd/model/model_inference.py
+++ b/smart_tree_amd/model/model_inference.py
@@ -54,7 +54,7 @@
     def forward(self, cloud: Cloud, return_masked: bool = True) -> Cloud:
         cloud = cloud.to_device(self.device)
         if cloud.rgb is None:
-            cloud = Cloud(cloud.xyz, torch.zeros_like(cloud.xyz), seg_off=cloud.seg_off)
+            cloud = Cloud(cloud.xyz, torch.zeros_like(cloud.xyz), seg_off=cloud.seg_off, centred_box=cloud.centred_box)
         with profiling.stage("voxelize"):
             if self.blocking == "whole":
                 vb = voxelize_cloud(cloud.xyz, cloud.rgb, self.voxel_size, seg_off=cloud.seg_off)
```

Result: faster. 927.9 million, median of 6 (+2.4%).
